# jorgeMFS/HYMET

Hardware: AMD Instinct MI355X
Metric: contigs/s + Mbp/s classified, CAMI-medium, 1/2/4/8 MI355X; % HBM roofline (higher is better)
Workload: dtype u64

## Files before the change

hymet_amd/_lib.py:

```python
from __future__ import annotations

import ctypes
import os

HERE = os.path.dirname(os.path.abspath(__file__))
LIB_PATH = os.path.join(HERE, "libhymet_gpu.so")

_c = ctypes
_i64, _u64, _i32, _u32, _vp = _c.c_int64, _c.c_uint64, _c.c_int, _c.c_uint32, _c.c_void_p

_SIGS = {
    "hymet_version": (_i32, []),
    "hymet_init": (_i32, [_i32, _c.POINTER(_vp)]),
    "hymet_destroy": (_i32, [_vp]),
    "hymet_last_error": (_c.c_char_p, []),
    "hymet_set_stream": (_i32, [_vp, _vp]),
    "hymet_sync": (_i32, [_vp]),
    "hymet_prof_enable": (_i32, [_vp, _i32]),
    "hymet_prof_reset": (_i32, [_vp]),
    "hymet_prof_query": (_i32, [_vp, _c.c_char_p, _c.POINTER(_c.c_double), _c.POINTER(_i64), _c.POINTER(_c.c_double)]),
    "hymet_prof_names": (_i32, [_vp, _c.c_char_p, _i64]),
    "hymet_scratch_trim": (_i32, [_vp, _c.POINTER(_i64)]),
    "hymet_scratch_cached": (_i32, [_vp, _c.POINTER(_i64)]),
    "hymet_scratch_stats": (_i32, [_vp, _vp]),
    "hymet_scratch_reserve": (_i32, [_vp, _i64]),
    "hymet_set_oom_hook": (_i32, [_vp, _vp]),
    "hymet_copy_to_host": (_i32, [_vp, _vp, _vp, _i64, _i32]),
    "hymet_copy_to_device": (_i32, [_vp, _vp, _vp, _i64, _i32]),
    "hymet_pack": (_i32, [_vp, _vp, _i64, _i32, _vp, _vp]),
    "hymet_fasta_index": (_i32, [_vp, _i64, _i32, _i64, _c.POINTER(_i64), _vp, _vp, _vp, _vp, _vp]),
    "hymet_fasta_names": (_i32, [_vp, _vp, _vp, _i64, _vp, _vp]),
    "hymet_fasta_compact": (_i32, [_vp, _vp, _i64, _i64, _vp, _vp, _vp, _i64, _vp, _i64, _vp]),
    "hymet_name_hash": (_i32, [_vp, _vp, _vp, _vp, _i64, _vp]),
    "hymet_sort_pairs_u64": (_i32, [_vp, _vp, _vp, _i64, _i32, _i32]),
    "hymet_scan_u32": (_i32, [_vp, _vp, _vp, _i64, _i32, _vp]),
    "hymet_msh_open": (_i32, [_c.c_char_p, _c.POINTER(_vp)]),
    "hymet_msh_info_get": (_i32, [_vp, _vp]),
    "hymet_msh_copy": (_i32, [_vp, _i32, _vp, _vp, _vp, _vp, _vp, _vp]),
    "hymet_msh_upload": (_i32, [_vp, _vp, _i32, _vp, _vp, _i32]),
    "hymet_msh_upload_range": (_i32, [_vp, _vp, _i32, _vp, _vp, _i32, _i64, _i64]),
    "hymet_msh_text_offsets": (_i32, [_vp, _vp, _vp]),
    "hymet_msh_close": (None, [_vp]),
    "hymet_screen_table_slots": (_i64, [_i64]),
    "hymet_screen_table_build": (_i32, [_vp, _vp, _i64, _vp, _i64, _vp, _vp, _i32]),
    "hymet_screen_count": (_i32, [_vp, _vp, _vp, _i64, _i64, _i64, _i32, _u32, _i32, _c.POINTER(_vp), _c.POINTER(_i64),
                                  _c.POINTER(_vp), _c.POINTER(_i64), _c.POINTER(_vp), _u64, _vp, _i64, _vp, _vp]),
    "hymet_screen_stats": (_i32, [_vp, _vp, _i64, _vp, _vp, _vp, _vp]),
    "hymet_screen_winner": (_i32, [_vp, _vp, _i64, _vp, _vp, _i64, _vp, _i64, _vp, _vp, _vp]),
    "hymet_sketch_max_size": (_i64, []),
    "hymet_sketch_batch": (_i32, [_vp, _vp, _vp, _i64, _i32, _u32, _i32, _i64, _vp, _vp, _vp, _i32, _vp, _vp]),
    "hymet_sketch_counted": (_i32, [_vp, _vp, _vp, _i64, _i32, _u32, _i32, _i32, _i64, _vp, _vp, _vp, _i32, _vp, _vp, _vp,
                                    _vp]),
    "hymet_sketch_counted_max_size": (_i32, []),
    "hymet_sketch_counted_tune": (_i32, [_i32]),
    "hymet_sketch_stream_create": (_i32, [_vp, _i32, _u32, _i32, _i32, _i64, _c.POINTER(_vp)]),
    "hymet_sketch_stream_add": (_i32, [_vp, _vp, _vp, _i64, _i64]),
    "hymet_sketch_stream_end_pass": (_i32, [_vp, _c.POINTER(_i32)]),
    "hymet_sketch_stream_result": (_i32, [_vp, _vp, _vp, _c.POINTER(_i32), _vp]),
    "hymet_sketch_stream_destroy": (_i32, [_vp]),
    "hymet_mash_dist": (_i32, [_vp, _vp, _i64, _vp, _i64, _vp, _i64, _vp, _i64, _i64, _i64, _i32, _vp]),
    "hymet_mash_dist_tile": (_i32, [_i32]),
    "hymet_mash_dist_tune": (_i32, [_i32, _i32]),
    "hymet_mash_dist_select": (_i32, [_vp, _vp, _i64, _i64, _vp, _i32, _vp, _vp, _vp, _i64, _c.POINTER(_i64)]),
    "hymet_mash_dist_tri": (_i32, [_vp, _vp, _i64, _vp, _i64, _i64, _i64, _i32, _vp]),
    "hymet_mash_link": (_i32, [_vp, _vp, _i64, _i64, _i64, _vp, _i32, _vp, _vp]),
    "hymet_mash_labels": (_i32, [_vp, _vp, _i64, _vp]),
    "hymet_mash_dist_sparse": (_i32, [_vp, _vp, _i64, _vp, _i64, _vp, _i64, _vp, _i64, _i64, _i64, _i32, _i32, _vp, _i32,
                                      _i64, _vp, _vp, _vp, _i64, _c.POINTER(_i64), _vp]),
    "hymet_mash_link_edges": (_i32, [_vp, _vp, _i64, _i64, _vp, _vp, _vp]),
    "hymet_mash_greedy": (_i32, [_vp, _vp, _i64, _i64, _i64, _vp, _i32, _vp, _vp, _c.POINTER(_i32)]),
    "hymet_mash_greedy_edges": (_i32, [_vp, _vp, _i64, _i64, _vp, _vp, _i32, _vp, _vp, _c.POINTER(_i32)]),
    "hymet_mash_topk_max": (_i32, []),
    "hymet_mash_topk_tune": (_i32, [_i32]),
    "hymet_mash_dist_topk": (_i32, [_vp, _vp, _i64, _i64, _vp, _i32, _i32, _vp, _vp, _vp]),
    "hymet_mash_topk_edges": (_i32, [_vp, _vp, _i64, _vp, _vp, _i32, _i32, _vp, _vp, _vp]),
    "hymet_mm_sketch": (_i32, [_vp, _vp, _vp, _vp, _vp, _i32, _i32, _i32, _i32, _vp, _vp, _i64, _c.POINTER(_i64)]),
    "hymet_mm_index_build": (_i32, [_vp, _vp, _vp, _vp, _vp, _i32, _i32, _i32, _c.POINTER(_vp)]),
    "hymet_mm_index_destroy": (_i32, [_vp]),
    "hymet_mm_index_info": (_i32, [_vp, _c.POINTER(_i32), _c.POINTER(_i32), _c.POINTER(_i32), _c.POINTER(_i64)]),
    "hymet_mm_index_max_occ": (_i32, [_vp, _vp, _c.c_float, _c.POINTER(_i32)]),
    "hymet_mm_index_save": (_i32, [_vp, _vp, _c.c_char_p, _i32, _c.POINTER(_i64)]),
    "hymet_mm_index_load": (_i32, [_vp, _c.c_char_p, _i64, _c.POINTER(_vp), _c.POINTER(_i64)]),
    "hymet_mm_index_export": (_i32, [_vp, _vp, _vp, _vp]),
    "hymet_mm_map": (_i32, [_vp, _vp, _vp, _vp, _vp, _vp, _vp, _vp, _i32, _c.POINTER(_vp)]),
    "hymet_mm_result_size": (_i32, [_vp, _c.POINTER(_i64)]),
    "hymet_mm_result_copy": (_i32, [_vp, _vp, _vp, _vp]),
    "hymet_mm_result_destroy": (_i32, [_vp]),
    "hymet_paf_acc_create": (_i32, [_vp, _c.POINTER(_vp)]),
    "hymet_paf_acc_reset": (_i32, [_vp]),
    "hymet_paf_acc_destroy": (_i32, [_vp]),
    "hymet_paf_acc_info": (_i32, [_vp, _c.POINTER(_i64), _c.POINTER(_vp), _c.POINTER(_vp), _c.POINTER(_vp),
                                  _c.POINTER(_vp), _c.POINTER(_vp)]),
    "hymet_paf_acc_append": (_i32, [_vp, _vp, _vp, _i64, _i64]),
    "hymet_paf_acc_copy": (_i32, [_vp, _vp, _vp, _vp, _vp]),
    "hymet_paf_acc_field": (_i32, [_vp, _vp, _i32, _vp]),
    "hymet_mm_map_acc": (_i32, [_vp, _vp, _vp, _vp, _vp, _vp, _vp, _vp, _i32, _i32, _i32, _i32, _vp]),
    "hymet_emit_paf": (_i32, [_vp, _vp, _vp, _vp, _vp, _vp, _vp, _vp, _vp, _i64, _c.POINTER(_i64), _vp]),
    "hymet_acc_ref_counts": (_i32, [_vp, _vp, _vp]),
    "hymet_acc_classify": (_i32, [_vp, _vp, _i32, _i32] + [_vp] * 15 + [_c.POINTER(_i32)]),
    "hymet_emit_tsv": (_i32, [_vp, _i32, _i32] + [_vp] * 14 + [_i64, _c.POINTER(_i64)]),
    "hymet_mm_chain_dp": (_i32, [_vp, _vp, _vp, _i64, _i32, _i32, _i32, _i32, _i32, _c.c_float, _c.c_float, _vp, _vp]),
    "hymet_mm_mark_compact": (_i32, [_vp, _vp, _vp, _vp, _i64, _vp, _vp, _i32, _vp, _vp, _vp, _c.POINTER(_i64)]),
    "hymet_mm_stamp_scratch": (_i32, [_vp, _c.POINTER(_i64), _c.POINTER(_i64)]),
    "hymet_mm_anchor_sort": (_i32, [_vp, _vp, _vp, _i64, _vp, _i32, _i32, _i32, _u64, _i64, _vp, _vp, _vp, _vp, _vp]),
    "hymet_lca_ref_counts": (_i32, [_vp, _vp, _i64, _vp]),
    "hymet_lca": (_i32, [_vp, _i32, _i32] + [_vp] * 17),
}

class SparseCounters(_c.Structure):
    _fields_ = [("postings", _i64), ("emitted", _i64), ("candidates", _i64)]


_lib = None
_oom_hook = None


def _release_torch_cache(_user):
    try:
        import torch
        torch.cuda.empty_cache()
    except Exception:
        pass


class HymetError(RuntimeError):
    pass


def load():
    global _lib
    if _lib is not None:
        return _lib
    path = os.environ.get("HYMET_LIB", LIB_PATH)
    if not os.path.exists(path):
        raise HymetError(f"{path} not found: build the HIP extension (python -m hymet_amd.build); "
                         "hymet_amd has no CPU fallback")
    lib = ctypes.CDLL(path)
    for name, (res, args) in _SIGS.items():
        fn = getattr(lib, name)
        fn.restype = res
        fn.argtypes = args
    global _oom_hook
    _oom_hook = _c.CFUNCTYPE(None, _vp)(_release_torch_cache)
    lib.hymet_set_oom_hook(_c.cast(_oom_hook, _vp), None)
    _lib = lib
    return lib


def exported_symbols():
    return list(_SIGS)


def check(rc: int, what: str):
    if rc != 0:
        msg = load().hymet_last_error()
        raise HymetError(f"{what} failed ({rc}): {msg.decode() if msg else ''}")


class Gpu:

    def __init__(self, device: int = 0, stream=None):
        import torch

        if not torch.cuda.is_available():
            raise HymetError("no GPU visible: hymet_amd runs on MI355X (gfx950) only")
        self.torch = torch
        self.device = device
        torch.cuda.set_device(device)
        self.dev = torch.device("cuda", device)
        self.lib = load()
        h = _vp()
        check(self.lib.hymet_init(device, _c.byref(h)), "hymet_init")
        self.ctx = h
        self.stream = stream
        self.children = []
        self.bind_stream(stream)

    def fork(self) -> "Gpu":
        child = Gpu(self.device, stream=self.torch.cuda.Stream(device=self.device))
        self.children.append(child)
        return child

    def bind_stream(self, stream=None):
        s = stream if stream is not None else self.torch.cuda.current_stream(self.device)
        check(self.lib.hymet_set_stream(self.ctx, _vp(s.cuda_stream)), "hymet_set_stream")
        self.bound_stream = s

    def call(self, name, *args):
        check(getattr(self.lib, name)(self.ctx, *args), name)

    def sync(self):
        check(self.lib.hymet_sync(self.ctx), "hymet_sync")
        for ch in self.children:
            ch.sync()

    def prof(self, on: bool = True):
        check(self.lib.hymet_prof_enable(self.ctx, int(on)), "hymet_prof_enable")
        for ch in self.children:
            ch.prof(on)

    def prof_reset(self):
        check(self.lib.hymet_prof_reset(self.ctx), "hymet_prof_reset")
        for ch in self.children:
            ch.prof_reset()

    def prof_table(self):
        buf = _c.create_string_buffer(1 << 16)
        check(self.lib.hymet_prof_names(self.ctx, buf, 1 << 16), "hymet_prof_names")
        out = {}
        for name in buf.value.decode().split():
            ms, n, b = _c.c_double(), _i64(), _c.c_double()
            check(self.lib.hymet_prof_query(self.ctx, name.encode(), _c.byref(ms), _c.byref(n), _c.byref(b)), "hymet_prof_query")
            out[name] = (ms.value, n.value, b.value)
        for ch in self.children:
            for name, (ms, n, b) in ch.prof_table().items():
                m0, n0, b0 = out.get(name, (0.0, 0, 0.0))
                out[name] = (m0 + ms, n0 + n, b0 + b)
        return out

    def trim(self) -> int:
        out = _i64()
        check(self.lib.hymet_scratch_trim(self.ctx, _c.byref(out)), "hymet_scratch_trim")
        return out.value

    def reserve(self, nbytes: int):
        check(self.lib.hymet_scratch_reserve(self.ctx, int(nbytes)), "hymet_scratch_reserve")

    def _alloc(self, fn, n, dtype):
        try:
            return fn(int(n), dtype=dtype, device=self.dev)
        except self.torch.OutOfMemoryError:
            if self.trim() == 0:
                raise
            return fn(int(n), dtype=dtype, device=self.dev)

    def empty(self, n, dtype):
        return self._alloc(self.torch.empty, n, dtype)

    def zeros(self, n, dtype):
        return self._alloc(self.torch.zeros, n, dtype)

    def close(self):
        if self.ctx:
            self.lib.hymet_destroy(self.ctx)
            self.ctx = None

    def __del__(self):
        try:
            self.close()
        except Exception:
            pass


def ptr(t) -> _vp:
    return _vp(t.data_ptr())
```

hymet_amd/csrc/common.hpp:

```cpp
#pragma once
#include <hip/hip_runtime.h>
#include <stdint.h>
#include <algorithm>
#include <cstdlib>
#include <map>
#include <string>
#include <utility>
#include <vector>
#include "../../include/hymet_gpu.h"

struct hymet_ctx {
    int device = 0;
    hipStream_t stream = nullptr;
    bool own_stream = false;
    int n_cu = 256;
    bool prof = false;
    std::map<std::string, std::vector<std::pair<hipEvent_t, hipEvent_t>>> ev;
    std::map<std::string, double> bytes;
    std::map<std::string, std::pair<int, double>> dev_bytes;
    int64_t *prof_dev = nullptr;
    void *stage[2] = {nullptr, nullptr};
    hipEvent_t stage_ev[2] = {nullptr, nullptr};
    int64_t *mbox_h = nullptr;
    int64_t *mbox_d = nullptr;
    int32_t *dctr = nullptr;
    int32_t *stamp = nullptr;
    int64_t stamp_cap = 0;
    size_t stamp_cls = 0;
};

namespace hymet {
struct ProfScope {
    hymet_ctx *c;
    const char *name;
    hipEvent_t a = nullptr, b = nullptr;
    ProfScope(hymet_ctx *ctx, const char *n, double alg_bytes = 0.0) : c(ctx), name(n) {
        if (c && c->prof && hipEventCreate(&a) == hipSuccess && hipEventCreate(&b) == hipSuccess) {
            (void)hipEventRecord(a, c->stream);
            c->bytes[name] += alg_bytes;
        }
    }
    ProfScope(hymet_ctx *ctx, const char *n, int slot, double per_unit) : ProfScope(ctx, n, 0.0) {
        if (c && c->prof) c->dev_bytes[name] = {slot, per_unit};
    }
    ~ProfScope() {
        if (c && c->prof && a && b) {
            (void)hipEventRecord(b, c->stream);
            c->ev[name].push_back({a, b});
        }
    }
};
constexpr int kProfSlots = 8;
inline int64_t *prof_dev_slot(hymet_ctx *c, int k) { return c && c->prof && c->prof_dev ? c->prof_dev + k : nullptr; }
}

namespace hymet {
constexpr int kMbox = 64;
inline int64_t *mb_dev(hymet_ctx *c, int i) { return c->mbox_d + i; }
inline int64_t mb_read(const hymet_ctx *c, int i) { return __atomic_load_n(c->mbox_h + i, __ATOMIC_ACQUIRE); }
}

namespace hymet {
inline const char *env_str(const char *name) {
    const char *e = getenv(name);
    return e && *e ? e : nullptr;
}
inline bool env_flag(const char *name, bool dflt = false) {
    const char *e = env_str(name);
    return e ? e[0] != '0' : dflt;
}
inline int64_t env_int(const char *name, int64_t dflt, int64_t lo, int64_t hi) {
    const char *e = env_str(name);
    return e ? std::max(lo, std::min(hi, (int64_t)atoll(e))) : dflt;
}
}

namespace hymet {
void set_error(const std::string &msg);
int fail(int code, const std::string &msg);
int hip_fail(hipError_t e, const char *what);
inline int64_t cdiv(int64_t a, int64_t b) { return (a + b - 1) / b; }
hipError_t scratch_alloc(size_t bytes, hipStream_t stream, void **p, size_t *cls);
void set_oom_hook(void (*hook)(void *), void *user);
void scratch_free(void *p, hipStream_t stream, size_t cls);
hipError_t stamp_scratch(hymet_ctx *ctx, int64_t n, int32_t **out);
void stamp_release(hymet_ctx *ctx);
}

#define HY_CHECK_LAUNCH(what)                                   \
    do {                                                        \
        hipError_t e_ = hipGetLastError();                      \
        if (e_ != hipSuccess) return hymet::hip_fail(e_, what); \
    } while (0)

#define HY_HIP(call)                                            \
    do {                                                        \
        hipError_t e_ = (call);                                 \
        if (e_ != hipSuccess) return hymet::hip_fail(e_, #call); \
    } while (0)

#define HY_ARG(cond, msg)                                                   \
    do {                                                                    \
        if (!(cond)) return hymet::fail(HYMET_E_ARG, std::string(msg));     \
    } while (0)
```

hymet_amd/csrc/mm_chain.hip:

```cpp
#include "mm_common.hpp"

#include <cstdlib>
#include <string>

namespace hymet {
namespace mm {
namespace {

#ifndef HYMET_CHAIN_RING
#define HYMET_CHAIN_RING 128
#endif
#ifndef HYMET_CHAIN_SUMRING
#define HYMET_CHAIN_SUMRING 16
#endif
#ifndef HYMET_CHAIN_BDQ
#define HYMET_CHAIN_BDQ 32
#endif
#ifndef HYMET_CHAIN_IDQ
#define HYMET_CHAIN_IDQ 64
#endif
#ifndef HYMET_CHAIN_SPEC_GAP0
#define HYMET_CHAIN_SPEC_GAP0 2
#endif
#ifndef HYMET_CHAIN_WPE
// ... 1000 lines not shown
                            const int m = min(ni, 64), base = ni - m;
                            bool gt = false;
                            int2 v = make_int2(0, 0);
                            if (lane < m) {
                                v = L(base + lane);
                                gt = key_less(e0y, i, v.x, v.y);
                            }
                            const uint64_t mg = __ballot(gt);
                            const int ngt = __popcll(mg);
                            if (ngt == m && base > 0) {
                                gy = INT32_MIN;
                            } else {
                                gpos = ni - ngt;
                                const int lg = __ffsll((unsigned long long)mg) - 1;
                                gy = rl(v.x, lg), gj = rl(v.y, lg);
                            }
                        }
                        if (lane >= 1 && !key_less(py, i + lane - 1, gy, gj)) ok = false;
                        gap_own = key_less(ky, i + lane, gy, gj);
                    }
#ifdef HYMET_CHAIN_PROF
                    const bool ok_geom = ok;
#endif
                    ok = ok && cand_ok && wok;
                    const uint64_t bad = __ballot(!ok);
                    const int acc = bad ? __ffsll((unsigned long long)bad) - 1 : 64;
#ifdef HYMET_CHAIN_PROF
                    if (acc < Lb) {
                        const int fl = acc;
                        const bool g_ = rl(ok_geom ? 1 : 0, fl), c_ = rl(cand_ok ? 1 : 0, fl), w_ = rl(wok ? 1 : 0, fl);
                        const bool xs = rl(kx != px ? 1 : 0, fl), yr = rl((py > ky - P.max_dist && py < ky) ? 1 : 0, fl);
                        if (!xs) CCOUNT(12);
                        else if (!yr) CCOUNT(13);
                        else if (!g_) CCOUNT(14);
                        else if (!c_) CCOUNT(15);
                        else if (!w_) CCOUNT(16);
                        else CCOUNT(17);
                    }
                    _pcnt[18] += acc;
#endif
                    if (acc < 4) {
                        spec_next = i + spec_gap;
                        spec_gap = min(spec_gap * 2, 64);
                    } else {
                        spec_gap = kSpecGap0;
                    }
                    AMARK(batch_verified);
                    if (acc > 0) {
                        bool ins_all = false;
                        if (i + acc < n) {
                            const int offn = (i - cb) + 64;
                            const int32_t xn = acc < 64 ? rl(kx, acc) : rl(nx, offn - 64);
                            ins_all = xn != rl(kx, acc - 1) && rl(gap_own ? 1 : 0, acc - 1) != 0;
                        }
                        advance(i + acc);
                        const int32_t k = i + lane;
                        const int32_t pk_local = linked ? (lane == 0 ? b0j : k - 1) : -1;
                        const int32_t pw = (int32_t)((uint32_t)(pk_local + 1) | (uint32_t)span_pw);
                        if (lane < acc) {
                            ring[k & kRingMask] = make_int4(kx, ky, fk, pw);
                            xring[k & (kXRing - 1)] = kx;
                        }
                        __builtin_amdgcn_wave_barrier();
                        CCOUNT(7);
                        GCNT(z, 1);
                        GCNT(w, acc);
                        const int nins = ins_all ? acc : acc - 1;
                        if (nins > 0) {
                            if (P.max_dist_inner > 0) {
                                if (gpos < ni) {
                                    const int kk = gpos + lane;
                                    const int2 v = L(kk);
                                    __builtin_amdgcn_wave_barrier();
                                    if (kk < ni) L(kk + nins) = v;
                                }
                                {
                                    if (lane < nins) L(gpos + lane) = make_int2(ky, k);
                                    __builtin_amdgcn_wave_barrier();
                                }
                                if (gpos == 0) lfy = rl(ky, 0), lfj = i;
                                if (gpos == ni) lby = rl(ky, nins - 1), lbj = i + nins - 1;
                                ni += nins;
                                const int v = fk + ksp;
                                int run = lane < nins ? v : INT32_MIN;
                                int sfx;
                                const int vnx = down1(v);
                                if (__ballot(lane >= nins - 1 || v < vnx) == ~0ull) {
                                    run = rl(v, nins - 1);
                                    sfx = lane < nins - 1 ? run : INT32_MIN;
                                } else
                                {
                                    run = suffix_max(run);
                                    sfx = down1(run);
                                    if (lane == 63) sfx = INT32_MIN;
                                }
                                const int vmax = rl(run, 0);
                                while (it > ih && ib_v <= vmax) {
                                    --it;
                                    if (it > ih) ib_v = idq[(it - 1) & (kIdq - 1)].y;
                                }
                                const bool recd = lane < nins && v > sfx;
                                const uint64_t rm = __ballot(recd);
                                const int nr = __popcll(rm);
                                if (it - ih + nr > kIdq) {
                                    iok = false;
                                } else {
                                    const int rank = __popcll(rm & ((1ull << lane) - 1));
                                    if (recd) idq[(it + rank) & (kIdq - 1)] = make_int2(k, v);
                                    __builtin_amdgcn_wave_barrier();
                                    if (it == ih) if_v = rl(v, __ffsll((unsigned long long)rm) - 1);
                                    ib_v = rl(v, 63 - __clzll((long long)rm));
                                    it += nr;
                                }
                            }
                            const int32_t nb0 = i >> 6, nb1 = (i + nins) >> 6;
                            for (int32_t b = nb0; b < nb1; ++b) complete_block(b);
                            const double pl_last = rld(pk, nins - 1);
                            if (((i + nins) & 63) == 0) {
                                t_pr = 0.0, t_j = -1, t_y = 0;
                            } else if (rld(ipm, nins - 1) == pl_last) {
                                if (nb1 > nb0 || (i & 63) == 0 || t_j < 0 || !(t_pr < pl_last))
                                    t_pr = pl_last, t_j = i + nins - 1, t_y = rl(ky, nins - 1);
                            } else
                            {
                                const int32_t tb = (i + nins) & ~63, j = tb + lane;
                                double tp = 0.0;
                                int32_t tj = -1, ty = 0;
                                if (j < i + nins) {
                                    const Ent e = fetch(j);
                                    tp = prio(e.f, e.x, e.y, c), tj = j, ty = e.y;
                                }
                                wave_argmin(tp, tj, ty);
                                t_pr = Ud(tp), t_j = U(tj), t_y = U(ty);
                            }
                            i0 = i + nins;
                        }
                        const int l = acc - 1;
                        if (lane < acc) {
                            P.f[g0 + k] = fk;
                            P.p[g0 + k] = pk_local < 0 ? -1 : (int32_t)(g0 + pk_local);
                        }
                        prev.x = rl(kx, l), prev.y = rl(ky, l), prev.f = rl(fk, l), prev.pw = rl(pw, l);
                        i += acc;
                        AMARK(batch_end);
                        continue;
                    }
                }
            }
            CPROF(2);
            double bp = 0.0;
            int32_t bj = -1;
            Ent eb;
            bool have_eb = false;
            const int32_t ylo = yi - P.max_dist;
            auto in_range = [&](int32_t y, int32_t j) { return y > ylo && (y < yi || (y == yi && qfirst && j == 0)); };
            if (st < i0) {
                bool cert = st <= (fe << 6);
                int32_t wy = 0, src = -1;
                if (cert) {
                    if (st < (fb << 6)) {
                        const int4 v = hsuf[st & 63];
                        bp = st_pr(v), bj = v.z, wy = v.w, src = 0;
                    }
                    if (fb < fe) {
                        if (!bok) cert = false;
                        else if (better(bf_pr, bf_j, bp, bj)) bp = bf_pr, bj = bf_j, wy = bf_y, src = 1;
                    }
                    if ((fe << 6) < i0 && better(t_pr, t_j, bp, bj)) bp = t_pr, bj = t_j, wy = t_y, src = 2;
                }
                if (cert && bj >= 0 && in_range(wy, bj)) {
                    if (src == 1) eb.x = bf_e.x, eb.y = bf_y, eb.f = bf_e.y, eb.pw = bf_e.z, have_eb = true;
                } else {
                    CCOUNT(3);
                    if (cert && bj >= 0) CCOUNT(6);
                    window_best(yi, ylo, true, bp, bj);
                }
            }
            CPROF(3);
            if (bj >= 0) {
                int32_t exact, width;
                if (!have_eb) eb = bj == i - 1 ? prev : fetch(bj);
                const int32_t sc = eb.f + comput_sc(xi, yi, eb.x, eb.y, eb.sp(), P.pen_gap, P.pen_skip, &exact, &width);
                if (width <= P.bw && sc > max_f) max_f = sc, max_j = bj;
                const int32_t n_inner = i0 > st_in ? i0 - st_in : 0;
                bool walk = !exact && n_inner > 0 && yi > 0 && P.max_dist_inner > 0;
                if (walk && iok && it > ih && if_v <= max_f) walk = false;
                CPROF(5);
                if (walk) {
                    CCOUNT(4);
                    const int32_t ylo_in = yi - P.max_dist_inner;
                    if (!overflow) {
                        int cnt = 0;
                        for (int e = lane; e < ni; e += 64) cnt += L(e).x < yi;
                        cnt = wave_sum(cnt);
                        int nsk = 0;
                        for (int top = cnt - 1; top >= 0; top -= 64) {
                            const int e = top - lane;
                            const int nl = min(64, top + 1);
                            int32_t yj = 0, jl = -1, sc_l = 0, w_l = INT32_MAX, pj = -1;
                            if (e >= 0) {
                                const int2 v = L(e);
                                yj = v.x, jl = v.y;
                                const Ent ej = fetch_p(jl);
                                int32_t ex;
                                sc_l = ej.f + comput_sc(xi, yi, ej.x, ej.y, ej.sp(), P.pen_gap, P.pen_skip, &ex, &w_l);
                                pj = ej.p();
                            }
                            const uint64_t mA = __ballot(e >= 0 && yj < ylo_in);
                            const int LA = mA ? __ffsll((unsigned long long)mA) - 1 : nl;
                            const bool valid = lane < LA && w_l <= P.bw;
                            if (valid && pj >= st_in && pj < i0) P.t_global[g0 + pj] = i + 1;
                            t_used = true;
                            __builtin_amdgcn_s_waitcnt(0);
                            const bool stamped = valid && ld_l2(P.t_global + g0 + jl) == i + 1;
                            const int incl = scan_max(valid ? sc_l : INT32_MIN);
                            const int excl = max(shr1(incl, INT32_MIN), max_f);
                            const bool imp = valid && sc_l > excl;
                            int a = imp ? -1 : (valid && stamped ? 1 : 0);
                            int bb = imp ? 0 : kNegInf;
                            scan_maxplus(a, bb);
                            const int s = max(nsk + a, bb);
                            const uint64_t mB = __ballot(valid && !imp && stamped && s > P.max_chn_skip);
                            const int LB = mB ? __ffsll((unsigned long long)mB) - 1 : 64;
                            const int lim = min(LA, LB + 1);
                            const uint64_t mI = __ballot(imp && lane < lim);
                            if (mI) {
                                const int Lh = 63 - __clzll((long long)mI);
                                max_f = rl(sc_l, Lh);
                                max_j = rl(jl, Lh);
                            }
                            if (mB || LA < nl) break;
                            nsk = rl(s, 63);
                            __builtin_amdgcn_wave_barrier();
                        }
                    } else {
                        int n_skip = 0;
                        int32_t cy_ = yi, cj = INT32_MIN;
                        bool first = true;
                        for (;;) {
                            int32_t by = INT32_MIN, bjl = INT32_MIN;
                            for (int32_t j = st_in + lane; j < i0; j += 64) {
                                const int32_t yj = fetch(j).y;
                                const bool below = first ? (yj <= yi - 1) : key_less(yj, j, cy_, cj);
                                if (below && (bjl == INT32_MIN || key_less(by, bjl, yj, j))) by = yj, bjl = j;
                            }
                            auto take = [&](int32_t oy, int32_t oj) {
                                if (oj != INT32_MIN && (bjl == INT32_MIN || key_less(by, bjl, oy, oj))) by = oy, bjl = oj;
                            };
                            take(xstep<0>(by), xstep<0>(bjl));
                            take(xstep<1>(by), xstep<1>(bjl));
                            take(xstep<2>(by), xstep<2>(bjl));
                            take(xstep<3>(by), xstep<3>(bjl));
                            take(xstep<4>(by), xstep<4>(bjl));
                            take(xstep<5>(by), xstep<5>(bjl));
                            if (bjl == INT32_MIN) break;
                            first = false;
                            cy_ = by, cj = bjl;
                            if (by < ylo_in) break;
                            const Ent ej = fetch_p(bjl);
                            int32_t ex, wl;
                            const int32_t sl = ej.f + comput_sc(xi, yi, ej.x, ej.y, ej.sp(), P.pen_gap, P.pen_skip, &ex, &wl);
                            if (wl <= P.bw) {
                                if (sl > max_f) {
                                    max_f = sl, max_j = bjl;
                                    if (n_skip > 0) --n_skip;
                                } else if (ld_l2(P.t_global + g0 + bjl) == i + 1) {
                                    if (++n_skip > P.max_chn_skip) break;
                                }
                                if (ej.p() >= 0) P.t_global[g0 + ej.p()] = i + 1;
                                t_used = true;
                            }
                        }
                    }
                }
            }
            CPROF(4);
            advance(i + 1);
            P.f[g0 + i] = max_f;
            P.p[g0 + i] = max_j < 0 ? -1 : (int32_t)(g0 + max_j);
            prev.x = xi, prev.y = yi, prev.f = max_f, prev.pw = (int32_t)((uint32_t)(max_j + 1) | (uint32_t)span_pw);
            if (lane == 0) {
                ring[i & kRingMask] = make_int4(prev.x, prev.y, prev.f, prev.pw);
                xring[i & (kXRing - 1)] = prev.x;
            }
            __builtin_amdgcn_wave_barrier();
            ++i;
        }
        if (t_used) {
            __builtin_amdgcn_wave_barrier();
            for (int32_t j = lane; j < n; j += 64) P.t_global[g0 + j] = 0;
        }
        CPROF_FLUSH;
        GTIME_STOP;
    }
}

struct BacktrackParams {
    const int64_t *g_start;
    const int32_t *f;
    const int32_t *p;
    uint8_t *t;
    const int32_t *z_cnt;
    const int32_t *z_idx;
    int32_t n_groups;
    int min_cnt, min_sc, max_drop;
    int64_t long_min;
    unsigned long long *prof;
    int32_t *chain_ids;
    uint64_t *chain_u;
    int64_t *chain_first;
    int32_t *n_chains;
};

constexpr int kBtWin = 8;

constexpr int64_t kBtLong = 64;
#ifndef HYMET_BT_GRAB
#define HYMET_BT_GRAB 1
#endif
#ifndef HYMET_BT_STRIPES
#define HYMET_BT_STRIPES 8
#endif
constexpr int kBtGrab = HYMET_BT_GRAB, kBtStripes = HYMET_BT_STRIPES, kBtCtrPad = 64;
#ifndef HYMET_BT_CHUNKS
#define HYMET_BT_CHUNKS 1
#endif
constexpr int kBtChunks = HYMET_BT_CHUNKS;
#ifndef HYMET_BT_PROBE
#define HYMET_BT_PROBE 4
#endif
constexpr int kBtProbe = HYMET_BT_PROBE;

__device__ __forceinline__ int32_t uni(int32_t v) { return __builtin_amdgcn_readfirstlane(v); }
__device__ __forceinline__ int64_t uni64(int64_t v) {
    return (int64_t)((uint64_t)(uint32_t)uni((int32_t)(v >> 32)) << 32 | (uint32_t)uni((int32_t)v));
}

__global__ void bt_long_count_kernel(const int64_t *g_start, const int32_t *order, int32_t n_work, int64_t long_min,
                                     int32_t *cnt) {
    int lo = 0, hi = n_work;
    while (lo < hi) {
        const int mid = (lo + hi) >> 1;
        const int g = order[mid];
        if (g_start[g + 1] - g_start[g] > long_min) lo = mid + 1;
        else hi = mid;
    }
    cnt[0] = lo;
    for (int k = 1; k <= kBtStripes; k++) cnt[k * kBtCtrPad] = 0;
}

__global__ __launch_bounds__(64) void backtrack_long_kernel(BacktrackParams P, const int32_t *list, const int32_t *cnt,
                                                            int32_t *counter) {
    __shared__ int32_t s_w;
    const int lane = threadIdx.x;
    const int32_t n_long = uni(ld_l2(cnt));
    int stripe = (int)(blockIdx.x % kBtStripes), exhausted = 0;
    int32_t w = 0, w_end = 0;
    for (;;) {
        if (w >= w_end) {
            for (;;) {
                if (lane == 0) s_w = atomicAdd(counter + stripe * kBtCtrPad, kBtGrab);
                __syncthreads();
                w = uni(s_w);
                __syncthreads();
                w_end = w + kBtGrab;
                if (stripe + kBtStripes * w < n_long || ++exhausted == kBtStripes) break;
                stripe = stripe + 1 == kBtStripes ? 0 : stripe + 1;
            }
            if (exhausted == kBtStripes) break;
        }
        const int32_t wcur = stripe + kBtStripes * w++;
        if (wcur >= n_long) {
            w = w_end;
            continue;
        }
        const int32_t g = uni(list[wcur]);
        const int64_t g0 = uni64(P.g_start[g]);
        const int64_t z0 = g0, z1 = g0 + uni(P.z_cnt[g]);
        int64_t wpos = g0;
        int nc = 0;
        int64_t k = z1 - 1;
        uint64_t c_probe = 0, c_walk = 0, c_step = 0, c_reload = 0, t_walk = 0, t_post = 0;
        const uint64_t t_g0 = P.prof ? clock64() : 0;
        int64_t ptop = -1;
        int64_t zrem = z1 - z0;
        int32_t zc[kBtProbe], tv[kBtProbe], zfv[kBtProbe];
        int32_t zpv[kBtProbe];
        int32_t tqv[kBtProbe], fqv[kBtProbe];
        bool stale = false;
        while (k >= z0 && zrem > 0) {
            if (ptop < 0 || k <= ptop - 64 * kBtProbe) {
                c_probe++;
                ptop = k;
                stale = false;
#pragma unroll
                for (int c = 0; c < kBtProbe; c++) {
                    const int64_t kk = k - 64 * c - lane;
                    zc[c] = kk >= z0 ? P.z_idx[kk] : 0;
                }
#pragma unroll
                for (int c = 0; c < kBtProbe; c++) {
                    const int64_t kk = k - 64 * c - lane;
                    tv[c] = kk >= z0 ? ld_l2(P.t + zc[c]) : 1;
                }
#pragma unroll
                for (int c = 0; c < kBtProbe; c++) {
                    zfv[c] = tv[c] == 0 ? P.f[zc[c]] : 0;
                    zpv[c] = tv[c] == 0 ? P.p[zc[c]] : -1;
                }
#pragma unroll
                for (int c = 0; c < kBtProbe; c++) {
                    const bool q = tv[c] == 0 && zpv[c] >= 0;
                    tqv[c] = q ? ld_l2(P.t + zpv[c]) : 0;
                    fqv[c] = q ? P.f[zpv[c]] : 0;
                }
            } else if (stale) {
                stale = false;
#pragma unroll
                for (int c = 0; c < kBtProbe; c++) {
                    const int64_t kk = ptop - 64 * c - lane;
                    if (kk >= z0 && kk <= k && tv[c] == 0) tv[c] = ld_l2(P.t + zc[c]);
                }
            }
            const int d = (int)(ptop - k);
            int hit = -1;
            int32_t zsel = 0, zfsel = 0;
            int32_t zpsel = -1;
            int32_t tqsel = 0, fqsel = 0;
#pragma unroll
            for (int c = kBtProbe - 1; c >= 0; c--) {
                const uint64_t m = __ballot(tv[c] == 0 && 64 * c + lane >= d);
                if (m) {
                    const int h = __ffsll((unsigned long long)m) - 1;
                    hit = 64 * c + h;
                    zsel = __builtin_amdgcn_readlane(zc[c], h);
                    zfsel = __builtin_amdgcn_readlane(zfv[c], h);
                    zpsel = __builtin_amdgcn_readlane(zpv[c], h);
                    tqsel = __builtin_amdgcn_readlane(tqv[c], h);
                    fqsel = __builtin_amdgcn_readlane(fqv[c], h);
                }
            }
            hit = uni(hit);
            if (hit < 0) {
                k = ptop - 64 * kBtProbe;
                continue;
            }
            const int64_t zi = (int64_t)uni(zsel);
            k = ptop - hit - 1;
            const int32_t zf = uni(zfsel);
            if (P.min_cnt >= 2 && (zpsel < 0 || uni(tqsel) != 0)) {
                const int32_t sv = zpsel < 0 ? zf : zf - uni(fqsel);
                if (sv > 0) P.t[zi] = 1, zrem--;
                c_walk++;
                continue;
            }
            stale = true;
            int32_t *buf = P.chain_ids + wpos;
            buf[0] = (int32_t)zi;
            P.t[zi] = 2;
            int64_t len = 1, nv = 0;
            int64_t zc_len = 1, zc_nv = 0;
            int32_t max_s = 0;
            int64_t nxt = (int64_t)uni(zpsel);
            int64_t whi = -1;
            int32_t wpc[kBtChunks], wfc[kBtChunks], wtc[kBtChunks];
#pragma unroll
            for (int c = 0; c < kBtChunks; c++) wpc[c] = -1, wfc[c] = 0, wtc[c] = 1;
            c_walk++;
            const uint64_t t_w0 = P.prof ? clock64() : 0;
            for (;;) {
                c_step++;
                if (nxt < 0) {
                    if (zf > max_s) max_s = zf, nv = len, zc_nv = zc_len;
                    break;
                }
                if (nxt > whi || nxt <= whi - 64 * kBtChunks) {
                    c_reload++;
                    whi = nxt;
#pragma unroll
                    for (int c = 0; c < kBtChunks; c++) {
                        const int64_t jj = nxt - 64 * c - lane;
                        const bool ok = jj >= g0;
                        wpc[c] = ok ? P.p[jj] : -1;
                        wfc[c] = ok ? P.f[jj] : 0;
                        wtc[c] = ok ? ld_l2(P.t + jj) : 1;
                    }
                }
                const int d = (int)(whi - nxt);
                const int cc = d >> 6, o = d & 63;
                int32_t wp = wpc[0], wf = wfc[0], wt = wtc[0];
#pragma unroll
                for (int c = 1; c < kBtChunks; c++)
                    if (cc == c) wp = wpc[c], wf = wfc[c], wt = wtc[c];
                const int64_t j = whi - 64 * cc - lane;
                const bool in = lane >= o;
                const uint64_t ms = __ballot(in && (lane == 63 || wp != j - 1 || j - 1 < g0));
                const int R = uni(__ffsll((unsigned long long)ms) - 1);
                const bool cand = in && lane <= R;
                const int32_t sv = cand ? zf - wf : INT32_MIN;
                const int32_t incl = scan_max(sv);
                const int32_t ex = max(max_s, shr1(incl, INT32_MIN));
                const bool upd = cand && sv > ex;
                const bool drop = cand && !upd && (int64_t)ex - sv > P.max_drop;
                const uint64_t mdrop = __ballot(drop);
                const uint64_t mb = mdrop | __ballot(cand && wt != 0);
                const uint64_t mupd = __ballot(upd);
                int last = R, ulim = R;
                const bool done = mb != 0;
                if (done) {
                    const int E = uni(__ffsll((unsigned long long)mb) - 1);
                    last = E - 1;
                    ulim = (mdrop >> E) & 1 ? E - 1 : E;
                }
                const uint64_t lim = ulim < 0 ? 0ull : ulim >= 63 ? ~0ull : (2ull << ulim) - 1;
                const uint64_t mu = mupd & lim;
                const uint64_t mz = __ballot(lane >= o && lane <= last && wf >= P.min_sc);
                if (mu) {
                    const int u = 63 - __clzll((long long)mu);
                    nv = len + (u - o);
                    zc_nv = zc_len + __popcll(mz & ((1ull << u) - 1));
                    max_s = __builtin_amdgcn_readlane(incl, u);
                }
                if (lane >= o && lane <= last) {
                    buf[len + (lane - o)] = (int32_t)j;
                    P.t[j] = 2;
                }
                len += last - o + 1;
                zc_len += __popcll(mz);
                if (done) break;
                nxt = (int64_t)__builtin_amdgcn_readlane(wp, R);
            }
            const uint64_t t_w1 = P.prof ? clock64() : 0;
            t_walk += t_w1 - t_w0;
            __builtin_amdgcn_fence(__ATOMIC_SEQ_CST, "workgroup");
            for (int64_t a = nv + lane; a < len; a += 64) P.t[ld_l2(buf + a)] = 0;
            zrem -= zc_nv;
            const int32_t sc = nv == 0 ? 0 : max_s;
            if (sc >= P.min_sc && nv > 0 && nv >= P.min_cnt) {
                P.chain_u[g0 + nc] = (uint64_t)(uint32_t)sc << 32 | (uint32_t)nv;
                P.chain_first[g0 + nc] = wpos;
                nc++;
                wpos += nv;
            } else {
                for (int64_t a = lane; a < nv; a += 64) P.t[ld_l2(buf + a)] = 1;
            }
            __builtin_amdgcn_fence(__ATOMIC_SEQ_CST, "workgroup");
            if (P.prof) t_post += clock64() - t_w1;
        }
        P.n_chains[g] = nc;
        if (P.prof) {
            const uint64_t v[8] = {1, c_probe, c_walk, c_step, c_reload, t_walk, t_post, clock64() - t_g0};
            for (int q = 0; q < 8; q++) atomicAdd(P.prof + q, lane == 0 ? (unsigned long long)v[q] : 0ull);
        }
    }
}


__global__ __launch_bounds__(64) void backtrack_groups_kernel(BacktrackParams P) {
    const int g = blockIdx.x * blockDim.x + threadIdx.x;
    if (g >= P.n_groups) return;
    const int64_t g0 = P.g_start[g];
    if (P.g_start[g + 1] - g0 > P.long_min) return;
    int64_t wpos = g0;
    int nc = 0;
    const int64_t z0 = g0, z1 = g0 + P.z_cnt[g];
    int64_t k = z1 - 1;
    while (k >= z0) {
        int32_t zc[kBtWin], tc[kBtWin];
#pragma unroll
        for (int u = 0; u < kBtWin; u++) zc[u] = k - u >= z0 ? P.z_idx[k - u] : 0;
#pragma unroll
        for (int u = 0; u < kBtWin; u++) tc[u] = k - u >= z0 ? P.t[zc[u]] : 1;
        int hit = -1;
#pragma unroll
        for (int u = kBtWin - 1; u >= 0; u--)
            if (tc[u] == 0) hit = u;
        if (hit < 0) {
            k -= kBtWin;
            continue;
        }
        int64_t zi = 0;
#pragma unroll
        for (int u = 0; u < kBtWin; u++)
            if (u == hit) zi = zc[u];
        k -= hit + 1;
        const int32_t zf = P.f[zi];
        int32_t *buf = P.chain_ids + wpos;
        int64_t len = 0, nv = 0;
        int32_t max_s = 0;
        int64_t i = zi, nxt = P.p[zi];
        int64_t whi = -1;
        int32_t wp[kBtWin], wf[kBtWin], wt[kBtWin];
        for (;;) {
            buf[len++] = (int32_t)i;
            P.t[i] = 2;
            int32_t fn = 0, tn = 1;
            int64_t pn = -1;
            if (nxt >= 0) {
                if (nxt > whi || nxt <= whi - kBtWin) {
                    whi = nxt;
#pragma unroll
                    for (int u = 0; u < kBtWin; u++) {
                        const bool ok = nxt - u >= g0;
                        wp[u] = ok ? P.p[nxt - u] : -1;
                        wf[u] = ok ? P.f[nxt - u] : 0;
                        wt[u] = ok ? P.t[nxt - u] : 1;
                    }
                }
                const int64_t o = whi - nxt;
#pragma unroll
                for (int u = 0; u < kBtWin; u++)
                    if (o == u) fn = wf[u], tn = wt[u], pn = wp[u];
            }
            const int32_t s = nxt < 0 ? zf : zf - fn;
            if (s > max_s) {
                max_s = s;
                nv = len;
            } else if (max_s - s > P.max_drop) {
                break;
            }
            if (nxt < 0 || tn != 0) break;
            i = nxt;
            nxt = pn;
        }
        const int32_t sc = nv == 0 ? 0 : max_s;
        for (int64_t a = nv; a < len; a++) P.t[buf[a]] = 0;
        if (sc >= P.min_sc && nv > 0 && nv >= P.min_cnt) {
            P.chain_u[g0 + nc] = (uint64_t)(uint32_t)sc << 32 | (uint32_t)nv;
            P.chain_first[g0 + nc] = wpos;
            nc++;
            wpos += nv;
        } else {
            for (int64_t a = 0; a < nv; a++) P.t[buf[a]] = 1;
        }
    }
    P.n_chains[g] = nc;
}

}


#ifndef HYMET_CHAIN_SMALL
#define HYMET_CHAIN_SMALL 24
#endif
constexpr int kSmall = HYMET_CHAIN_SMALL;
#ifndef HYMET_CHAIN_SMALL_LONG
#define HYMET_CHAIN_SMALL_LONG 16
#endif
constexpr int kSmallLong = HYMET_CHAIN_SMALL_LONG < kSmall ? HYMET_CHAIN_SMALL_LONG : kSmall;

__global__ void chain_small_split_kernel(const int64_t *g_start, const int32_t *order, int32_t n_work, int32_t *split,
                                         int32_t *counter, int small_max) {
    if (threadIdx.x != 0) return;
    for (int k = 0; k < kChainStripes; k++) counter[k * kChainCtrPad] = 0;
    int32_t lo = 0, hi = n_work;
    while (lo < hi) {
        const int32_t mid = (lo + hi) >> 1;
        const int g = order[mid];
        if (g_start[g + 1] - g_start[g] <= small_max) hi = mid;
        else lo = mid + 1;
    }
    *split = lo;
}

__global__ __launch_bounds__(256) void chain_work_anchors_kernel(const int64_t *g_start, const int32_t *order,
                                                                  int32_t n_work, const int32_t *split, int64_t *cnt) {
    __shared__ unsigned long long sw, ss;
    if (threadIdx.x == 0) sw = 0, ss = 0;
    __syncthreads();
    const int32_t sp = *split;
    unsigned long long w = 0, s = 0;
    for (int32_t k = blockIdx.x * 256 + threadIdx.x; k < n_work; k += gridDim.x * 256) {
        const int g = order[k];
        const unsigned long long a = (unsigned long long)(g_start[g + 1] - g_start[g]);
        if (k < sp) w += a;
        else s += a;
    }
    for (int o = 32; o > 0; o >>= 1) w += __shfl_xor(w, o), s += __shfl_xor(s, o);
    if ((threadIdx.x & 63) == 0) atomicAdd(&sw, w), atomicAdd(&ss, s);
    __syncthreads();
    if (threadIdx.x == 0) {
        atomicAdd(reinterpret_cast<unsigned long long *>(cnt), sw);
        atomicAdd(reinterpret_cast<unsigned long long *>(cnt + 1), ss);
    }
}

__global__ __launch_bounds__(64) void chain_small_kernel(ChainParams P, const int32_t *split) {
    const int32_t w = *split + (int32_t)(blockIdx.x * 64 + threadIdx.x);
    if (w >= P.n_work) return;
    const int g = P.order[w];
    const int64_t g0 = P.g_start[g];
    const int n = (int)(P.g_start[g + 1] - g0);
    const bool qfirst = P.g_qfirst[g] != 0;
    const double c = 0.5 * (double)P.pen_gap;
    int32_t X[kSmall], Y[kSmall], F[kSmall], PJ[kSmall], T[kSmall];
    int8_t ord[kSmall];
    for (int j = 0; j < n; ++j) {
        X[j] = P.ax[g0 + j], Y[j] = (int32_t)P.ay[g0 + j];
        F[j] = 0, PJ[j] = -1, T[j] = -1;
        int k = j;
        while (k > 0 && Y[ord[k - 1]] > Y[j]) {
            ord[k] = ord[k - 1];
            --k;
        }
        ord[k] = (int8_t)j;
    }
    uint32_t in_out = 0, in_in = 0;
    int size_out = 0, size_in = 0, i0 = 0, st = 0, st_in = 0;
    for (int i = 0; i < n; ++i) {
        const int32_t xi = X[i], yi = Y[i];
        int32_t max_f = P.span, max_j = -1;
        if (i0 < i && X[i0] != xi) {
            for (int j = i0; j < i; ++j) {
                in_out |= 1u << j, size_out++;
                if (P.max_dist_inner > 0) in_in |= 1u << j, size_in++;
            }
            i0 = i;
        }
        while (st < i && ((int64_t)(uint32_t)xi > (int64_t)(uint32_t)X[st] + P.max_dist || size_out > P.cap_rmq_size)) {
            if (st < i0) in_out &= ~(1u << st), size_out--;
            ++st;
        }
        if (P.max_dist_inner > 0)
            while (st_in < i &&
                   ((int64_t)(uint32_t)xi > (int64_t)(uint32_t)X[st_in] + P.max_dist_inner || size_in > P.cap_rmq_size)) {
                if (st_in < i0) in_in &= ~(1u << st_in), size_in--;
                ++st_in;
            }
        double bp = 0.0;
        int32_t bj = -1;
        const int32_t ylo = yi - P.max_dist;
        for (uint32_t m = in_out; m; m &= m - 1) {
            const int j = __ffs(m) - 1;
            const int32_t yj = Y[j];
            if (yj > ylo && (yj < yi || (yj == yi && qfirst && j == 0))) {
                const double pr = prio(F[j], X[j], yj, c);
                if (better(pr, j, bp, bj)) bp = pr, bj = j;
            }
        }
        if (bj >= 0) {
            int32_t exact, width;
            const int32_t sc = F[bj] + comput_sc(xi, yi, X[bj], Y[bj], P.span, P.pen_gap, P.pen_skip, &exact, &width);
            if (width <= P.bw && sc > max_f) max_f = sc, max_j = bj;
            if (!exact && size_in > 0 && yi > 0) {
                const int32_t ylo_in = yi - P.max_dist_inner;
                int r = n - 1;
                while (r >= 0 && Y[ord[r]] >= yi) --r;
                int n_skip = 0;
                for (; r >= 0; --r) {
                    const int jj = ord[r];
                    if (Y[jj] < ylo_in) break;
                    if (!(in_in >> jj & 1)) continue;
                    int32_t ex2, w2;
                    const int32_t sc2 = F[jj] + comput_sc(xi, yi, X[jj], Y[jj], P.span, P.pen_gap, P.pen_skip, &ex2, &w2);
                    if (w2 <= P.bw) {
                        if (sc2 > max_f) {
                            max_f = sc2, max_j = jj;
                            if (n_skip > 0) --n_skip;
                        } else if (T[jj] == i) {
                            if (++n_skip > P.max_chn_skip) break;
                        }
                        if (PJ[jj] >= 0) T[PJ[jj]] = i;
                    }
                }
            }
        }
        F[i] = max_f, PJ[i] = max_j;
        P.f[g0 + i] = max_f;
        P.p[g0 + i] = max_j < 0 ? -1 : (int32_t)(g0 + max_j);
    }
}

int launch_chain_raw(hipStream_t st, const ChainParams &P0, int64_t blocks, int32_t *split) {
    ChainParams P = P0;
    hipLaunchKernelGGL(chain_small_split_kernel, dim3(1), dim3(64), 0, st, P.g_start, P.order, P.n_work, split,
                       P.work_counter, P.max_dist > 10000 ? kSmallLong : kSmall);
    HY_CHECK_LAUNCH("chain_small_split_kernel");
    P.work_end = split;
    const bool long_pass = P.max_dist > 10000;
    if (long_pass) hipLaunchKernelGGL(chain_groups_kernel<1>, dim3((unsigned)blocks), dim3(64), kChainLds, st, P);
    else hipLaunchKernelGGL(chain_groups_kernel<0>, dim3((unsigned)blocks), dim3(64), kChainLds, st, P);
    HY_CHECK_LAUNCH("chain_groups_kernel");
    hipLaunchKernelGGL(chain_small_kernel, dim3((unsigned)cdiv(P.n_work, 64)), dim3(64), 0, st, P, (const int32_t *)split);
    HY_CHECK_LAUNCH("chain_small_kernel");
    return HYMET_OK;
}

int launch_chain(hymet_ctx *ctx, const int32_t *ax, const uint32_t *ay, int span, const int64_t *g_start, const uint8_t *g_qfirst,
                 const int32_t *order, int32_t n_work, int32_t *f, int32_t *p, int32_t *t_global, int max_dist,
                 int max_dist_inner, int bw, int max_chn_skip, int cap_rmq_size, float pen_gap, float pen_skip,
                 int64_t n_anchors, int64_t n_groups) {
    if (n_work <= 0) return HYMET_OK;
    DevBuf cnt, sum, split;
    const size_t n_sum = (size_t)(n_anchors >> 6) + (size_t)n_groups + 2;
    HY_HIP(sum.alloc(16 * kGSumInts * n_sum, ctx->stream));
    HY_HIP(cnt.alloc(4 * (size_t)kChainCtrPad * kChainStripes, ctx->stream));
    HY_HIP(split.alloc(4, ctx->stream));
    if (max_dist < bw) max_dist = bw;
    if (max_dist_inner <= 0 || max_dist_inner >= max_dist) max_dist_inner = 0;
    ChainParams P{ax, ay, span, g_start, g_qfirst, order, n_work, cnt.as<int32_t>(), f, p, t_global, sum.as<int4>(), max_dist, max_dist_inner, bw, max_chn_skip, cap_rmq_size, pen_gap, pen_skip, nullptr};
    int64_t blocks = n_work;
    int per_cu = 0;
    const bool long_pass = max_dist > 10000;
    auto kern = long_pass ? chain_groups_kernel<1> : chain_groups_kernel<0>;
    if (hipOccupancyMaxActiveBlocksPerMultiprocessor(&per_cu, kern, 64, kChainLds) != hipSuccess ||
        per_cu <= 0)
        per_cu = 8;
    per_cu = (int)env_int("HYMET_CHAIN_WAVES", per_cu, 1, per_cu);
    const int64_t cap = (int64_t)ctx->n_cu * per_cu;
    if (blocks > cap) blocks = cap;
    const int slot = long_pass ? 2 : 0;
    hipStream_t st = ctx->stream;
    {
        ProfScope _ps(ctx, long_pass ? "mm_chain_long" : "mm_chain", slot, 24.0);
        hipLaunchKernelGGL(chain_small_split_kernel, dim3(1), dim3(64), 0, st, P.g_start, P.order, P.n_work,
                           split.as<int32_t>(), P.work_counter, long_pass ? kSmallLong : kSmall);
        HY_CHECK_LAUNCH("chain_small_split_kernel");
        if (int64_t *pc = prof_dev_slot(ctx, slot)) {
            const unsigned wb = (unsigned)std::min<int64_t>(cdiv(P.n_work, 256), 1024);
            hipLaunchKernelGGL(chain_work_anchors_kernel, dim3(wb), dim3(256), 0, st, P.g_start, P.order, P.n_work,
                               (const int32_t *)split.as<int32_t>(), pc);
            HY_CHECK_LAUNCH("chain_work_anchors_kernel");
        }
        P.work_end = split.as<int32_t>();
        if (long_pass) hipLaunchKernelGGL(chain_groups_kernel<1>, dim3((unsigned)blocks), dim3(64), kChainLds, st, P);
        else hipLaunchKernelGGL(chain_groups_kernel<0>, dim3((unsigned)blocks), dim3(64), kChainLds, st, P);
        HY_CHECK_LAUNCH("chain_groups_kernel");
    }
    ProfScope _pl(ctx, long_pass ? "mm_chain_long_small" : "mm_chain_small", slot + 1, 24.0);
    hipLaunchKernelGGL(chain_small_kernel, dim3((unsigned)cdiv(P.n_work, 64)), dim3(64), 0, st, P, (const int32_t *)split.as<int32_t>());
    HY_CHECK_LAUNCH("chain_small_kernel");
    return HYMET_OK;
}

int launch_backtrack(hymet_ctx *ctx, const int64_t *g_start, const int32_t *f, const int32_t *p, uint8_t *t,
                     const int32_t *z_cnt, const int32_t *z_idx, int32_t n_groups, const int32_t *order, int32_t n_work,
                     int min_cnt, int min_sc, int max_drop, int32_t *chain_ids, uint64_t *chain_u, int64_t *chain_first,
                     int32_t *n_chains, int64_t n_anchors) {
    if (n_groups <= 0) return HYMET_OK;
    const int64_t long_min = env_int("HYMET_BT_LONG", kBtLong, 0, INT64_MAX);
    const bool prof = env_flag("HYMET_BT_PROF");
    DevBuf pbuf;
    if (prof) {
        HY_HIP(pbuf.alloc(64, ctx->stream));
        HY_HIP(hipMemsetAsync(pbuf.p, 0, 64, ctx->stream));
    }
    BacktrackParams P{g_start,  f,         p,       t,           z_cnt,    z_idx, n_groups, min_cnt, min_sc, max_drop,
                      long_min, (unsigned long long *)pbuf.p, chain_ids, chain_u, chain_first, n_chains};
    DevBuf cnt;
    HY_HIP(cnt.alloc(4 * (size_t)kBtCtrPad * (kBtStripes + 1), ctx->stream));
    ProfScope _ps(ctx, "mm_backtrack", 18.0 * (double)n_anchors);
    if (n_work > 0) {
        hipLaunchKernelGGL(bt_long_count_kernel, dim3(1), dim3(1), 0, ctx->stream, g_start, order, n_work, long_min,
                           cnt.as<int32_t>());
        HY_CHECK_LAUNCH("bt_long_count_kernel");
    }
    hipLaunchKernelGGL(backtrack_groups_kernel, dim3((unsigned)cdiv(n_groups, 64)), dim3(64), 0, ctx->stream, P);
    HY_CHECK_LAUNCH("backtrack_groups_kernel");
    if (n_work > 0) {
        ProfScope _pl(ctx, "mm_backtrack.long");
        const int per_cu = (int)env_int("HYMET_BT_WAVES", 24, 1, 1024);
        const int64_t nb = std::min<int64_t>(n_work, (int64_t)ctx->n_cu * per_cu);
        hipLaunchKernelGGL(backtrack_long_kernel, dim3((unsigned)nb), dim3(64), 0, ctx->stream, P, order,
                           cnt.as<int32_t>(), cnt.as<int32_t>() + kBtCtrPad);
        HY_CHECK_LAUNCH("backtrack_long_kernel");
    }
    if (prof) {
        unsigned long long h[8];
        HY_HIP(hipMemcpyAsync(h, pbuf.p, 64, hipMemcpyDeviceToHost, ctx->stream));
        HY_HIP(hipStreamSynchronize(ctx->stream));
        fprintf(stderr, "[bt_long] groups=%llu probes=%llu walks=%llu steps=%llu reloads=%llu cyc_walk=%.3g cyc_post=%.3g cyc_all=%.3g\n",
                h[0], h[1], h[2], h[3], h[4], (double)h[5], (double)h[6], (double)h[7]);
    }
    return HYMET_OK;
}

}
}
```

hymet_amd/csrc/mm_chainset.hip:

```cpp
#include "mm_stages.hpp"

#include <algorithm>
#include <cstdio>

namespace hymet {
namespace mm {

int launch_chain(hymet_ctx *ctx, const int32_t *ax, const uint32_t *ay, int span, const int64_t *g_start, const uint8_t *g_qfirst,
                 const int32_t *order, int32_t n_work, int32_t *f, int32_t *p, int32_t *t_global, int max_dist,
                 int max_dist_inner, int bw, int max_chn_skip, int cap_rmq_size, float pen_gap, float pen_skip,
                 int64_t n_anchors, int64_t n_groups);
int launch_backtrack(hymet_ctx *ctx, const int64_t *g_start, const int32_t *f, const int32_t *p, uint8_t *t,
                     const int32_t *z_cnt, const int32_t *z_idx, int32_t n_groups, const int32_t *order, int32_t n_work,
                     int min_cnt, int min_sc, int max_drop, int32_t *chain_ids, uint64_t *chain_u, int64_t *chain_first,
                     int32_t *n_chains, int64_t n_anchors);

namespace {

constexpr int kGTile = 16384;

__device__ __forceinline__ uint64_t group_tile_bits(const uint32_t *hb, int64_t n, const int64_t *qoff, int n_q, int64_t t0,
                                                    uint64_t *qs) {
    __shared__ int s_q0;
    const int tid = threadIdx.x;
    const int64_t t1 = min(t0 + kGTile, n);
    const int64_t a0 = t0 + 64 * (int64_t)tid;
    const uint64_t hw = a0 < n ? reinterpret_cast<const uint64_t *>(hb)[a0 >> 6] : 0;
    qs[tid] = 0;
    if (tid == 0) {
        int lo = 0, hi = n_q;
        while (lo < hi) {
            const int mid = (lo + hi) >> 1;
            if (qoff[mid + 1] <= t0) lo = mid + 1;
            else hi = mid;
        }
        s_q0 = lo;
    }
    __syncthreads();
    for (int q = s_q0 + tid; q < n_q; q += 256) {
        const int64_t a = qoff[q];
        if (a >= t1) break;
        if (a >= t0 && a < qoff[q + 1]) atomicOr((unsigned long long *)&qs[(a - t0) >> 6], 1ull << ((a - t0) & 63));
    }
    __syncthreads();
    const int64_t m = n - a0;
    const uint64_t live = m >= 64 ? ~0ull : m > 0 ? (1ull << m) - 1 : 0ull;
    return (hw | qs[tid]) & live;
}

__global__ __launch_bounds__(256) void group_heads_count_kernel(const uint32_t *hb, int64_t n, const int64_t *qoff, int n_q,
                                                          uint32_t *tile_cnt) {
    __shared__ uint64_t qs[kGTile / 64];
    __shared__ uint32_t ws[4];
    const uint64_t h = group_tile_bits(hb, n, qoff, n_q, (int64_t)blockIdx.x * kGTile, qs);
    uint32_t c = (uint32_t)__popcll(h);
    for (int o = 32; o > 0; o >>= 1) c += (uint32_t)__shfl_xor((int)c, o, 64);
    if ((threadIdx.x & 63) == 0) ws[threadIdx.x >> 6] = c;
    __syncthreads();
    if (threadIdx.x == 0) tile_cnt[blockIdx.x] = ws[0] + ws[1] + ws[2] + ws[3];
}

__global__ __launch_bounds__(256) void group_heads_write_kernel(const uint32_t *hb, int64_t n, const int64_t *qoff, int n_q,
                                                          const int64_t *tile_off, int64_t *g_start, uint8_t *qfirst,
                                                          int64_t G) {
    __shared__ uint64_t qs[kGTile / 64];
    __shared__ uint32_t ws[4];
    const int64_t t0 = (int64_t)blockIdx.x * kGTile;
    uint64_t h = group_tile_bits(hb, n, qoff, n_q, t0, qs);
    const int lane = threadIdx.x & 63, w = threadIdx.x >> 6;
    const uint32_t c = (uint32_t)__popcll(h);
    uint32_t inc = c;
    for (int d = 1; d < 64; d <<= 1) {
        const uint32_t o = (uint32_t)__shfl_up((int)inc, d, 64);
        if (lane >= d) inc += o;
    }
    if (lane == 63) ws[w] = inc;
    __syncthreads();
    int64_t g = tile_off[blockIdx.x] + inc - c;
    for (int k = 0; k < w; k++) g += ws[k];
    const uint64_t qw = qs[threadIdx.x];
    const int64_t a0 = t0 + 64 * (int64_t)threadIdx.x;
    while (h) {
        const int b = __ffsll((unsigned long long)h) - 1;
        h &= h - 1;
        g_start[g] = a0 + b;
        qfirst[g] = (uint8_t)(qw >> b & 1);
        ++g;
    }
    if (blockIdx.x == gridDim.x - 1 && threadIdx.x == 0) g_start[G] = n;
}

__global__ void x_low_kernel(const uint64_t *x, int64_t n, uint32_t *x32) {
    const int64_t i = (int64_t)blockIdx.x * blockDim.x + threadIdx.x;
    if (i < n) x32[i] = (uint32_t)x[i];
}

__global__ __launch_bounds__(256) void head_bits_x_kernel(const uint64_t *x, int64_t n, uint64_t *hb) {
    const int64_t i = (int64_t)blockIdx.x * 256 + threadIdx.x;
    const bool hd = i < n && (i == 0 || (x[i] >> 32) != (x[i - 1] >> 32));
    const uint64_t b = __ballot(hd);
    if ((threadIdx.x & 63) == 0 && i < n) hb[i >> 6] = b;
}

__global__ void max_group_kernel(const int64_t *g_start, const int32_t *order, int32_t G, int64_t *out) {
    if (blockIdx.x != 0 || threadIdx.x != 0) return;
    int64_t best = 0;
    for (int32_t w = 0; w < G; w++) {
        const int g = order[w];
        const int64_t sz = g_start[g + 1] - g_start[g];
        best = max(best, sz);
        if (sz < 0xffff) break;
    }
    *out = best;
}

__global__ void nonwork_fp_kernel(const int64_t *g_start, int32_t G, int min_cnt, int32_t *f, int32_t *p) {
    const int g = blockIdx.x * blockDim.x + threadIdx.x;
    if (g >= G) return;
    const int64_t a0 = g_start[g], a1 = g_start[g + 1];
    if (a1 - a0 >= min_cnt) return;
    for (int64_t a = a0; a < a1; a++) f[a] = 0, p[a] = -1;
}

__global__ void group_size_kernel(const int64_t *g_start, int32_t G, int min_cnt, uint32_t *key, uint32_t *gidx,
                                  uint32_t *is_work, uint8_t *qfirst, int32_t *zlists) {
    const int g = blockIdx.x * blockDim.x + threadIdx.x;
    if (g < 8) zlists[g] = 0;
    if (g >= G) return;
    if (qfirst) qfirst[g] = 0;
    const int64_t sz = g_start[g + 1] - g_start[g];
    key[g] = 0xffffu - (uint32_t)min(sz, (int64_t)0xffff);
    gidx[g] = (uint32_t)g;
    is_work[g] = sz >= min_cnt ? 1u : 0u;
}

constexpr int kZs = 2048;
constexpr int kZRuns = 16;
constexpr int kZmLds = 6144;
constexpr int kZmUnit = 2048;
constexpr int kZLane = 16;
#ifndef HYMET_Z_DEPTH
#define HYMET_Z_DEPTH 8
#endif
constexpr int kZDepth = HYMET_Z_DEPTH;

struct ZParams {
    const int32_t *f;
    const int64_t *g_start;
    const int32_t *order;
    int32_t G;
    int min_sc, max_runs;
    int zm_lds, zm_unit;
    uint64_t *zkey;
    int32_t *z_idx;
    int32_t *z_cnt;
    int32_t *z_runs;
    int32_t *run_start;
    int32_t *lists;
    int32_t *merge_list;
    int64_t *mergeu_list;
    int32_t *mid_list;
    int32_t *big_list;
    int64_t *big_off;
    int64_t *mail;
};

__global__ void zsplit_kernel(ZParams P) {
    if (threadIdx.x != 0 || blockIdx.x != 0) return;
    int32_t lo = 0, hi = P.G;
    while (lo < hi) {
        const int32_t mid = (lo + hi) >> 1;
        const int g = P.order[mid];
        if (P.g_start[g + 1] - P.g_start[g] <= kZLane) hi = mid;
        else lo = mid + 1;
    }
    P.lists[0] = lo;
}

__device__ __forceinline__ uint64_t shfl64(uint64_t v, int src) {
    const uint32_t lo = (uint32_t)__shfl((int)(uint32_t)v, src, 64);
    const uint32_t hi = (uint32_t)__shfl((int)(uint32_t)(v >> 32), src, 64);
    return (uint64_t)hi << 32 | lo;
}

__global__ __launch_bounds__(256) void zorder_wave_kernel(ZParams P) {
    const int lane = threadIdx.x & 63;
    const int32_t split = P.lists[0];
    const int nw = (int)(gridDim.x * (blockDim.x >> 6));
    int32_t pend[3] = {0, 0, 0};
    int np[3] = {0, 0, 0};
    unsigned long long big_m = 0;
    int32_t *const lst[3] = {P.merge_list, P.mid_list, P.big_list};
    auto flush = [&](int l) {
        if (np[l] == 0) return;
        int base = 0;
        if (lane == 0) base = atomicAdd(P.lists + (l == 0 ? 3 : l == 1 ? 1 : 2), np[l]);
        base = __shfl(base, 0, 64);
        if (lane < np[l]) lst[l][base + lane] = pend[l];
        np[l] = 0;
    };
    auto push = [&](int l, int g) {
        if (lane == np[l]) pend[l] = g;
        if (++np[l] == 64) flush(l);
    };
    for (int wb = (int)(blockIdx.x * (blockDim.x >> 6) + (threadIdx.x >> 6)); wb < split; wb += 64 * nw) {
        const int64_t wl = (int64_t)wb + (int64_t)lane * nw;
        int gl = 0;
        int64_t sl = 0, el = 0;
        if (wl < split) {
            gl = P.order[wl];
            sl = P.g_start[gl];
            el = P.g_start[gl + 1];
        }
        const int nr = (int)min((int64_t)64, ((int64_t)split - wb + nw - 1) / nw);
        for (int r = 0; r < nr; r++) {
            const int g = __builtin_amdgcn_readlane(gl, r);
            const int64_t g0 = (int64_t)((uint64_t)(uint32_t)__builtin_amdgcn_readlane((int32_t)(sl >> 32), r) << 32 |
                                         (uint32_t)__builtin_amdgcn_readlane((int32_t)sl, r));
            const int64_t n = (int64_t)((uint64_t)(uint32_t)__builtin_amdgcn_readlane((int32_t)(el >> 32), r) << 32 |
                                        (uint32_t)__builtin_amdgcn_readlane((int32_t)el, r)) - g0;
            int32_t *rs = P.run_start + (int64_t)g * kZRuns;
            int m = 0, K = 0;
            uint64_t last = 0;
            const uint64_t below = (1ull << lane) - 1;
            for (int64_t base0 = 0; base0 < n; base0 += 64 * kZDepth) {
                int32_t fc[kZDepth];
#pragma unroll
                for (int d = 0; d < kZDepth; d++) {
                    const int64_t i = base0 + 64 * d + lane;
                    fc[d] = i < n ? P.f[g0 + i] : 0;
                }
#pragma unroll
                for (int d = 0; d < kZDepth; d++) {
                    const int64_t i = base0 + 64 * d + lane;
                    const bool ok = i < n;
                    const int32_t fv = fc[d];
                    const bool z = ok && fv >= P.min_sc;
                    const uint64_t bal = __ballot(z);
                    if (bal == 0) continue;
                    const uint64_t key = (uint64_t)(uint32_t)fv << 32 | (uint32_t)(g0 + i);
                    const uint64_t lower = bal & below;
                    const int pos = m + __popcll(lower);
                    const int prev = lower ? 63 - __clzll((long long)lower) : lane;
                    uint64_t pk = shfl64(key, prev);
                    if (!lower) pk = last;
                    const bool desc = z && pos > 0 && key < pk;
                    const uint64_t dbal = __ballot(desc);
                    if (z) P.z_idx[g0 + pos] = (int32_t)(g0 + i);
                    if (desc) {
                        const int r = K + 1 + __popcll(dbal & below);
                        if (r < kZRuns) rs[r] = pos;
                    }
                    K += __popcll(dbal);
                    m += __popcll(bal);
                    last = shfl64(key, 63 - __clzll((long long)bal));
                }
            }
            const int runs = m > 0 ? K + 1 : 0;
            if (lane == 0) {
                rs[0] = 0;
                P.z_cnt[g] = m;
                P.z_runs[g] = runs;
            }
            if (runs > 1) {
                int m2 = 0;
                for (int64_t base0 = 0; base0 < n; base0 += 64 * kZDepth) {
                    int32_t fc[kZDepth];
#pragma unroll
                    for (int d = 0; d < kZDepth; d++) {
                        const int64_t i = base0 + 64 * d + lane;
                        fc[d] = i < n ? P.f[g0 + i] : 0;
                    }
#pragma unroll
                    for (int d = 0; d < kZDepth; d++) {
                        const int64_t i = base0 + 64 * d + lane;
                        const bool z = i < n && fc[d] >= P.min_sc;
                        const uint64_t bal = __ballot(z);
                        if (bal == 0) continue;
                        if (z) P.zkey[g0 + m2 + __popcll(bal & below)] = (uint64_t)(uint32_t)fc[d] << 32 | (uint32_t)(g0 + i);
                        m2 += __popcll(bal);
                    }
                }
            }
            if (runs > 1 && runs <= P.max_runs) {
                if (m <= P.zm_lds) {
                    push(0, g);
                } else {
                    const int nu = (m + P.zm_unit - 1) / P.zm_unit;
                    int base = 0;
                    if (lane == 0) base = atomicAdd(P.lists + 6, nu);
                    base = __shfl(base, 0, 64);
                    for (int u = lane; u < nu; u += 64) P.mergeu_list[base + u] = (int64_t)g << 32 | (uint32_t)u;
                }
            }
            if (runs > P.max_runs) {
                if (m <= kZs) {
                    push(1, g);
                } else {
                    push(2, g);
                    big_m += (unsigned long long)m;
                }
            }
        }
    }
    flush(0), flush(1), flush(2);
    if (lane == 0 && big_m) atomicAdd((unsigned long long *)(P.lists + 4), big_m);
}

__global__ __launch_bounds__(256) void zorder_lane_kernel(ZParams P) {
    const int32_t w = P.lists[0] + (int32_t)(blockIdx.x * blockDim.x + threadIdx.x);
    if (w >= P.G) return;
    const int g = P.order[w];
    const int64_t g0 = P.g_start[g];
    const int n = (int)(P.g_start[g + 1] - g0);
    uint64_t key[kZLane];
#pragma unroll
    for (int j = 0; j < kZLane; j++) {
        const int32_t fv = j < n ? P.f[g0 + j] : 0;
        key[j] = j < n && fv >= P.min_sc ? (uint64_t)(uint32_t)fv << 32 | (uint32_t)(g0 + j) : ~0ull;
    }
    int m = 0;
#pragma unroll
    for (int j = 0; j < kZLane; j++) {
        if (key[j] == ~0ull) continue;
        int r = 0;
#pragma unroll
        for (int k = 0; k < kZLane; k++) r += key[k] < key[j];
        P.z_idx[g0 + r] = (int32_t)(uint32_t)key[j];
        m++;
    }
    P.z_cnt[g] = m;
    P.z_runs[g] = m > 0 ? 1 : 0;
}

__device__ __forceinline__ void zmerge_group(const uint64_t *zk, const int32_t *rs, int K, int m, int qa, int qb,
                                             int32_t *out) {
    const int S = (qb - qa + (int)blockDim.x - 1) / (int)blockDim.x;
    const int q0 = qa + (int)threadIdx.x * S, q1 = min(q0 + S, qb);
    if (q0 >= qb) return;
    int rsr[kZRuns + 1], lo[kZRuns];
#pragma unroll
    for (int k = 0; k <= kZRuns; k++) rsr[k] = k <= K ? rs[k] : m;
    int own = 0, own_s = 0;
#pragma unroll
    for (int k = 1; k < kZRuns; k++)
        if (k < K && rsr[k] <= q0) own = k, own_s = rsr[k];
    uint64_t prev = ~0ull;
    for (int q = q0; q < q1; q++) {
        const uint64_t key = zk[q];
        const bool restart = key < prev;
        prev = key;
        if (restart && q > q0) own++, own_s = q;
        int pos = q - own_s;
#pragma unroll
        for (int k = 0; k < kZRuns; k++) {
            if (k < K && k != own) {
                const int s1 = rsr[k + 1];
                int l = restart ? rsr[k] : lo[k];
                if (l < s1 && zk[l] < key) {
                    int b = 1;
                    while (l + b < s1 && zk[l + b] < key) {
                        l += b;
                        b <<= 1;
                    }
                    int a = l + 1, e = min(l + b, s1);
                    while (a < e) {
                        const int mid = (a + e) >> 1;
                        if (zk[mid] < key) a = mid + 1;
                        else e = mid;
                    }
                    l = a;
                }
                lo[k] = l;
                pos += l - rsr[k];
            }
        }
        out[pos] = (int32_t)(uint32_t)key;
    }
}

__global__ __launch_bounds__(256) void zmerge_kernel(ZParams P) {
    __shared__ uint64_t sk[kZmLds];
    __shared__ int32_t srs[kZRuns + 1];
    const int n_list = P.lists[3], n_units = P.lists[6];
    if (blockIdx.x == 0 && threadIdx.x == 0) {
        P.mail[0] = P.lists[2];
        P.mail[1] = *reinterpret_cast<const int64_t *>(P.lists + 4);
    }
    for (int w = blockIdx.x; w < n_units + n_list; w += gridDim.x) {
        const bool unit = w < n_units;
        const int64_t uw = unit ? P.mergeu_list[w] : 0;
        const int g = unit ? (int)(uw >> 32) : P.merge_list[w - n_units];
        const int K = P.z_runs[g];
        const int64_t z0 = P.g_start[g];
        const int m = P.z_cnt[g];
        const int32_t *rs = P.run_start + (int64_t)g * kZRuns;
        const uint64_t *zk = P.zkey + z0;
        __syncthreads();
        if (threadIdx.x <= K) srs[threadIdx.x] = threadIdx.x < K ? rs[threadIdx.x] : m;
        if (!unit)
            for (int q = threadIdx.x; q < m; q += blockDim.x) sk[q] = zk[q];
        __syncthreads();
        if (unit) {
            const int qa = (int)(uint32_t)uw * P.zm_unit;
            zmerge_group(zk, srs, K, m, qa, min(qa + P.zm_unit, m), P.z_idx + z0);
        } else {
            zmerge_group(sk, srs, K, m, 0, m, P.z_idx + z0);
        }
    }
}

__global__ __launch_bounds__(256) void zsort_block_kernel(ZParams P) {
    __shared__ uint64_t s[kZs];
    const int n_list = P.lists[1];
    for (int w = blockIdx.x; w < n_list; w += gridDim.x) {
        const int g = P.mid_list[w];
        const int64_t z0 = P.g_start[g];
        const int n = P.z_cnt[g];
        int np = 128;
        while (np < n) np <<= 1;
        for (int i = threadIdx.x; i < np; i += 256) s[i] = i < n ? P.zkey[z0 + i] : ~0ull;
        __syncthreads();
        for (int k = 2; k <= np; k <<= 1)
            for (int j = k >> 1; j > 0; j >>= 1) {
                for (int i = threadIdx.x; i < np; i += 256) {
                    const int ij = i ^ j;
                    if (ij > i) {
                        const uint64_t a = s[i], b = s[ij];
                        if (((i & k) == 0) == (a > b)) {
                            s[i] = b;
                            s[ij] = a;
                        }
                    }
                }
                __syncthreads();
            }
        for (int i = threadIdx.x; i < n; i += 256) P.z_idx[z0 + i] = (int32_t)(uint32_t)s[i];
        __syncthreads();
    }
}

__global__ void zbig_count_kernel(ZParams P, int32_t n_big, uint32_t *cnt) {
    const int r = blockIdx.x * blockDim.x + threadIdx.x;
    if (r < n_big) cnt[r] = (uint32_t)P.z_cnt[P.big_list[r]];
}

__global__ void zbig_gather_kernel(ZParams P, uint64_t *skey, uint32_t *sval) {
    const int r = blockIdx.x, g = P.big_list[r];
    const int64_t z0 = P.g_start[g], n = P.z_cnt[g], o = P.big_off[r];
    for (int64_t t = threadIdx.x; t < n; t += blockDim.x) {
        const uint64_t k = P.zkey[z0 + t];
        skey[o + t] = (uint64_t)r << 32 | (k >> 32);
        sval[o + t] = (uint32_t)k;
    }
}

__global__ void zbig_scatter_kernel(ZParams P, const uint32_t *sval) {
    const int r = blockIdx.x, g = P.big_list[r];
    const int64_t z0 = P.g_start[g], n = P.z_cnt[g], o = P.big_off[r];
    for (int64_t t = threadIdx.x; t < n; t += blockDim.x) P.z_idx[z0 + t] = (int32_t)sval[o + t];
}

__global__ void chain_list_kernel(const int64_t *g_start, const int32_t *n_chains, const int64_t *c_pos, int32_t G,
                                  const uint64_t *chain_u, const int64_t *chain_first, const int32_t *chain_ids,
                                  uint64_t *ckey, uint64_t *cu, int64_t *cfirst) {
    const int g = blockIdx.x * blockDim.x + threadIdx.x;
    if (g >= G) return;
    const int64_t g0 = g_start[g];
    int64_t o = c_pos[g];
    for (int c = 0; c < n_chains[g]; c++, o++) {
        const int64_t fo = chain_first[g0 + c];
        ckey[o] = (uint64_t)chain_ids[fo + (uint32_t)chain_u[g0 + c] - 1];
        cu[o] = chain_u[g0 + c];
        cfirst[o] = fo;
    }
}

__global__ void chain_cnt_kernel(const uint64_t *cu, const uint32_t *cq, const uint32_t *qflag, int64_t n, uint32_t *cnt,
                                 uint32_t *cnt2) {
    const int64_t i = (int64_t)blockIdx.x * blockDim.x + threadIdx.x;
    if (i >= n) return;
    const uint32_t m = (uint32_t)cu[i];
    const bool fl = qflag && qflag[cq[i]];
    cnt[i] = fl ? 0u : m;
    if (cnt2) cnt2[i] = fl ? m : 0u;
}

__global__ void rechain_flag_kernel(const uint32_t *ay, const int32_t *chain_ids, const uint64_t *cu, const int64_t *cfirst,
                                    const int64_t *qc, const int64_t *qlen, int n_q, int rescue_size, float rescue_ratio,
                                    uint32_t *flag) {
    const int q = blockIdx.x * blockDim.x + threadIdx.x;
    if (q >= n_q) return;
    const int64_t c0 = qc[q], nc = qc[q + 1] - c0;
    uint32_t f = 0;
    if (nc > 1) {
        const int32_t m = (int32_t)cu[c0];
        const int64_t fo = cfirst[c0];
        const int32_t st = (int32_t)ay[chain_ids[fo + m - 1]], en = (int32_t)ay[chain_ids[fo]];
        const int32_t ql = (int32_t)qlen[q];
        if (ql - (en - st) > rescue_size || (float)(en - st) > __fmul_rn((float)ql, rescue_ratio)) f = 1;
    }
    flag[q] = f;
}

__global__ void chain_qb_kernel(const int64_t *qc, const int64_t *bpos, int64_t n_chain, int64_t nb, int n_q, int64_t *qb) {
    const int q = blockIdx.x * blockDim.x + threadIdx.x;
    if (q > n_q) return;
    const int64_t c = qc[q];
    qb[q] = c < n_chain ? bpos[c] : nb;
}

__device__ __forceinline__ uint32_t keep_bits16(const uint8_t *t, int64_t n, const uint32_t *qflag, const int64_t *qoff,
                                                int n_q, int64_t e0) {
    if (e0 >= n) return 0u;
    int lo = 0, hi = n_q - 1;
    while (lo < hi) {
        const int mid = (lo + hi + 1) >> 1;
        if (qoff[mid] <= e0) lo = mid;
        else hi = mid - 1;
    }
    int q = lo;
    int64_t qend = qoff[q + 1];
    uint32_t v[4] = {0, 0, 0, 0};
    if (e0 + 16 <= n) {
        const uint4 w = *reinterpret_cast<const uint4 *>(t + e0);
        v[0] = w.x, v[1] = w.y, v[2] = w.z, v[3] = w.w;
    } else {
#pragma unroll
        for (int u = 0; u < 16; u++) v[u >> 2] |= (e0 + u < n ? (uint32_t)t[e0 + u] : 0u) << (8 * (u & 3));
    }
    uint32_t bits = 0, fl = qflag[q];
#pragma unroll
    for (int u = 0; u < 16; u++) {
        while (e0 + u >= qend && q + 1 < n_q) {
            q++;
            qend = qoff[q + 1];
            fl = qflag[q];
        }
        bits |= (uint32_t)((v[u >> 2] >> (8 * (u & 3)) & 0xffu) == 2u && fl != 0) << u;
    }
    return bits;
}

__global__ __launch_bounds__(256) void mark_count_kernel(const uint8_t *t, int64_t n, const uint32_t *qflag,
                                                         const int64_t *qoff, int n_q, uint32_t *cnt, int64_t *last_kept) {
    __shared__ uint32_t ws[4];
    __shared__ int64_t wl[4];
    const int64_t e0 = (int64_t)blockIdx.x * 4096 + threadIdx.x * 16;
    const uint32_t kb = keep_bits16(t, n, qflag, qoff, n_q, e0);
    uint32_t c = __popc(kb);
    long long l = kb ? e0 + 31 - __clz((int)kb) : -1;
    for (int o = 32; o > 0; o >>= 1) {
        c += __shfl_xor((int)c, o, 64);
        l = max(l, __shfl_xor(l, o, 64));
    }
    if ((threadIdx.x & 63) == 0) ws[threadIdx.x >> 6] = c, wl[threadIdx.x >> 6] = l;
    __syncthreads();
    if (threadIdx.x == 0) {
        cnt[blockIdx.x] = ws[0] + ws[1] + ws[2] + ws[3];
        last_kept[blockIdx.x] = max(max(wl[0], wl[1]), max(wl[2], wl[3]));
    }
}

__global__ __launch_bounds__(256) void mark_compact_kernel(const uint8_t *t, int64_t n, const uint32_t *qflag,
                                                           const int64_t *qoff, int n_q, const int64_t *tile_off,
                                                           const int64_t *last_kept, const uint64_t *ax, const uint32_t *ay,
                                                           uint64_t *ox, uint32_t *oy, uint32_t *ohb, uint32_t *ox32) {
    __shared__ uint32_t rc[64];
    __shared__ uint32_t nk[64];
    __shared__ uint32_t lx[64];
    __shared__ uint16_t kb[256];
    const int64_t t0 = (int64_t)blockIdx.x * 4096;
    const int lane = threadIdx.x & 63, w = threadIdx.x >> 6;
    kb[threadIdx.x] = (uint16_t)keep_bits16(t, n, qflag, qoff, n_q, t0 + threadIdx.x * 16);
    __syncthreads();
    bool m[16];
#pragma unroll
    for (int j = 0; j < 16; j++) {
        const int r = j * 256 + threadIdx.x;
        m[j] = (kb[r >> 4] >> (r & 15)) & 1;
        const uint64_t b = __ballot(m[j]);
        if (lane == 0) rc[j * 4 + w] = (uint32_t)__popcll(b);
    }
    __syncthreads();
    uint32_t v = 0, inc = 0;
    if (w == 0) nk[lane] = rc[lane];
    if (w == 0) {
        v = rc[lane];
        inc = v;
        for (int d = 1; d < 64; d <<= 1) {
            const uint32_t o = (uint32_t)__shfl_up((int)inc, d, 64);
            if (lane >= d) inc += o;
        }
    }
    __syncthreads();
    if (w == 0) rc[lane] = inc - v;
    __syncthreads();
    const int64_t base = tile_off[blockIdx.x];
    uint32_t xh[16];
#pragma unroll
    for (int j = 0; j < 16; j++) {
        const uint64_t b = __ballot(m[j]);
        xh[j] = 0;
        if (m[j]) {
            const int64_t e = t0 + j * 256 + threadIdx.x;
            const int64_t o = base + rc[j * 4 + w] + __popcll(b & ((1ull << lane) - 1));
            const uint64_t xv = ax[e];
            xh[j] = (uint32_t)(xv >> 32);
            ox[o] = xv;
            ox32[o] = (uint32_t)xv;
            oy[o] = ay[e];
        }
        if (b && lane == 63 - __clzll((long long)b)) lx[j * 4 + w] = xh[j];
    }
    __syncthreads();
#pragma unroll
    for (int j = 0; j < 16; j++) {
        const uint64_t b = __ballot(m[j]);
        const uint64_t below = b & ((1ull << lane) - 1);
        const int src = below ? 63 - __clzll((long long)below) : lane;
        const uint32_t xp = (uint32_t)__shfl((int)xh[j], src, 64);
        if (m[j]) {
            bool hd;
            if (below) {
                hd = xp != xh[j];
            } else {
                int c = j * 4 + w - 1;
                while (c >= 0 && nk[c] == 0) --c;
                if (c >= 0) {
                    hd = lx[c] != xh[j];
                } else {
                    int64_t tt = (int64_t)blockIdx.x - 1;
                    while (tt >= 0 && last_kept[tt] < 0) --tt;
                    hd = tt < 0 || (uint32_t)(ax[last_kept[tt]] >> 32) != xh[j];
                }
            }
            if (hd) {
                const int64_t o = base + rc[j * 4 + w] + __popcll(below);
                atomicOr(ohb + (o >> 5), 1u << (o & 31));
            }
        }
    }
}

__global__ void chain_query_kernel(const uint64_t *ckey, int64_t n, const int64_t *a_off, int n_q, uint32_t *cq) {
    const int64_t c = (int64_t)blockIdx.x * blockDim.x + threadIdx.x;
    if (c < n) cq[c] = (uint32_t)upper_idx(a_off, n_q, (int64_t)ckey[c]);
}

__global__ void count_per_query_kernel(const uint32_t *cq, int64_t n, int n_q, int64_t *q_first) {
    const int64_t p = (int64_t)blockIdx.x * blockDim.x + threadIdx.x;
    if (p > n) return;
    const int64_t qp = p == 0 ? -1 : (int64_t)cq[p - 1];
    const int64_t qc = p == n ? (int64_t)n_q : (int64_t)cq[p];
    for (int64_t q = qp + 1; q <= qc; q++) q_first[q] = p;
}

struct Groups {
    DevBuf g_start;
    DevBuf qfirst;
    int64_t G = 0;
};

struct WorkList {
    DevBuf order;
    DevBuf zlists;
    int64_t n_work = 0, largest = 0;
};

struct DpArgs {
    int max_dist, max_dist_inner, bw, max_chn_skip, cap_rmq_size;
    float pen_gap, pen_skip;
    int min_cnt;
};

struct ZOrder {
    DevBuf idx, cnt;
};

struct Backtrack {
    DevBuf ids, u, first, n_chains;
};

static int derive_heads(hymet_ctx *ctx, AnchorSet &A) {
    const int64_t n = A.n;
    if (!A.has_hb) {
        HY_HIP(A.hb.alloc(head_bits_bytes(n), ctx->stream));
        LAUNCH1(head_bits_x_kernel, n, A.ax.as<uint64_t>(), n, A.hb.as<uint64_t>());
        A.has_hb = true;
    }
    if (!A.has_x32) {
        HY_HIP(A.ax32.alloc(4 * (size_t)n, ctx->stream));
        LAUNCH1(x_low_kernel, n, A.ax.as<uint64_t>(), n, A.ax32.as<uint32_t>());
        A.has_x32 = true;
    }
    return HYMET_OK;
}

static int build_groups(hymet_ctx *ctx, const AnchorSet &A, int n_q, Groups &Gr) {
    const int64_t n = A.n, ntile = cdiv(n, kGTile);
    DevBuf tcnt, toff;
    HY_HIP(tcnt.alloc(4 * (size_t)(ntile + 1), ctx->stream));
    HY_HIP(toff.alloc(8 * (size_t)(ntile + 1), ctx->stream));
    hipLaunchKernelGGL(group_heads_count_kernel, dim3((unsigned)ntile), dim3(256), 0, ctx->stream, A.hb.as<uint32_t>(), n,
                       A.d_off.as<int64_t>(), n_q, tcnt.as<uint32_t>());
    HY_CHECK_LAUNCH("group_heads_count_kernel");
    int rc = exclusive_scan_u32_i64(ctx, tcnt.as<uint32_t>(), toff.as<int64_t>(), ntile, &Gr.G);
    if (rc) return rc;
    HY_HIP(Gr.g_start.alloc(8 * (size_t)(Gr.G + 1), ctx->stream));
    HY_HIP(Gr.qfirst.alloc((size_t)Gr.G, ctx->stream));
    hipLaunchKernelGGL(group_heads_write_kernel, dim3((unsigned)ntile), dim3(256), 0, ctx->stream, A.hb.as<uint32_t>(), n,
                       A.d_off.as<int64_t>(), n_q, toff.as<int64_t>(), Gr.g_start.as<int64_t>(), Gr.qfirst.as<uint8_t>(), Gr.G);
    HY_CHECK_LAUNCH("group_heads_write_kernel");
    return HYMET_OK;
}

static int build_work_list(hymet_ctx *ctx, const Groups &Gr, int min_cnt, WorkList &W) {
    const int64_t G = Gr.G;
    DevBuf skey, sidx, swork, skey2, sidx2, wpos;
    for (DevBuf *b : {&skey, &sidx, &swork, &skey2, &sidx2}) HY_HIP(b->alloc(4 * (size_t)G, ctx->stream));
    HY_HIP(W.zlists.alloc(32, ctx->stream));
    LAUNCH1(group_size_kernel, std::max<int64_t>(G, 8), Gr.g_start.as<int64_t>(), (int32_t)G, min_cnt, skey.as<uint32_t>(),
            sidx.as<uint32_t>(), swork.as<uint32_t>(), (uint8_t *)nullptr, W.zlists.as<int32_t>());
    int rc = scan_flags(ctx, swork.as<uint32_t>(), G, wpos, &W.n_work);
    if (rc) return rc;
    uint32_t *kp = skey.as<uint32_t>(), *ka = skey2.as<uint32_t>(), *vp = sidx.as<uint32_t>(), *va = sidx2.as<uint32_t>();
    rc = sort_pairs(ctx, kp, ka, vp, va, G, 0, 16, "radix_sort_groups");
    if (rc) return rc;
    LAUNCH1(max_group_kernel, 1, Gr.g_start.as<int64_t>(), (const int32_t *)vp, (int32_t)G, mb_dev(ctx, kMbGmax));
    HY_HIP(hipStreamSynchronize(ctx->stream));
    W.largest = mb_read(ctx, kMbGmax);
    HY_ARG(W.largest < (1ll << 24) - 1, "chaining: an anchor group exceeds 2^24 anchors");
    W.order.swap(vp == sidx.as<uint32_t>() ? sidx : sidx2);
    return HYMET_OK;
}

static int chain_dp(hymet_ctx *ctx, const DpArgs &a, const AnchorSet &A, const Groups &Gr, const WorkList &W, DevBuf &f,
                    DevBuf &p) {
    HY_HIP(f.alloc(4 * (size_t)A.n, ctx->stream));
    HY_HIP(p.alloc(4 * (size_t)A.n, ctx->stream));
    int32_t *stamp = nullptr;
    HY_HIP(stamp_scratch(ctx, A.n, &stamp));
    LAUNCH1(nonwork_fp_kernel, Gr.G, Gr.g_start.as<int64_t>(), (int32_t)Gr.G, a.min_cnt, f.as<int32_t>(), p.as<int32_t>());
    return launch_chain(ctx, A.ax32.as<int32_t>(), A.ay.as<uint32_t>(), A.span, Gr.g_start.as<int64_t>(), Gr.qfirst.as<uint8_t>(),
                        W.order.as<int32_t>(), (int32_t)W.n_work, f.as<int32_t>(), p.as<int32_t>(), stamp, a.max_dist,
                        a.max_dist_inner, a.bw, a.max_chn_skip, a.cap_rmq_size, a.pen_gap, a.pen_skip, A.n, Gr.G);
}

static int z_order(hymet_ctx *ctx, int min_sc, const DevBuf &f, int64_t n, const Groups &Gr, const WorkList &W, ZOrder &Z) {
    const int64_t G = Gr.G;
    DevBuf zkey, z_runs, run_start, merge_list, mergeu_list, mid_list, big_list, big_off;
    HY_HIP(zkey.alloc(8 * (size_t)n, ctx->stream));
    HY_HIP(Z.idx.alloc(4 * (size_t)n, ctx->stream));
    HY_HIP(Z.cnt.alloc(4 * (size_t)G, ctx->stream));
    HY_HIP(z_runs.alloc(4 * (size_t)G, ctx->stream));
    HY_HIP(run_start.alloc(4 * (size_t)G * kZRuns, ctx->stream));
    HY_HIP(merge_list.alloc(4 * (size_t)G, ctx->stream));
    const int zm_lds = (int)env_int("HYMET_ZM_LDS", kZmLds, 0, kZmLds);
    const int zm_unit = (int)env_int("HYMET_ZM_UNIT", kZmUnit, 1, INT32_MAX);
    const int max_runs = (int)env_int("HYMET_Z_RUNS", kZRuns, 1, kZRuns);
    HY_HIP(mergeu_list.alloc(8 * (size_t)(n / zm_unit + G + 16), ctx->stream));
    HY_HIP(mid_list.alloc(4 * (size_t)G, ctx->stream));
    HY_HIP(big_list.alloc(4 * (size_t)G, ctx->stream));
    HY_HIP(big_off.alloc(8 * (size_t)G, ctx->stream));
    ProfScope _ps(ctx, "mm_z_order", 16.0 * (double)n);
    ZParams P{f.as<int32_t>(), Gr.g_start.as<int64_t>(), W.order.as<int32_t>(), (int32_t)G, min_sc,
              max_runs, zm_lds, zm_unit, zkey.as<uint64_t>(), Z.idx.as<int32_t>(), Z.cnt.as<int32_t>(), z_runs.as<int32_t>(),
              run_start.as<int32_t>(), W.zlists.as<int32_t>(), merge_list.as<int32_t>(), mergeu_list.as<int64_t>(),
              mid_list.as<int32_t>(), big_list.as<int32_t>(),
              big_off.as<int64_t>(), mb_dev(ctx, kMbZBig)};
    hipLaunchKernelGGL(zsplit_kernel, dim3(1), dim3(64), 0, ctx->stream, P);
    HY_CHECK_LAUNCH("zsplit_kernel");
    const int64_t nwb = std::min<int64_t>(cdiv(G, 4), (int64_t)ctx->n_cu * 8);
    hipLaunchKernelGGL(zorder_wave_kernel, dim3((unsigned)std::max<int64_t>(nwb, 1)), dim3(256), 0, ctx->stream, P);
    HY_CHECK_LAUNCH("zorder_wave_kernel");
    LAUNCH1(zorder_lane_kernel, G, P);
    const int64_t nb = std::min<int64_t>(G, (int64_t)ctx->n_cu * 8);
    hipLaunchKernelGGL(zmerge_kernel, dim3((unsigned)nb), dim3(256), 0, ctx->stream, P);
    HY_CHECK_LAUNCH("zmerge_kernel");
    hipLaunchKernelGGL(zsort_block_kernel, dim3((unsigned)nb), dim3(256), 0, ctx->stream, P);
    HY_CHECK_LAUNCH("zsort_block_kernel");
    HY_HIP(hipStreamSynchronize(ctx->stream));
    const int64_t n_big = mb_read(ctx, kMbZBig), nz_big = mb_read(ctx, kMbZBigTotal);
    if (n_big == 0) return HYMET_OK;
    DevBuf bcnt;
    HY_HIP(bcnt.alloc(4 * (size_t)(n_big + 1), ctx->stream));
    LAUNCH1(zbig_count_kernel, n_big, P, (int32_t)n_big, bcnt.as<uint32_t>());
    int64_t nz_scan = 0;
    int rc = exclusive_scan_u32_i64(ctx, bcnt.as<uint32_t>(), big_off.as<int64_t>(), n_big, &nz_scan);
    if (rc) return rc;
    if (nz_scan != nz_big) return hymet::fail(HYMET_E_INTERNAL, "hymet_mm_map: z list count mismatch");
    DevBuf sk, sk2, sv, sv2;
    HY_HIP(sk.alloc(8 * (size_t)nz_big, ctx->stream));
    HY_HIP(sk2.alloc(8 * (size_t)nz_big, ctx->stream));
    HY_HIP(sv.alloc(4 * (size_t)nz_big, ctx->stream));
    HY_HIP(sv2.alloc(4 * (size_t)nz_big, ctx->stream));
    hipLaunchKernelGGL(zbig_gather_kernel, dim3((unsigned)n_big), dim3(256), 0, ctx->stream, P, sk.as<uint64_t>(),
                       sv.as<uint32_t>());
    HY_CHECK_LAUNCH("zbig_gather_kernel");
    uint64_t *kp = sk.as<uint64_t>(), *ka = sk2.as<uint64_t>();
    uint32_t *vp = sv.as<uint32_t>(), *va = sv2.as<uint32_t>();
    rc = sort_pairs(ctx, kp, ka, vp, va, nz_big, 0, 32 + bits_for(n_big), "radix_sort_z_big");
    if (rc) return rc;
    hipLaunchKernelGGL(zbig_scatter_kernel, dim3((unsigned)n_big), dim3(256), 0, ctx->stream, P, (const uint32_t *)vp);
    HY_CHECK_LAUNCH("zbig_scatter_kernel");
    return HYMET_OK;
}

static int backtrack(hymet_ctx *ctx, const hymet_mm_opt *opt, int bw, int64_t n, const Groups &Gr, const WorkList &W,
                     const DevBuf &f, const DevBuf &p, DevBuf &t, const ZOrder &Z, Backtrack &B) {
    HY_HIP(B.ids.alloc(4 * (size_t)n, ctx->stream));
    HY_HIP(B.u.alloc(8 * (size_t)n, ctx->stream));
    HY_HIP(B.first.alloc(8 * (size_t)n, ctx->stream));
    HY_HIP(B.n_chains.alloc(4 * (size_t)Gr.G, ctx->stream));
    return launch_backtrack(ctx, Gr.g_start.as<int64_t>(), f.as<int32_t>(), p.as<int32_t>(), t.as<uint8_t>(), Z.cnt.as<int32_t>(),
                            Z.idx.as<int32_t>(), (int32_t)Gr.G, W.order.as<int32_t>(), (int32_t)W.n_work, opt->min_cnt,
                            opt->min_chain_score, bw, B.ids.as<int32_t>(), B.u.as<uint64_t>(), B.first.as<int64_t>(),
                            B.n_chains.as<int32_t>(), n);
}

static int chain_list(hymet_ctx *ctx, const AnchorSet &A, int n_q, const Groups &Gr, const Backtrack &B, ChainSet &C,
                      DevBuf &cfirst) {
    const int64_t G = Gr.G;
    DevBuf cpos;
    int64_t NC = 0;
    int rc = scan_flags(ctx, (const uint32_t *)B.n_chains.p, G, cpos, &NC);
    if (rc) return rc;
    C.n_chain = NC;
    DevBuf ckey, cu, cf;
    HY_HIP(ckey.alloc(8 * (size_t)(NC + 1), ctx->stream));
    HY_HIP(cu.alloc(8 * (size_t)(NC + 1), ctx->stream));
    HY_HIP(cf.alloc(8 * (size_t)(NC + 1), ctx->stream));
    LAUNCH1(chain_list_kernel, G, Gr.g_start.as<int64_t>(), B.n_chains.as<int32_t>(), cpos.as<int64_t>(), (int32_t)G,
            B.u.as<uint64_t>(), B.first.as<int64_t>(), B.ids.as<int32_t>(), ckey.as<uint64_t>(), cu.as<uint64_t>(),
            cf.as<int64_t>());
    DevBuf perm, perm2, ckeyb;
    HY_HIP(perm.alloc(4 * (size_t)(NC + 1), ctx->stream));
    HY_HIP(perm2.alloc(4 * (size_t)(NC + 1), ctx->stream));
    HY_HIP(ckeyb.alloc(8 * (size_t)(NC + 1), ctx->stream));
    LAUNCH1(iota_u32_kernel, NC, perm.as<uint32_t>(), NC);
    uint64_t *ck = ckey.as<uint64_t>(), *cka = ckeyb.as<uint64_t>();
    uint32_t *pp = perm.as<uint32_t>(), *ppa = perm2.as<uint32_t>();
    rc = sort_pairs(ctx, ck, cka, pp, ppa, NC, 0, bits_for(A.n), "radix_sort_chains");
    if (rc) return rc;
    HY_HIP(C.cu.alloc(8 * (size_t)(NC + 1), ctx->stream));
    HY_HIP(cfirst.alloc(8 * (size_t)(NC + 1), ctx->stream));
    LAUNCH1(gather_kernel<uint64_t>, NC, cu.as<uint64_t>(), pp, C.cu.as<uint64_t>(), NC);
    LAUNCH1(gather_kernel<int64_t>, NC, cf.as<int64_t>(), pp, cfirst.as<int64_t>(), NC);
    HY_HIP(C.cq.alloc(4 * (size_t)(NC + 1), ctx->stream));
    LAUNCH1(chain_query_kernel, NC, ck, NC, A.d_off.as<int64_t>(), n_q, C.cq.as<uint32_t>());
    HY_HIP(C.d_qc.alloc(8 * (size_t)(n_q + 1), ctx->stream));
    hipLaunchKernelGGL(count_per_query_kernel, dim3((unsigned)cdiv(NC + 1, 256)), dim3(256), 0, ctx->stream,
                       C.cq.as<uint32_t>(), NC, n_q, C.d_qc.as<int64_t>());
    HY_CHECK_LAUNCH("count_per_query_kernel");
    return HYMET_OK;
}

static int chain_layout(hymet_ctx *ctx, const AnchorSet &A, int n_q, const DevBuf &chain_ids, const DevBuf &cfirst,
                        ChainSet &C, LeanJoin *lj, DevBuf &t) {
    const int64_t NC = C.n_chain;
    DevBuf ccnt, ccnt2;
    HY_HIP(ccnt.alloc(4 * (size_t)(NC + 1), ctx->stream));
    if (lj) {
        HY_HIP(lj->flag.alloc(4 * (size_t)n_q, ctx->stream));
        LAUNCH1(rechain_flag_kernel, n_q, A.ay.as<uint32_t>(), chain_ids.as<int32_t>(), C.cu.as<uint64_t>(),
                cfirst.as<int64_t>(), C.d_qc.as<int64_t>(), lj->qlen, n_q, lj->rescue_size, lj->rescue_ratio,
                lj->flag.as<uint32_t>());
        HY_HIP(ccnt2.alloc(4 * (size_t)(NC + 1), ctx->stream));
    }
    LAUNCH1(chain_cnt_kernel, NC, C.cu.as<uint64_t>(), C.cq.as<uint32_t>(), lj ? lj->flag.as<uint32_t>() : nullptr, NC,
            ccnt.as<uint32_t>(), lj ? ccnt2.as<uint32_t>() : nullptr);
    int64_t NB = 0;
    int rc = scan_flags(ctx, ccnt.as<uint32_t>(), NC, C.cboff, &NB);
    if (rc) return rc;
    C.n_anchor = NB;
    HY_HIP(C.d_qb.alloc(8 * (size_t)(n_q + 1), ctx->stream));
    LAUNCH1(chain_qb_kernel, n_q + 1, C.d_qc.as<int64_t>(), C.cboff.as<int64_t>(), NC, NB, n_q, C.d_qb.as<int64_t>());
    if (lj) {
        DevBuf boff2;
        rc = scan_flags(ctx, ccnt2.as<uint32_t>(), NC, boff2, &lj->n2);
        if (rc) return rc;
        lj->mark.swap(t);
        HY_HIP(lj->qb2.alloc(8 * (size_t)(n_q + 1), ctx->stream));
        LAUNCH1(chain_qb_kernel, n_q + 1, C.d_qc.as<int64_t>(), boff2.as<int64_t>(), NC, lj->n2, n_q, lj->qb2.as<int64_t>());
    }
    return HYMET_OK;
}

}

int chain_set(hymet_ctx *ctx, const hymet_mm_opt *opt, float pen_gap, float pen_skip, int bw, AnchorSet &A, int n_q,
              ChainSet &C, LeanJoin *lj) {
    const int64_t n = A.n;
    HY_ARG(n >= 0 && n < INT32_MAX, "chain_set: an anchor set of 2^31 anchors or more (32-bit chain links)");
    C.ax = A.ax.as<uint64_t>(), C.ay = A.ay.as<uint32_t>(), C.span = A.span;
    if (n == 0) {
        HY_HIP(C.d_qc.alloc(8 * (size_t)(n_q + 1), ctx->stream));
        HY_HIP(C.d_qb.alloc(8 * (size_t)(n_q + 1), ctx->stream));
        HY_HIP(hipMemsetAsync(C.d_qc.p, 0, 8 * (size_t)(n_q + 1), ctx->stream));
        HY_HIP(hipMemsetAsync(C.d_qb.p, 0, 8 * (size_t)(n_q + 1), ctx->stream));
        return HYMET_OK;
    }
    int rc = derive_heads(ctx, A);
    if (rc) return rc;
    Groups Gr;
    rc = build_groups(ctx, A, n_q, Gr);
    if (rc) return rc;
    DevBuf t;
    HY_HIP(t.alloc((size_t)n + 16, ctx->stream));
    HY_HIP(hipMemsetAsync(t.p, 0, (size_t)n + 16, ctx->stream));
    WorkList W;
    rc = build_work_list(ctx, Gr, opt->min_cnt, W);
    if (rc) return rc;
    if (env_flag("HYMET_CHAIN_STATS"))
        fprintf(stderr, "[chain] bw %d anchors %lld groups %lld work %lld largest %lld\n", bw, (long long)n, (long long)Gr.G,
                (long long)W.n_work, (long long)W.largest);
    DevBuf f, p;
    rc = chain_dp(ctx, DpArgs{opt->max_gap, opt->rmq_inner_dist, bw, opt->max_chain_skip, opt->rmq_size_cap, pen_gap, pen_skip,
                              opt->min_cnt}, A, Gr, W, f, p);
    if (rc) return rc;
    ZOrder Z;
    rc = z_order(ctx, opt->min_chain_score, f, n, Gr, W, Z);
    if (rc) return rc;
    Backtrack B;
    rc = backtrack(ctx, opt, bw, n, Gr, W, f, p, t, Z, B);
    if (rc) return rc;
    DevBuf cfirst;
    rc = chain_list(ctx, A, n_q, Gr, B, C, cfirst);
    if (rc) return rc;
    rc = chain_layout(ctx, A, n_q, B.ids, cfirst, C, lj, t);
    if (rc) return rc;
    C.ids.swap(B.ids);
    C.cfirst.swap(cfirst);
    return HYMET_OK;
}

static int compact_marked(hymet_ctx *ctx, const AnchorSet &S1, const uint8_t *mark, const uint32_t *flag, int n_q,
                          int64_t expect, AnchorSet &S2) {
    hipStream_t st = ctx->stream;
    const int64_t n1 = S1.n, nt = cdiv(n1, 4096);
    DevBuf tcnt, toff, tlast;
    HY_HIP(tcnt.alloc(4 * (size_t)(nt + 1), st));
    HY_HIP(toff.alloc(8 * (size_t)(nt + 1), st));
    HY_HIP(tlast.alloc(8 * (size_t)(nt + 1), st));
    hipLaunchKernelGGL(mark_count_kernel, dim3((unsigned)nt), dim3(256), 0, st, mark, n1, flag,
                       S1.d_off.as<int64_t>(), n_q, tcnt.as<uint32_t>(), tlast.as<int64_t>());
    HY_CHECK_LAUNCH("mark_count_kernel");
    int64_t A2 = 0;
    int rc = exclusive_scan_u32_i64(ctx, tcnt.as<uint32_t>(), toff.as<int64_t>(), nt, &A2);
    if (rc) return rc;
    if (expect >= 0 && A2 != expect) return hymet::fail(HYMET_E_INTERNAL, "hymet_mm_map: long-join anchor count mismatch");
    HY_HIP(S2.ax.alloc(8 * (size_t)(A2 + 1), st));
    HY_HIP(S2.ay.alloc(4 * (size_t)(A2 + 1), st));
    HY_HIP(S2.hb.alloc(head_bits_bytes(A2), st));
    HY_HIP(S2.ax32.alloc(4 * (size_t)(A2 + 1), st));
    HY_HIP(hipMemsetAsync(S2.hb.p, 0, head_bits_bytes(A2), st));
    hipLaunchKernelGGL(mark_compact_kernel, dim3((unsigned)nt), dim3(256), 0, st, mark, n1, flag,
                       S1.d_off.as<int64_t>(), n_q, toff.as<int64_t>(), tlast.as<int64_t>(), S1.ax.as<uint64_t>(),
                       S1.ay.as<uint32_t>(), S2.ax.as<uint64_t>(), S2.ay.as<uint32_t>(), S2.hb.as<uint32_t>(),
                       S2.ax32.as<uint32_t>());
    HY_CHECK_LAUNCH("mark_compact_kernel");
    S2.n = A2;
    S2.span = S1.span;
    S2.has_hb = S2.has_x32 = true;
    return HYMET_OK;
}

int marked_anchor_set(hymet_ctx *ctx, const AnchorSet &S1, const LeanJoin &lj, const uint32_t *flag, int n_q, int64_t A2,
                      AnchorSet &S2) {
    if (A2 != lj.n2) return hymet::fail(HYMET_E_INTERNAL, "hymet_mm_map: long-join anchor count mismatch");
    return compact_marked(ctx, S1, lj.mark.as<uint8_t>(), flag, n_q, A2, S2);
}

static int narrow_y(const uint64_t *h_y, int64_t n, std::vector<uint32_t> &y32, int *span, const char *what) {
    y32.resize((size_t)n);
    for (int64_t i = 0; i < n; i++) {
        if ((h_y[i] >> 32) != (h_y[0] >> 32)) return hymet::fail(HYMET_E_ARG, what);
        y32[(size_t)i] = (uint32_t)h_y[i];
    }
    *span = n > 0 ? (int)(h_y[0] >> 32 & 0xff) : 0;
    return HYMET_OK;
}

}
}

using namespace hymet;
using namespace hymet::mm;

extern "C" int hymet_mm_chain_dp(hymet_ctx *ctx, const uint64_t *h_x, const uint64_t *h_y, int64_t n, int max_dist,
                                 int max_dist_inner, int bw, int max_chn_skip, int cap_rmq_size, float pen_gap,
                                 float pen_skip, int32_t *h_f, int64_t *h_p) {
    HY_ARG(ctx && (n == 0 || (h_x && h_y && h_f && h_p)), "hymet_mm_chain_dp: null argument");
    HY_ARG(n >= 0 && n < INT32_MAX, "hymet_mm_chain_dp: n out of range");
    if (n == 0) return HYMET_OK;
    HY_HIP(hipSetDevice(ctx->device));
    hipStream_t st = ctx->stream;
    AnchorSet A;
    const int64_t h_off[2] = {0, n};
    A.n = n;
    std::vector<uint32_t> y32;
    int rc = narrow_y(h_y, n, y32, &A.span, "hymet_mm_chain_dp: the anchors' y values carry different spans");
    if (rc) return rc;
    HY_HIP(A.ax.alloc(8 * (size_t)n, st));
    HY_HIP(A.ay.alloc(4 * (size_t)n, st));
    HY_HIP(A.d_off.alloc(sizeof h_off, st));
    HY_HIP(hipMemcpyAsync(A.ax.p, h_x, 8 * (size_t)n, hipMemcpyHostToDevice, st));
    HY_HIP(hipMemcpyAsync(A.ay.p, y32.data(), 4 * (size_t)n, hipMemcpyHostToDevice, st));
    HY_HIP(hipMemcpyAsync(A.d_off.p, h_off, sizeof h_off, hipMemcpyHostToDevice, st));
    rc = derive_heads(ctx, A);
    if (rc) return rc;
    Groups Gr;
    rc = build_groups(ctx, A, 1, Gr);
    if (rc) return rc;
    WorkList W;
    rc = build_work_list(ctx, Gr, 1, W);
    if (rc) return rc;
    DevBuf f, p;
    rc = chain_dp(ctx, DpArgs{max_dist, max_dist_inner, bw, max_chn_skip, cap_rmq_size, pen_gap, pen_skip, 1}, A, Gr, W, f, p);
    if (rc) return rc;
    HY_HIP(hipMemcpyAsync(h_f, f.p, 4 * (size_t)n, hipMemcpyDeviceToHost, st));
    std::vector<int32_t> p32((size_t)n);
    HY_HIP(hipMemcpyAsync(p32.data(), p.p, 4 * (size_t)n, hipMemcpyDeviceToHost, st));
    HY_HIP(hipStreamSynchronize(st));
    for (int64_t i = 0; i < n; i++) h_p[i] = p32[(size_t)i];
    return HYMET_OK;
}

namespace {
__global__ __launch_bounds__(256) void stamp_nonzero_kernel(const int32_t *t, int64_t n, unsigned long long *out) {
    unsigned long long c = 0;
    for (int64_t i = (int64_t)blockIdx.x * 256 + threadIdx.x; i < n; i += (int64_t)gridDim.x * 256) c += t[i] != 0;
    for (int o = 32; o > 0; o >>= 1) c += __shfl_xor(c, o, 64);
    if ((threadIdx.x & 63) == 0 && c) atomicAdd(out, c);
}
}

extern "C" int hymet_mm_stamp_scratch(hymet_ctx *ctx, int64_t *capacity, int64_t *nonzero) {
    HY_ARG(ctx && capacity && nonzero, "hymet_mm_stamp_scratch: null argument");
    HY_HIP(hipSetDevice(ctx->device));
    hipStream_t st = ctx->stream;
    HY_HIP(hipStreamSynchronize(st));
    *capacity = ctx->stamp_cap;
    *nonzero = 0;
    if (ctx->stamp_cap == 0) return HYMET_OK;
    DevBuf cnt;
    HY_HIP(cnt.alloc(8, st));
    HY_HIP(hipMemsetAsync(cnt.p, 0, 8, st));
    const int64_t nb = std::min<int64_t>(cdiv(ctx->stamp_cap, 256), (int64_t)ctx->n_cu * 8);
    hipLaunchKernelGGL(stamp_nonzero_kernel, dim3((unsigned)nb), dim3(256), 0, st, (const int32_t *)ctx->stamp, ctx->stamp_cap,
                       cnt.as<unsigned long long>());
    HY_CHECK_LAUNCH("stamp_nonzero_kernel");
    unsigned long long h = 0;
    HY_HIP(hipMemcpyAsync(&h, cnt.p, 8, hipMemcpyDeviceToHost, st));
    HY_HIP(hipStreamSynchronize(st));
    *nonzero = (int64_t)h;
    return HYMET_OK;
}

extern "C" int hymet_mm_mark_compact(hymet_ctx *ctx, const uint64_t *h_x, const uint64_t *h_y, const int32_t *h_mark, int64_t n,
                                     const int64_t *h_qoff, const uint32_t *h_qflag, int32_t n_q, uint64_t *h_ox,
                                     uint64_t *h_oy, uint32_t *h_ohb, int64_t *n_kept) {
    HY_ARG(ctx && h_x && h_y && h_mark && h_qoff && h_qflag && h_ox && h_oy && h_ohb && n_kept,
           "hymet_mm_mark_compact: null argument");
    HY_ARG(n > 0 && n < INT32_MAX && n_q > 0, "hymet_mm_mark_compact: n or n_q out of range");
    HY_ARG(h_qoff[0] == 0 && h_qoff[n_q] == n, "hymet_mm_mark_compact: query offsets do not span the anchors");
    for (int32_t q = 0; q < n_q; q++) HY_ARG(h_qoff[q] <= h_qoff[q + 1], "hymet_mm_mark_compact: query offsets not rising");
    HY_HIP(hipSetDevice(ctx->device));
    hipStream_t st = ctx->stream;
    AnchorSet S1, S2;
    S1.n = n;
    std::vector<uint32_t> y32;
    int rc = narrow_y(h_y, n, y32, &S1.span, "hymet_mm_mark_compact: the anchors' y values carry different spans");
    if (rc) return rc;
    DevBuf mark, flag;
    HY_HIP(S1.ax.alloc(8 * (size_t)n, st));
    HY_HIP(S1.ay.alloc(4 * (size_t)n, st));
    HY_HIP(S1.d_off.alloc(8 * (size_t)(n_q + 1), st));
    std::vector<uint8_t> m8((size_t)n);
    for (int64_t i = 0; i < n; i++) m8[(size_t)i] = h_mark[i] == 2 ? 2 : (h_mark[i] != 0);
    HY_HIP(mark.alloc((size_t)n + 16, st));
    HY_HIP(flag.alloc(4 * (size_t)n_q, st));
    HY_HIP(hipMemcpyAsync(S1.ax.p, h_x, 8 * (size_t)n, hipMemcpyHostToDevice, st));
    HY_HIP(hipMemcpyAsync(S1.ay.p, y32.data(), 4 * (size_t)n, hipMemcpyHostToDevice, st));
    HY_HIP(hipMemcpyAsync(S1.d_off.p, h_qoff, 8 * (size_t)(n_q + 1), hipMemcpyHostToDevice, st));
    HY_HIP(hipMemcpyAsync(mark.p, m8.data(), (size_t)n, hipMemcpyHostToDevice, st));
    HY_HIP(hipMemcpyAsync(flag.p, h_qflag, 4 * (size_t)n_q, hipMemcpyHostToDevice, st));
    rc = compact_marked(ctx, S1, mark.as<uint8_t>(), flag.as<uint32_t>(), n_q, -1, S2);
    if (rc) {
        HY_HIP(hipStreamSynchronize(st));
        return rc;
    }
    const int64_t m = S2.n;
    std::vector<uint32_t> oy32((size_t)m);
    if (m > 0) {
        HY_HIP(hipMemcpyAsync(h_ox, S2.ax.p, 8 * (size_t)m, hipMemcpyDeviceToHost, st));
        HY_HIP(hipMemcpyAsync(oy32.data(), S2.ay.p, 4 * (size_t)m, hipMemcpyDeviceToHost, st));
        HY_HIP(hipMemcpyAsync(h_ohb, S2.hb.p, 4 * (size_t)((m + 31) / 32), hipMemcpyDeviceToHost, st));
    }
    HY_HIP(hipStreamSynchronize(st));
    for (int64_t i = 0; i < m; i++) h_oy[i] = (h_y[0] >> 32) << 32 | oy32[(size_t)i];
    *n_kept = m;
    return HYMET_OK;
}
```

hymet_amd/csrc/mm_common.hpp:

```cpp
#pragma once
#include "common.hpp"

#include <cstring>
#include <vector>

namespace hymet {
namespace mm {

constexpr uint64_t kMax64 = ~0ull;
constexpr int kChunk = 512;

__host__ __device__ __forceinline__ uint64_t hash64m(uint64_t key, uint64_t mask) {
    key = (~key + (key << 21)) & mask;
    key = key ^ key >> 24;
    key = ((key + (key << 3)) + (key << 8)) & mask;
    key = key ^ key >> 14;
    key = ((key + (key << 2)) + (key << 4)) & mask;
    key = key ^ key >> 28;
    key = (key + (key << 31)) & mask;
    return key;
}
__host__ __device__ __forceinline__ uint64_t hash64(uint64_t key) {
    key = (~key + (key << 21));
    key = key ^ key >> 24;
    key = ((key + (key << 3)) + (key << 8));
    key = key ^ key >> 14;
    key = ((key + (key << 2)) + (key << 4));
    key = key ^ key >> 28;
    key = (key + (key << 31));
    return key;
}

struct MiniWord {
    uint64_t bits;
    uint32_t base;
    uint32_t pad;
};
__device__ __forceinline__ int32_t mini_word_idx(const MiniWord &e, int32_t x) {
    const uint64_t below = (1ull << (x & 63)) - 1;
    return (e.bits >> (x & 63) & 1) ? (int32_t)(e.base + (uint32_t)__popcll(e.bits & below)) : -1;
}

struct DevBuf {
    void *p = nullptr;
    size_t n = 0, cls = 0;
    hipStream_t st = nullptr;
    DevBuf() = default;
    DevBuf(const DevBuf &) = delete;
    DevBuf &operator=(const DevBuf &) = delete;
    ~DevBuf() { release(); }
    hipError_t alloc(size_t bytes, hipStream_t stream) {
        release();
        n = bytes;
        st = stream;
        return scratch_alloc(bytes == 0 ? 16 : bytes, stream, &p, &cls);
    }
    void release() {
        if (p) scratch_free(p, st, cls);
        p = nullptr;
        n = 0;
    }
    template <typename T>
    T *as() const { return reinterpret_cast<T *>(p); }
    void swap(DevBuf &o) {
        std::swap(p, o.p);
        std::swap(n, o.n);
        std::swap(cls, o.cls);
        std::swap(st, o.st);
    }
};

struct SketchParams {
    const uint32_t *w2b;
    const uint32_t *wm;
    const int64_t *seq_start;
    const int64_t *seq_len;
    const int64_t *chunk_off;
    int64_t n_chunks;
    int n_seq;
    int k;
    int warm;
    int rid_mode;
    uint32_t *counts;
    const int64_t *out_off;
    uint64_t *out_x;
    uint64_t *out_y;
    int slot_cap;
    uint32_t *overflow;
};

int launch_sketch(hymet_ctx *ctx, int w, bool write, const SketchParams &P);

int exclusive_scan_u32_i64(hymet_ctx *ctx, const uint32_t *in, int64_t *out, int64_t n, int64_t *total);
int scan_u32_i64(hymet_ctx *ctx, const uint32_t *in, int64_t *out, int64_t n, DevBuf &part, int64_t *mail = nullptr);
enum : int { kMbScan = 0, kMbGmax = 1, kMbZBig = 2, kMbZBigTotal = 3, kMbFlag = 4, kMbRegBig = 5, kMbRegBig2 = 6, kMbQClass = 8,
             kMbGroups = 20, kMbGClass = 24 };
enum : int { kCtrQClass = 0, kCtrGroups = 16, kCtrGClass = 24, kCtrScan = 40, kCtrMaxScan = 41, kCtrRegBig = 42, kCtrRegBig2 = 44 };
enum : int { kCtrUfErr = 48 };
enum : int { kCtrGreedyErr = 49 };

__device__ __forceinline__ void publish_counters(int32_t *cnt, int n, int64_t *mail) {
    __shared__ bool last;
    __syncthreads();
    if (threadIdx.x == 0) {
        __threadfence();
        last = atomicAdd(reinterpret_cast<uint32_t *>(cnt + n), 1u) == gridDim.x - 1;
    }
    __syncthreads();
    if (!last) return;
    __threadfence();
    if ((int)threadIdx.x < n) mail[threadIdx.x] = atomicExch(cnt + threadIdx.x, 0);
    if (threadIdx.x == 0) atomicExch(cnt + n, 0);
}

inline int bits_for(int64_t v) {
    int b = 0;
    while (b < 63 && (1ll << b) <= v) b++;
    return b < 1 ? 1 : b;
}
int scan_u32(hymet_ctx *ctx, const uint32_t *in, uint32_t *out, int64_t n, DevBuf &part, int64_t *mail = nullptr);
int scan_u64(hymet_ctx *ctx, const uint64_t *in, uint64_t *out, int64_t n, DevBuf &part, int64_t *mail = nullptr);
int inclusive_max_scan_i32(hymet_ctx *ctx, const int32_t *in, int32_t *out, int64_t n, DevBuf &part);

inline int anchor_word_ybits(int rb, int pb, int64_t max_qlen) {
    int yb = 1;
    while (yb <= 32 && (1ll << yb) <= max_qlen) yb++;
    return yb <= 32 && 1 + rb + pb + yb <= 63 ? yb : 0;
}
int grouped_anchor_sort(hymet_ctx *ctx, const uint64_t *word, int64_t n, const int64_t *d_qoff, int n_q, int rb, int pb,
                        int64_t max_qlen, uint64_t *oword, uint64_t *ax, uint32_t *ay, uint32_t *hb,
                        uint32_t *ax32, unsigned long long *d_stats = nullptr);
inline size_t head_bits_bytes(int64_t n) { return 8 * (size_t)((n + 63) / 64 + 1); }

int sketch_sequences(hymet_ctx *ctx, const uint32_t *d_2b, const uint32_t *d_mask, const int64_t *h_starts,
                     const int64_t *h_lens, int n_seq, int w, int k, int rid_mode, DevBuf &d_x, DevBuf &d_y,
                     int64_t *n_out, DevBuf *d_seq_off);

}
}

struct hymet_mm_index {
    int w = 10, k = 15, n_seq = 0;
    int64_t n_pos = 0;
    int64_t n_buckets = 0;
    uint32_t *d_koff = nullptr;
    uint64_t *d_pos = nullptr;
    uint32_t *d_hash = nullptr;
    int64_t *d_len = nullptr;
    std::vector<int64_t> h_len;
    int device = 0;
};

struct hymet_paf_acc {
    int device = 0;
    int64_t n = 0, cap = 0;
    hymet::mm::DevBuf regs;
    hymet::mm::DevBuf q;
    hymet::mm::DevBuf part;
    hymet::mm::DevBuf rl;
    hymet::mm::DevBuf t;
};
```

hymet_amd/csrc/mm_regs.hip:

```cpp
#include "mm_common.hpp"

#include <cstdio>
#include <cstdlib>

namespace hymet {
namespace mm {
namespace {

__device__ __forceinline__ uint32_t wang32(uint32_t key) {
    key += ~(key << 15);
    key ^= (key >> 10);
    key += (key << 3);
    key ^= (key >> 6);
    key += ~(key << 11);
    key ^= (key >> 16);
    return key;
}

struct U128 {
    uint64_t x, y;
};
__device__ __forceinline__ bool lt128(const U128 &a, const U128 &b) { return a.x < b.x || (a.x == b.x && a.y < b.y); }

template <typename T, typename Less>
__device__ void heap_sort(T *a, int64_t n, Less less) {
    auto sift = [&](int64_t i, int64_t m) {
        for (;;) {
            int64_t l = 2 * i + 1, r = l + 1, b = i;
            if (l < m && less(a[b], a[l])) b = l;
            if (r < m && less(a[b], a[r])) b = r;
            if (b == i) return;
            T t = a[b];
            a[b] = a[i];
            a[i] = t;
            i = b;
        }
    };
    for (int64_t i = n / 2 - 1; i >= 0; --i) sift(i, n);
    for (int64_t e = n - 1; e > 0; --e) {
        T t = a[0];
        a[0] = a[e];
        a[e] = t;
        sift(0, e);
    }
}

struct RegParams {
    const uint64_t *ax;
    const uint32_t *ay;
    int span;
    const int32_t *ids;
    const int64_t *cfirst;
    const uint64_t *cu;
    const int64_t *cboff;
    const int64_t *qc;
    const int64_t *qb;
    const uint64_t *mini_pos;
    const int64_t *mp_off;
    const int64_t *qlen;
    const uint32_t *name_hash;
    const int32_t *rep_len;
    const int64_t *ref_len;
    int n_q;
    int seed, k;
    float mask_level, pri_ratio;
    int mask_len, best_n, max_gap, min_chain_score;
    U128 *z;
    hymet_mm_reg *regs;
    int32_t *w;
    uint64_t *cov;
    int32_t *tmp;
    int32_t *n_regs;
    const int32_t *c_mlen, *c_blen, *c_st, *c_last, *c_fv;
    const uint64_t *q_sumk;
    const uint32_t *skip_q;
    int wave_min;
    int lds_max;
    unsigned long long *prof;
    int prim_regs;
};

__device__ void set_coor(hymet_mm_reg *r, int32_t qlen, uint64_t x0, uint32_t y0, uint64_t x1, uint32_t y1, int32_t q_span,
                         int32_t mlen, int32_t blen) {
    r->rev = (int32_t)(x0 >> 63);
    r->rid = (int32_t)(x0 << 1 >> 33);
    r->rs = (int32_t)x0 + 1 > q_span ? (int32_t)x0 + 1 - q_span : 0;
    r->re = (int32_t)x1 + 1;
    if (!r->rev) {
        r->qs = (int32_t)y0 + 1 - q_span;
        r->qe = (int32_t)y1 + 1;
    } else {
        r->qs = qlen - ((int32_t)y1 + 1);
        r->qe = qlen - ((int32_t)y0 + 1 - q_span);
    }
    r->mlen = mlen;
    r->blen = blen;
}

struct AnchorStatParams {
    const uint64_t *ax, *cu;
    const uint32_t *ay;
    int span;
    const int32_t *ids;
    const int64_t *cfirst;
    const int64_t *cboff, *qb, *qlen, *mp_off;
    const uint64_t *mini_pos;
    int64_t NB, NC;
    int n_q;
    const uint32_t *cq;
    int32_t *c_mlen, *c_blen, *c_st, *c_last;
    const MiniWord *mtab;
    const int64_t *qbase;
    const uint32_t *skip_q;
};

__device__ __forceinline__ int32_t mini_idx_at(const AnchorStatParams &P, int64_t q, int qlen, uint64_t ax, uint32_t ay) {
    int32_t x = (int32_t)ay;
    if (ax >> 63) x = qlen - 1 - (int32_t)ay + P.span - 1;
    return (x >= 0 && x < qlen) ? mini_word_idx(P.mtab[(P.qbase[q] + x) >> 6], x) : -1;
}

#ifndef HYMET_STAT_ITEMS
#define HYMET_STAT_ITEMS 2
#endif
constexpr int kStatItems = HYMET_STAT_ITEMS;
constexpr int kStatSpan = 256 * kStatItems;

__global__ void block_chain_kernel(const int64_t *cboff, int64_t NC, int64_t NB, int32_t *blk_c0) {
    const int64_t c = (int64_t)blockIdx.x * blockDim.x + threadIdx.x;
    if (c >= NC) return;
    const int64_t s = cboff[c], e = c + 1 < NC ? cboff[c + 1] : NB;
    for (int64_t b = (s + kStatSpan - 1) / kStatSpan; b * kStatSpan < e; ++b) blk_c0[b] = (int32_t)c;
}

__global__ __launch_bounds__(256) void chain_stats_flat_kernel(AnchorStatParams P, const int32_t *blk_c0, int32_t *c_fv) {
    constexpr int K = kStatItems;
    __shared__ int32_t s_st[kStatSpan + 1];
    const int64_t b0 = (int64_t)blockIdx.x * kStatSpan;
    const int64_t cb0 = blk_c0[blockIdx.x];
    for (int i = threadIdx.x; i <= kStatSpan; i += blockDim.x) {
        const int64_t cc = cb0 + i;
        s_st[i] = cc < P.NC ? (int32_t)min(P.cboff[cc] - b0, (int64_t)kStatSpan) : kStatSpan;
    }
    __syncthreads();
    const int lane = threadIdx.x & 63;
    int64_t c[K], q[K], f0[K];
    bool act[K];
    int32_t cnt[K], j[K], qlen[K], cur[K];
    uint64_t x[K];
    uint32_t y[K];
    const bool one_chain = s_st[1] >= kStatSpan;
    int32_t t_dm = 0, t_db = 0, t_fv = INT32_MAX;
    int64_t qb[K];
    if (one_chain) {
        const int64_t qq = (int64_t)P.cq[cb0];
        const int32_t cn = (int32_t)P.cu[cb0];
        const int64_t cbs = P.cboff[cb0], f00 = P.cfirst[cb0] + cn - 1;
        const int ql = (int)P.qlen[qq];
        const int64_t qbb = P.qbase[qq];
        const bool sk = P.skip_q && P.skip_q[qq];
#pragma unroll
        for (int k = 0; k < K; k++) {
            const int64_t b = b0 + 256 * k + threadIdx.x;
            c[k] = b < P.NB ? cb0 : -1;
            q[k] = qq, cnt[k] = cn, f0[k] = f00, qlen[k] = ql, qb[k] = qbb;
            act[k] = b < P.NB && !sk;
            j[k] = act[k] ? (int32_t)(b - cbs) : 0;
        }
    } else {
#pragma unroll
        for (int k = 0; k < K; k++) {
            const int r = 256 * k + (int)threadIdx.x;
            const int64_t b = b0 + r;
            c[k] = -1;
            if (b < P.NB) {
                int lo = 0, hi = kStatSpan;
                while (lo < hi) {
                    const int mid = (lo + hi + 1) >> 1;
                    if (s_st[mid] <= r) lo = mid;
                    else hi = mid - 1;
                }
                c[k] = cb0 + lo;
                if (lo == kStatSpan) {
                    int64_t l2 = c[k], h2 = P.NC - 1;
                    while (l2 < h2) {
                        const int64_t mid = (l2 + h2 + 1) >> 1;
                        if (P.cboff[mid] <= b) l2 = mid;
                        else h2 = mid - 1;
                    }
                    c[k] = l2;
                }
            }
        }
#pragma unroll
        for (int k = 0; k < K; k++) q[k] = (int64_t)P.cq[c[k] >= 0 ? c[k] : 0];
#pragma unroll
        for (int k = 0; k < K; k++) {
            const int64_t cc = c[k] >= 0 ? c[k] : 0;
            cnt[k] = (int32_t)P.cu[cc];
            const int64_t cb = P.cboff[cc];
            f0[k] = P.cfirst[cc] + cnt[k] - 1;
            j[k] = (int32_t)(b0 + 256 * k + threadIdx.x - cb);
            qlen[k] = (int)P.qlen[q[k]];
            qb[k] = P.qbase[q[k]];
        }
#pragma unroll
        for (int k = 0; k < K; k++) {
            act[k] = c[k] >= 0;
            if (P.skip_q) act[k] = act[k] && !P.skip_q[q[k]];
            if (!act[k]) j[k] = 0;
        }
    }
#pragma unroll
    for (int k = 0; k < K; k++) {
        const int64_t a = P.ids[f0[k] - j[k]];
        x[k] = P.ax[a], y[k] = P.ay[a];
    }
#pragma unroll
    for (int k = 0; k < K; k++) {
        int32_t xq = (int32_t)y[k];
        if (x[k] >> 63) xq = qlen[k] - 1 - (int32_t)y[k] + P.span - 1;
        const bool inq = xq >= 0 && xq < qlen[k];
        const int32_t xc = inq ? xq : 0;
        const int32_t v = mini_word_idx(P.mtab[(qb[k] + xc) >> 6], xc);
        cur[k] = act[k] && inq ? v : -1;
    }
#pragma unroll
    for (int k = 0; k < K; k++) {
        const int32_t ci = (int32_t)c[k];
        const int32_t cprev = __shfl_up(ci, 1, 64), cnext = __shfl_down(ci, 1, 64);
        uint64_t xp = __shfl_up(x[k], 1, 64), xn = __shfl_down(x[k], 1, 64);
        uint32_t yp = __shfl_up(y[k], 1, 64), yn = __shfl_down(y[k], 1, 64);
        const int32_t cur_p = __shfl_up(cur[k], 1, 64), cur_n = __shfl_down(cur[k], 1, 64);
        int dm = 0, db = 0, fv = INT32_MAX;
        if (act[k]) {
            const bool rev = x[k] >> 63;
            const bool own_p = lane > 0 && cprev == ci, own_n = lane < 63 && cnext == ci;
            if (j[k] > 0 && !own_p) {
                const int64_t a = P.ids[f0[k] - j[k] + 1];
                xp = P.ax[a], yp = P.ay[a];
            }
            if (rev && j[k] + 1 < cnt[k] && !own_n) {
                const int64_t a = P.ids[f0[k] - j[k] - 1];
                xn = P.ax[a], yn = P.ay[a];
            }
            const int32_t span = P.span;
            if (j[k] == 0) {
                dm = db = span;
            } else {
                const int32_t tl = (int32_t)x[k] - (int32_t)xp;
                const int32_t ql = (int32_t)y[k] - (int32_t)yp;
                db = tl > ql ? tl : ql;
                dm = tl > span && ql > span ? span : tl < ql ? tl : ql;
            }
            const int32_t kk = rev ? cnt[k] - 1 - j[k] : j[k];
            fv = cnt[k];
            if (kk >= 1) {
                const int32_t prev = rev ? (own_n ? cur_n : mini_idx_at(P, q[k], qlen[k], xn, yn))
                                         : (own_p ? cur_p : mini_idx_at(P, q[k], qlen[k], xp, yp));
                if (cur[k] < 0 || cur[k] <= prev) fv = kk;
            }
            if (kk == 0) P.c_st[c[k]] = cur[k];
            if (kk == cnt[k] - 1) P.c_last[c[k]] = cur[k];
        }
        if (one_chain) {
            t_dm += dm, t_db += db, t_fv = min(t_fv, fv);
            continue;
        }
        const int32_t cr = act[k] ? ci : -1;
#pragma unroll
        for (int d = 1; d < 64; d <<= 1) {
            const int32_t co = __shfl_up(cr, d, 64);
            const int dmo = __shfl_up(dm, d, 64), dbo = __shfl_up(db, d, 64), fvo = __shfl_up(fv, d, 64);
            if (lane >= d && co == cr) dm += dmo, db += dbo, fv = min(fv, fvo);
        }
        const int32_t cn = __shfl_down(cr, 1, 64);
        if (act[k] && (lane == 63 || cn != cr)) {
            atomicAdd(P.c_mlen + c[k], dm);
            atomicAdd(P.c_blen + c[k], db);
            atomicMin(c_fv + c[k], fv);
        }
    }
    if (one_chain) {
        __shared__ int32_t r_dm[4], r_db[4], r_fv[4];
#pragma unroll
        for (int o = 32; o > 0; o >>= 1) {
            t_dm += __shfl_xor(t_dm, o, 64);
            t_db += __shfl_xor(t_db, o, 64);
            t_fv = min(t_fv, __shfl_xor(t_fv, o, 64));
        }
        const int w = threadIdx.x >> 6;
        if (lane == 0) r_dm[w] = t_dm, r_db[w] = t_db, r_fv[w] = t_fv;
        __syncthreads();
        if (threadIdx.x == 0 && act[0]) {
            atomicAdd(P.c_mlen + cb0, r_dm[0] + r_dm[1] + r_dm[2] + r_dm[3]);
            atomicAdd(P.c_blen + cb0, r_db[0] + r_db[1] + r_db[2] + r_db[3]);
            atomicMin(c_fv + cb0, min(min(r_fv[0], r_fv[1]), min(r_fv[2], r_fv[3])));
        }
    }
}

__global__ __launch_bounds__(64) void query_sumk_kernel(const uint64_t *mini_pos, const int64_t *mp_off, int n_q,
                                                        unsigned long long *sumk) {
    for (int q = blockIdx.x; q < n_q; q += gridDim.x) {
        unsigned long long sk = 0;
        const int64_t m1 = mp_off[q + 1];
        for (int64_t m = mp_off[q] + threadIdx.x; m < m1; m += 256) {
            uint64_t v[4];
#pragma unroll
            for (int j = 0; j < 4; j++) v[j] = m + 64 * j < m1 ? mini_pos[m + 64 * j] : 0;
#pragma unroll
            for (int j = 0; j < 4; j++) sk += v[j] >> 32 & 0xff;
        }
        for (int o = 32; o > 0; o >>= 1) sk += __shfl_xor(sk, o, 64);
        if (threadIdx.x == 0) sumk[q] = sk;
    }
}

constexpr int kRegWave = 16;
constexpr int kRegSmall = 256;
constexpr int kRegEntryBytes = 16 + 16 + 4 * 3 + 8;
constexpr int kRegScrStride = 2 * ((kRegEntryBytes + 15) & ~15) - 16;
static_assert(kRegScrStride % 16 == 0 && kRegScrStride >= 2 * kRegEntryBytes, "regions scratch stride");

__device__ __forceinline__ bool wave_query(const RegParams &P, int q, int n, int32_t qlen) {
    return n > P.wave_min && qlen != 0 && !(P.skip_q && P.skip_q[q]);
}

__device__ void regions_seq(const RegParams &P, int q) {
    const int64_t c0 = P.qc[q], c1 = P.qc[q + 1];
    int n = (int)(c1 - c0);
    const int32_t qlen = (int32_t)P.qlen[q];
    if (n == 0 || qlen == 0 || (P.skip_q && P.skip_q[q])) {
        P.n_regs[q] = 0;
        return;
    }
    const int64_t b0 = P.qb[q];
    U128 *z = P.z + c0;
    hymet_mm_reg *r = P.regs + c0;
    uint32_t hash = P.name_hash[q];
    hash ^= wang32((uint32_t)qlen) + wang32((uint32_t)P.seed);
    hash = wang32(hash);
    for (int i = 0; i < n; ++i) {
        const int64_t k = P.cboff[c0 + i] - b0;
        const uint64_t u = P.cu[c0 + i];
        const int64_t a = P.ids[P.cfirst[c0 + i] + (int32_t)u - 1];
        const uint32_t h = (uint32_t)hash64((hash64(P.ax[a]) + hash64((uint64_t)P.span << 32 | P.ay[a])) ^ hash);
        z[i].x = u ^ h;
        z[i].y = (uint64_t)k << 32 | (uint32_t)i;
    }
    heap_sort(z, n, [](const U128 &a, const U128 &b) { return lt128(a, b); });
    for (int i = 0; i < n >> 1; ++i) {
        U128 t = z[i];
        z[i] = z[n - 1 - i];
        z[n - 1 - i] = t;
    }
    for (int i = 0; i < n; ++i) {
        hymet_mm_reg *ri = &r[i];
        ri->id = i;
        ri->parent = -1;
        ri->score = (int32_t)(z[i].x >> 32);
        ri->hash = (uint32_t)z[i].x;
        const int64_t c = c0 + (uint32_t)z[i].y;
        ri->cnt = (int32_t)P.cu[c];
        ri->as = (int32_t)(z[i].y >> 32);
        ri->div = -1.0f;
        ri->subsc = 0;
        ri->n_sub = 0;
        ri->strand_retained = 0;
        ri->mapq = 0;
        ri->pad = (int32_t)(c - c0);
        const int64_t a0 = P.ids[P.cfirst[c] + ri->cnt - 1], a1 = P.ids[P.cfirst[c]];
        set_coor(ri, qlen, P.ax[a0], P.ay[a0], P.ax[a1], P.ay[a1], P.span, P.c_mlen[c], P.c_blen[c]);
    }
    {
        int32_t *w = P.w + c0;
        uint64_t *cov = P.cov + c0;
        for (int i = 0; i < n; ++i) r[i].id = i;
        int i, j, k;
        w[0] = 0, r[0].parent = 0;
        for (i = 1, k = 1; i < n; ++i) {
            hymet_mm_reg *ri = &r[i];
            const int si = ri->qs, ei = ri->qe;
            int n_cov = 0, uncov_len = 0;
            for (j = 0; j < k; ++j) {
                const hymet_mm_reg *rp = &r[w[j]];
                int sj = rp->qs, ej = rp->qe;
                if (ej <= si || sj >= ei) continue;
                if (sj < si) sj = si;
                if (ej > ei) ej = ei;
                cov[n_cov++] = (uint64_t)(uint32_t)sj << 32 | (uint32_t)ej;
            }
            if (n_cov == 0) goto set_parent_test;
            {
                int x = si;
                heap_sort(cov, n_cov, [](uint64_t a, uint64_t b) { return a < b; });
                for (int jj = 0; jj < n_cov; ++jj) {
                    if ((int)(cov[jj] >> 32) > x) uncov_len += (int)(cov[jj] >> 32) - x;
                    x = (int32_t)cov[jj] > x ? (int32_t)cov[jj] : x;
                }
                if (ei > x) uncov_len += ei - x;
            }
            for (j = 0; j < k; ++j) {
                hymet_mm_reg *rp = &r[w[j]];
                const int sj = rp->qs, ej = rp->qe;
                if (ej <= si || sj >= ei) continue;
                const int mn = ej - sj < ei - si ? ej - sj : ei - si;
                const int mx = ej - sj > ei - si ? ej - sj : ei - si;
                const int ol = si < sj ? (ei < sj ? 0 : ei < ej ? ei - sj : ej - sj) : (ej < si ? 0 : ej < ei ? ej - si : ei - si);
                if (__fsub_rn(__fdiv_rn((float)ol, (float)mn), __fdiv_rn((float)uncov_len, (float)mx)) > P.mask_level &&
                    uncov_len <= P.mask_len) {
                    const int sci = ri->score;
                    ri->parent = rp->parent;
                    rp->subsc = rp->subsc > sci ? rp->subsc : sci;
                    if (ri->cnt >= rp->cnt) ++rp->n_sub;
                    break;
                }
            }
        set_parent_test:
            if (j == k) w[k++] = i, ri->parent = i, ri->n_sub = 0;
        }
    }
    {
        const int min_diff = P.k * 2;
        const int min_strand_sc = (int)(P.max_gap * 0.8);
        int i, k, n_2nd = 0;
        for (i = k = 0; i < n; ++i) {
            const int p = r[i].parent;
            if (p == i) {
                r[k++] = r[i];
            } else if (((float)r[i].score >= __fmul_rn((float)r[p].score, P.pri_ratio) || r[i].score + min_diff >= r[p].score) &&
                       n_2nd < P.best_n) {
                if (!(r[i].qs == r[p].qs && r[i].qe == r[p].qe && r[i].rid == r[p].rid && r[i].rs == r[p].rs && r[i].re == r[p].re))
                    r[k++] = r[i], ++n_2nd;
            } else if (n_2nd < P.best_n && r[i].score > min_strand_sc && r[i].rev != r[p].rev) {
                r[i].strand_retained = 1;
                r[k++] = r[i], ++n_2nd;
            }
        }
        if (k != n) {
            int32_t *tmp = P.tmp + c0;
            int max_id = -1;
// ... 314 lines not shown
                    }
                    const uint64_t mh = __ballot(hit);
                    if (mh) jfound = __ffsll((unsigned long long)mh) - 1;
                }
            } else {
                int ncov = 0;
                for (int jb = 0; jb < k; jb += 64) {
                    const int j = jb + lane;
                    int sj = ps, ej = pe;
                    if (j >= R) {
                        sj = 0, ej = 0;
                        if (j < k) {
                            const int4 o = slot[wl[j]];
                            sj = o.x, ej = o.y;
                        }
                    }
                    const bool ov = j < k && !(ej <= si || sj >= ei);
                    const uint64_t mov = __ballot(ov);
                    if (ov) covb[ncov + __popcll(mov & ((1ull << lane) - 1))] = (uint64_t)(uint32_t)max(sj, si) << 32 | (uint32_t)min(ej, ei);
                    ncov += __popcll(mov);
                }
                wsync();
                if (ncov > 0) {
                    int uncov = 0, carry = si;
                    if (ncov == 1) {
                        const uint64_t kv = covb[0];
                        const int s_ = (int)(kv >> 32), e_ = (int)(uint32_t)kv;
                        uncov = s_ > si ? s_ - si : 0;
                        carry = max(si, e_);
                    } else if (ncov <= 64) {
                        const uint64_t kv = wave_sort_u64(lane < ncov ? covb[lane] : ~0ull);
                        const int s_ = (int)(kv >> 32), e_ = lane < ncov ? (int)(uint32_t)kv : INT32_MIN;
                        const int x = wave_excl_max(e_, si);
                        uncov = wave_sum_i(lane < ncov && s_ > x ? s_ - x : 0);
                        carry = max(si, wave_max_i(e_));
                    } else {
                        int mm = 64;
                        while (mm < ncov) mm <<= 1;
                        for (int t = ncov + lane; t < mm; t += 64) covb[t] = ~0ull;
                        wsync();
                        lds_sort_asc_u64(covb, mm);
                        for (int tb = 0; tb < ncov; tb += 64) {
                            const int t = tb + lane;
                            const uint64_t kv = t < ncov ? covb[t] : ~0ull;
                            const int s_ = (int)(kv >> 32), e_ = t < ncov ? (int)(uint32_t)kv : INT32_MIN;
                            const int x = wave_excl_max(e_, carry);
                            uncov += wave_sum_i(t < ncov && s_ > x ? s_ - x : 0);
                            carry = max(carry, wave_max_i(e_));
                        }
                    }
                    if (ei > carry) uncov += ei - carry;
                    for (int jb = 0; jb < k && jfound < 0; jb += 64) {
                        const int j = jb + lane;
                        bool hit = false;
                        int sj = ps, ej = pe;
                        bool in = true;
                        if (j >= R) {
                            in = j < k;
                            if (in) {
                                const int4 o = slot[wl[j]];
                                sj = o.x, ej = o.y;
                            }
                        }
                        if (in && !(ej <= si || sj >= ei)) {
                            const int mn = ej - sj < ei - si ? ej - sj : ei - si;
                            const int mx = ej - sj > ei - si ? ej - sj : ei - si;
                            const int ol = si < sj ? (ei < sj ? 0 : ei < ej ? ei - sj : ej - sj)
                                                   : (ej < si ? 0 : ej < ei ? ej - si : ei - si);
                            hit = __fsub_rn(__fdiv_rn((float)ol, (float)mn), __fdiv_rn((float)uncov, (float)mx)) > P.mask_level &&
                                  uncov <= P.mask_len;
                        }
                        const uint64_t mh = __ballot(hit);
                        if (mh) jfound = jb + __ffsll((unsigned long long)mh) - 1;
                    }
                }
            }
            if (jfound >= 0) {
                if (jfound < R) {
                    const int p = __builtin_amdgcn_readlane(pw, jfound);
                    if (lane == 0) r[i].parent = p;
                    if (lane == jfound) {
                        psb = psb > sci ? psb : sci;
                        if (cnti >= pc) ++pnb;
                    }
                } else {
                    const int p = wl[jfound];
                    if (lane == 0) {
                        r[i].parent = p;
                        psub[jfound] = psub[jfound] > sci ? psub[jfound] : sci;
                        if (cnti >= slot[p].w) ++pns[jfound];
                    }
                    wsync();
                }
            } else {
                if (k < R) {
                    if (lane == k) ps = si, pe = ei, pc = cnti, pw = i, psb = 0, pnb = 0;
                } else {
                    if (lane == 0) wl[k] = i, psub[k] = 0, pns[k] = 0;
                }
                if (lane == 0) r[i].parent = i;
                ++k;
                if (k > R) wsync();
            }
        }
        if (lane < k && lane < R) {
            r[pw].subsc = psb;
            r[pw].n_sub = pnb;
        }
        for (int j = R + lane; j < k; j += 64) {
            r[wl[j]].subsc = psub[j];
            r[wl[j]].n_sub = pns[j];
        }
    }
    __threadfence_block();
    wsync();
    RPROF(3);
    int nk = 0;
    {
        const int min_diff = P.k * 2;
        const int min_strand_sc = (int)(P.max_gap * 0.8);
        int n_2nd = 0;
        int32_t *kept = wl;
        uint64_t *sflag = covb;
        for (int t = lane; t < (n + 63) / 64; t += 64) sflag[t] = 0;
        wsync();
        for (int base = 0; base < n; base += 64) {
            const int i = base + lane;
            const int pl = i < n ? r[i].parent : 0;
            uint64_t keepm = 0, strm = 0;
            const int cnt_chunk = min(64, n - base);
            for (int l = 0; l < cnt_chunk; ++l) {
                const int ii = base + l, p = __builtin_amdgcn_readlane(pl, l);
                bool keep = false, str = false;
                if (p == ii) {
                    keep = true;
                } else {
                    const int src = nk > p ? kept[p] : p;
                    const int4 mi = slot[ii], xi = aux[ii], mp = slot[src], xp = aux[src];
                    if (((float)mi.z >= __fmul_rn((float)mp.z, P.pri_ratio) || mi.z + min_diff >= mp.z) && n_2nd < P.best_n) {
                        if (!(mi.x == mp.x && mi.y == mp.y && (xi.x & 0x7fffffff) == (xp.x & 0x7fffffff) && xi.y == xp.y &&
                              xi.z == xp.z))
                            keep = true, ++n_2nd;
                    } else if (n_2nd < P.best_n && mi.z > min_strand_sc && ((uint32_t)xi.x >> 31) != ((uint32_t)xp.x >> 31)) {
                        keep = str = true, ++n_2nd;
                    }
                }
                if (keep) {
                    if (lane == 0) kept[nk] = ii;
                    keepm |= 1ull << l;
                    ++nk;
                }
                if (str) strm |= 1ull << l;
                wsync();
            }
            if (lane == 0) sflag[base >> 6] = strm;
            wsync();
        }
        if (nk != n) {
            for (int ob = 0; ob < nk; ob += 64) {
                const int o = ob + lane;
                hymet_mm_reg v;
                if (o < nk) {
                    const int src = kept[o];
                    v = r[src];
                    if (sflag[src >> 6] >> (src & 63) & 1) v.strand_retained = 1;
                }
                __threadfence_block();
                wsync();
                if (o < nk) r[o] = v;
                __threadfence_block();
                wsync();
            }
            int32_t *pos_of = psub;
            for (int j = lane; j < n; j += 64) pos_of[j] = -1;
            wsync();
            for (int o = lane; o < nk; o += 64) pos_of[kept[o]] = o;
            wsync();
            for (int o = lane; o < nk; o += 64) {
                const int par = r[o].parent;
                r[o].id = o;
                r[o].parent = par >= 0 && pos_of[par] >= 0 ? pos_of[par] : -1;
            }
        } else {
            for (int o = lane; o < n; o += 64)
                if (sflag[o >> 6] >> (o & 63) & 1) r[o].strand_retained = 1;
        }
        n = nk;
    }
    __threadfence_block();
    wsync();
    RPROF(4);
    {
        const int64_t m0 = P.mp_off[q];
        const int32_t nm = (int32_t)(P.mp_off[q + 1] - m0);
        if (nm > 0) {
            const uint64_t sum_k = P.q_sumk[q];
            const float avg_k = __fdiv_rn((float)sum_k, (float)nm);
            for (int i = lane; i < n; i += 64) {
                hymet_mm_reg *ri = &r[i];
                float div = -1.0f;
                if (ri->cnt != 0) {
                    const int64_t c = c0 + ri->pad;
                    const int32_t st = P.c_st[c];
                    if (st >= 0) {
                        const int32_t fv = P.c_fv[c] < ri->cnt ? P.c_fv[c] : ri->cnt;
                        const int32_t n_match = fv;
                        const int32_t en = fv == ri->cnt ? P.c_last[c] : nm - 1;
                        const int32_t l_ref = (int32_t)P.ref_len[ri->rid];
                        int32_t n_tot = en - st + 1;
                        if ((float)ri->qs > avg_k && (float)ri->rs > avg_k) ++n_tot;
                        if ((float)(qlen - ri->qe) > avg_k && (float)(l_ref - ri->re) > avg_k) ++n_tot;
                        div = n_match >= n_tot ? 0.0f : (float)(1.0 - pow((double)n_match / n_tot, 1.0 / (double)avg_k));
                    }
                }
                ri->div = div;
            }
        }
    }
    __threadfence_block();
    wsync();
    RPROF(5);
    {
        int first_drop = n;
        for (int base = 0; base < n && first_drop == n; base += 64) {
            const int i = base + lane;
            bool drop = false;
            if (i < n && r[i].strand_retained) {
                const int p = r[i].parent;
                drop = !(r[i].div < __fmul_rn(r[p].div, 5.0f) || r[i].div < 0.01f);
            }
            const uint64_t md = __ballot(drop);
            if (md) first_drop = base + __ffsll((unsigned long long)md) - 1;
        }
        if (first_drop < n) {
            if (lane == 0) {
                int i, k = first_drop;
                for (i = first_drop + 1; i < n; ++i) {
                    const int p = r[i].parent;
                    if (!r[i].strand_retained || r[i].div < __fmul_rn(r[p].div, 5.0f) || r[i].div < 0.01f) r[k++] = r[i];
                }
                psub[0] = k;
            }
            __threadfence_block();
            wsync();
            n = psub[0];
        }
    }
    __threadfence_block();
    wsync();
    {
        const float q_coef = 40.0f;
        int64_t sum_sc = 0;
        for (int i = lane; i < n; i += 64)
            if (r[i].parent == r[i].id) sum_sc += r[i].score;
        sum_sc = wave_sum_l(sum_sc);
        const float uniq_ratio = __fdiv_rn((float)sum_sc, (float)(sum_sc + P.rep_len[q]));
        for (int i = lane; i < n; i += 64) {
            hymet_mm_reg *ri = &r[i];
            ri->pad = 0;
            if (ri->parent == ri->id) {
                const float pen_s1 = __fmul_rn(ri->score > 100 ? 1.0f : __fmul_rn(0.01f, (float)ri->score), uniq_ratio);
                float pen_cm = ri->cnt > 10 ? 1.0f : __fmul_rn(0.1f, (float)ri->cnt);
                pen_cm = pen_s1 < pen_cm ? pen_s1 : pen_cm;
                const int subsc = ri->subsc > P.min_chain_score ? ri->subsc : P.min_chain_score;
                const float x = __fdiv_rn((float)subsc, (float)ri->score);
                int mapq = (int)__fmul_rn(__fmul_rn(__fmul_rn(pen_cm, q_coef), __fsub_rn(1.0f, x)), logf((float)ri->score));
                mapq -= (int)__fadd_rn(__fmul_rn(4.343f, logf((float)(ri->n_sub + 1))), .499f);
                mapq = mapq > 0 ? mapq : 0;
                ri->mapq = mapq < 60 ? mapq : 60;
            } else
                ri->mapq = 0;
        }
    }
    RPROF(6);
    if (P.prof) {
        atomicAdd(P.prof + 6, lane == 0 ? 1ull : 0ull);
        atomicAdd(P.prof + 7, lane == 0 ? (unsigned long long)(c1 - c0) : 0ull);
    }
#undef RPROF
    if (lane == 0) P.n_regs[q] = n;
}

__global__ void chain_stats_init_kernel(int32_t *c_mlen, int32_t *c_blen, int32_t *c_fv, int64_t n) {
    const int64_t i = (int64_t)blockIdx.x * blockDim.x + threadIdx.x;
    if (i < n) c_mlen[i] = 0, c_blen[i] = 0, c_fv[i] = 0x7f7f7f7f;
}

}

int launch_regions(hymet_ctx *ctx, const uint64_t *ax, const uint32_t *ay, int span, const int32_t *ids, const int64_t *cfirst,
                   const uint64_t *cu, const int64_t *cboff,
                   const int64_t *qc, const int64_t *qb, const uint64_t *mini_pos, const int64_t *mp_off, const int64_t *qlen,
                   const uint32_t *name_hash, const int32_t *rep_len, const int64_t *ref_len, int n_q, const hymet_mm_opt *o,
                   int k, void *z, hymet_mm_reg *regs, int32_t *w, uint64_t *cov, int32_t *tmp, int32_t *n_regs,
                   int64_t NB, int64_t NC, int64_t NM, const uint32_t *cq,
                   const MiniWord *mtab, const int64_t *qbase, const uint32_t *skip_q, uint64_t *sumk, bool sumk_done) {
    if (n_q <= 0) return HYMET_OK;
    hipStream_t st = ctx->stream;
    DevBuf cst, blk;
    HY_HIP(cst.alloc(4 * 5 * (size_t)(NC + 1), st));
    int32_t *c_mlen = cst.as<int32_t>(), *c_blen = c_mlen + (NC + 1), *c_st = c_blen + (NC + 1), *c_last = c_st + (NC + 1),
            *c_fv = c_last + (NC + 1);
    {
        ProfScope _ps(ctx, "mm_chain_stats", (double)NB * (4.0 + 12.0 + 4.0) + (double)NM * 8.0);
        AnchorStatParams A{ax, cu, ay, span, ids, cfirst, cboff, qb, qlen, mp_off, mini_pos, NB, NC, n_q, cq,
                           c_mlen, c_blen, c_st, c_last, mtab, qbase, skip_q};
        if (NB > 0) {
            hipLaunchKernelGGL(chain_stats_init_kernel, dim3((unsigned)cdiv(NC + 1, 256)), dim3(256), 0, st, c_mlen, c_blen,
                               c_fv, NC + 1);
            HY_CHECK_LAUNCH("chain_stats_init_kernel");
            HY_HIP(blk.alloc(4 * (size_t)(cdiv(NB, kStatSpan) + 1), st));
            hipLaunchKernelGGL(block_chain_kernel, dim3((unsigned)cdiv(NC, 256)), dim3(256), 0, st, cboff, NC, NB,
                               blk.as<int32_t>());
            HY_CHECK_LAUNCH("block_chain_kernel");
            hipLaunchKernelGGL(chain_stats_flat_kernel, dim3((unsigned)cdiv(NB, kStatSpan)), dim3(256), 0, st, A,
                               (const int32_t *)blk.as<int32_t>(), c_fv);
            HY_CHECK_LAUNCH("chain_stats_flat_kernel");
        }
        if (!sumk_done) {
            const int nqb = n_q < ctx->n_cu * 64 ? n_q : ctx->n_cu * 64;
            hipLaunchKernelGGL(query_sumk_kernel, dim3((unsigned)nqb), dim3(64), 0, st, mini_pos, mp_off, n_q,
                               (unsigned long long *)sumk);
            HY_CHECK_LAUNCH("query_sumk_kernel");
        }
    }
    RegParams P{ax, ay, span, ids, cfirst, cu, cboff, qc, qb, mini_pos, mp_off, qlen, name_hash, rep_len, ref_len, n_q, o->seed, k,
                o->mask_level, o->pri_ratio, o->mask_len, o->best_n, o->max_gap, o->min_chain_score, (U128 *)z, regs, w, cov,
                tmp, n_regs, c_mlen, c_blen, c_st, c_last, c_fv, sumk, skip_q, kRegWave, kRegSmall, nullptr, 64};
    P.wave_min = (int)env_int("HYMET_REG_WAVE", P.wave_min, 0, INT32_MAX);
    P.lds_max = (int)env_int("HYMET_REG_LDS", P.lds_max, 32, kRegSmall);
    P.prim_regs = (int)env_int("HYMET_REG_PRIM", P.prim_regs, 0, 64);
    ProfScope _ps(ctx, "mm_regions", (double)NC * (8.0 + 8.0 + 4.0 * 5) + (double)n_q * 64.0);
    if (env_flag("HYMET_REG_STATS")) {
        std::vector<int64_t> hq(n_q + 1);
        HY_HIP(hipMemcpyAsync(hq.data(), qc, 8 * (size_t)(n_q + 1), hipMemcpyDeviceToHost, st));
        HY_HIP(hipStreamSynchronize(st));
        int64_t h[8] = {0}, mx = 0, tot = 0, big_tot = 0;
        for (int q = 0; q < n_q; q++) {
            const int64_t c = hq[q + 1] - hq[q];
            const int b = c <= 48 ? 0 : c <= 256 ? 1 : c <= 1024 ? 2 : c <= 2048 ? 3 : c <= 8192 ? 4 : 5;
            h[b]++, mx = c > mx ? c : mx, tot += c;
            if (c > 2048) big_tot += c;
        }
        fprintf(stderr, "[regions] n_q %d anchors %lld chains %lld max %lld | <=48 %lld <=256 %lld <=1k %lld <=2k %lld <=8k %lld >8k %lld (chains in >2k: %lld)\n",
                n_q, (long long)NB, (long long)tot, (long long)mx, (long long)h[0], (long long)h[1], (long long)h[2], (long long)h[3],
                (long long)h[4], (long long)h[5], (long long)big_tot);
    }
    if (env_flag("HYMET_REG_PROF")) {
        HY_HIP(hipMalloc((void **)&P.prof, 8 * 8));
        HY_HIP(hipMemsetAsync(P.prof, 0, 8 * 8, st));
    }
    DevBuf big, gscr;
    HY_HIP(big.alloc(4 * (size_t)n_q, st));
    HY_HIP(gscr.alloc((size_t)kRegScrStride * (size_t)(NC + 1), st));
    int32_t *n_big = ctx->dctr + kCtrRegBig;
    hipLaunchKernelGGL(regions_kernel, dim3((unsigned)cdiv(n_q, 64)), dim3(64), 0, st, P, big.as<int32_t>(), n_big);
    HY_CHECK_LAUNCH("regions_kernel");
    hipLaunchKernelGGL(regions_wave_kernel, dim3((unsigned)std::min<int64_t>(n_q, 12 * (int64_t)ctx->n_cu)), dim3(64),
                       (size_t)kRegSmall * kRegEntryBytes, st, P, (const int32_t *)big.as<int32_t>(), n_big,
                       mb_dev(ctx, kMbRegBig), gscr.as<unsigned char>());
    HY_CHECK_LAUNCH("regions_wave_kernel");
    if (P.prof) {
        unsigned long long h[8];
        HY_HIP(hipMemcpyAsync(h, P.prof, sizeof h, hipMemcpyDeviceToHost, st));
        HY_HIP(hipStreamSynchronize(st));
        fprintf(stderr, "[regprof] queries %llu chains %llu | Mcycles keys %.1f sort+fill %.1f parent %.1f select %.1f est %.1f filter+mapq %.1f\n",
                h[6], h[7], h[0] / 1e6, h[1] / 1e6, h[2] / 1e6, h[3] / 1e6, h[4] / 1e6, h[5] / 1e6);
        (void)hipFree(P.prof);
    }
    return HYMET_OK;
}

}
}
```

include/hymet_gpu.h:

```cpp
#ifndef HYMET_GPU_H
#define HYMET_GPU_H

#include <stdint.h>

#ifdef __cplusplus
extern "C" {
#endif

#define HYMET_OK 0
#define HYMET_E_HIP (-1)
#define HYMET_E_ARG (-2)
#define HYMET_E_CAPACITY (-3)
#define HYMET_E_INTERNAL (-4)

typedef struct hymet_ctx hymet_ctx;

int hymet_init(int device, hymet_ctx **out);
int hymet_destroy(hymet_ctx *ctx);
const char *hymet_last_error(void);
int hymet_set_stream(hymet_ctx *ctx, void *hip_stream);
int hymet_sync(hymet_ctx *ctx);
int hymet_version(void);
int hymet_prof_enable(hymet_ctx *ctx, int on);
int hymet_prof_reset(hymet_ctx *ctx);
int hymet_prof_query(hymet_ctx *ctx, const char *name, double *total_ms, int64_t *count, double *alg_bytes);
int hymet_prof_names(hymet_ctx *ctx, char *buf, int64_t cap);
int hymet_scratch_trim(hymet_ctx *ctx, int64_t *freed_bytes);
int hymet_scratch_cached(hymet_ctx *ctx, int64_t *bytes);
int hymet_scratch_reserve(hymet_ctx *ctx, int64_t bytes);
int hymet_set_oom_hook(void (*hook)(void *user), void *user);
int hymet_scratch_stats(hymet_ctx *ctx, int64_t *counts);
int hymet_copy_to_host(hymet_ctx *ctx, void *dst, const void *src, int64_t n, int threads);
int hymet_copy_to_device(hymet_ctx *ctx, void *dst, const void *src, int64_t n, int threads);

int hymet_pack(hymet_ctx *ctx, const uint8_t *d_ascii, int64_t n, int alphabet,
               uint32_t *d_2b, uint32_t *d_mask);

int hymet_fasta_index(const char *h_buf, int64_t n, int threads, int64_t cap, int64_t *n_rec, int64_t *h_name_off,
                      int32_t *h_name_len, int64_t *h_seq_off, int64_t *h_seq_end, int64_t *h_nbases);
int hymet_fasta_names(const char *h_buf, const int64_t *h_name_off, const int32_t *h_name_len, int64_t n, char *h_pool,
                      int64_t *h_pool_off);
int hymet_fasta_compact(hymet_ctx *ctx, const uint8_t *d_raw, int64_t raw_len, int64_t raw_base, const int64_t *h_seq_off,
                        const int64_t *h_seq_end, const int64_t *h_nbases, int64_t n_rec, uint8_t *d_pool,
                        int64_t pool_len, int64_t *d_pool_start);
int hymet_name_hash(hymet_ctx *ctx, const uint8_t *d_raw, const int64_t *d_name_off, const int32_t *d_name_len, int64_t n,
                    uint32_t *d_hash);

int64_t hymet_screen_table_slots(int64_t n_hashes);
int hymet_screen_table_build(hymet_ctx *ctx, const uint64_t *d_hashes, int64_t n_hashes,
                             uint64_t *d_table, int64_t n_slots, int64_t *d_scratch, int32_t *d_canon_of,
                             int key_bits);
int hymet_sort_pairs_u64(hymet_ctx *ctx, uint64_t *d_keys, uint32_t *d_vals, int64_t n, int begin_bit, int end_bit);

int hymet_scan_u32(hymet_ctx *ctx, const uint32_t *d_in, int64_t *d_out, int64_t n, int mode, int64_t *total);

typedef struct hymet_msh hymet_msh;
typedef struct {
    int32_t k, window_size, sketch_size;
    uint32_t seed;
    int32_t noncanonical, preserve_case, use64;
    int64_t n_refs, n_hashes, names_bytes, comments_bytes, alphabet_len;
} hymet_msh_info;
int hymet_msh_open(const char *path, hymet_msh **out);
int hymet_msh_info_get(const hymet_msh *m, hymet_msh_info *info);
int hymet_msh_copy(const hymet_msh *m, int threads, uint64_t *hashes, int64_t *offsets, int64_t *lengths,
                   char *names, char *comments, char *alphabet);
int hymet_msh_text_offsets(const hymet_msh *m, int64_t *name_start, int64_t *comment_start);
int hymet_msh_upload(hymet_ctx *ctx, const hymet_msh *m, int threads, uint64_t *pinned, uint64_t *d_hashes,
                     int n_chunks);
int hymet_msh_upload_range(hymet_ctx *ctx, const hymet_msh *m, int threads, uint64_t *pinned, uint64_t *d_hashes,
                           int n_chunks, int64_t lo_h, int64_t hi_h);
void hymet_msh_close(hymet_msh *m);
int hymet_screen_count(hymet_ctx *ctx, const uint32_t *d_2b, const uint32_t *d_mask,
                       int64_t n_bases, int64_t pos_begin, int64_t pos_end, int k, uint32_t seed,
                       int ndb, const uint64_t *const *h_d_tables, const int64_t *h_n_slots,
                       const uint64_t *const *h_d_hashes, const int64_t *h_n_hashes,
                       uint32_t *const *h_d_counts, uint64_t cand_thr, uint64_t *d_cand,
                       int64_t cand_cap, unsigned long long *d_cand_n,
                       unsigned long long *d_nkmers);
int hymet_screen_stats(hymet_ctx *ctx, const int64_t *d_ref_off, int64_t n_refs,
                       const int32_t *d_canon_of, const uint32_t *d_counts, uint32_t *d_shared,
                       uint32_t *d_median);
int hymet_screen_winner(hymet_ctx *ctx, const int64_t *d_ref_off, int64_t n_refs,
                        const int32_t *d_canon_of, const uint32_t *d_counts, int64_t n_hashes,
                        const int32_t *d_comp, int64_t n_comp, uint32_t *d_win, uint32_t *d_shared,
                        uint32_t *d_median);

int64_t hymet_sketch_max_size(void);
int hymet_sketch_batch(hymet_ctx *ctx, const uint32_t *d_2b, const uint32_t *d_mask, int64_t n_bases,
                       int k, uint32_t seed, int32_t s, int64_t n_chunks, const int32_t *h_chunk_sketch,
                       const int64_t *h_chunk_begin, const int64_t *h_chunk_end, int32_t n_sketches,
                       uint64_t *d_out, int32_t *d_out_n);
int hymet_sketch_counted(hymet_ctx *ctx, const uint32_t *d_2b, const uint32_t *d_mask, int64_t n_bases,
                         int k, uint32_t seed, int32_t s, int32_t min_copies, int64_t n_chunks,
                         const int32_t *h_chunk_sketch, const int64_t *h_chunk_begin,
                         const int64_t *h_chunk_end, int32_t n_sketches, uint64_t *d_out,
                         uint32_t *d_out_count, int32_t *d_out_n, int64_t *h_stats);
int hymet_sketch_counted_max_size(void);
int hymet_sketch_counted_tune(int keep);
typedef struct hymet_sketch_stream hymet_sketch_stream;
int hymet_sketch_stream_create(hymet_ctx *ctx, int k, uint32_t seed, int32_t s, int32_t min_copies,
                               int64_t max_live, hymet_sketch_stream **out);
int hymet_sketch_stream_add(hymet_sketch_stream *st, const uint32_t *d_2b, const uint32_t *d_mask,
                            int64_t n_bases, int64_t slice_bases);
int hymet_sketch_stream_end_pass(hymet_sketch_stream *st, int32_t *need_more);
int hymet_sketch_stream_result(hymet_sketch_stream *st, uint64_t *d_out, uint32_t *d_out_count, int32_t *n,
                               int64_t *h_stats);
int hymet_sketch_stream_destroy(hymet_sketch_stream *st);

int hymet_mash_dist(hymet_ctx *ctx, const uint64_t *d_ref_hashes, int64_t n_ref_hashes, const int64_t *d_ref_off,
                    int64_t n_ref, const uint64_t *d_qry_hashes, int64_t n_qry_hashes, const int64_t *d_qry_off,
                    int64_t n_qry, int64_t q_begin, int64_t q_end, int32_t s, uint32_t *d_out);
int hymet_mash_dist_tile(int32_t s);
int hymet_mash_dist_tune(int path, int tq);
int hymet_mash_dist_select(hymet_ctx *ctx, const uint32_t *d_block, int64_t n_rows, int64_t n_ref,
                           const uint16_t *d_min_common, int32_t s, int64_t *d_row_off, int32_t *d_ref_idx,
                           uint32_t *d_val, int64_t cap, int64_t *total);
int hymet_mash_dist_tri(hymet_ctx *ctx, const uint64_t *d_hashes, int64_t n_hashes, const int64_t *d_off, int64_t n,
                        int64_t q_begin, int64_t q_end, int32_t s, uint32_t *d_out);
int hymet_mash_link(hymet_ctx *ctx, const uint32_t *d_block, int64_t n_rows, int64_t n, int64_t q_begin,
                    const uint16_t *d_min_common, int32_t s, int32_t *d_parent, uint64_t *d_n_links);
int hymet_mash_labels(hymet_ctx *ctx, int32_t *d_parent, int64_t n, int32_t *d_label);
typedef struct hymet_sparse_counters {
    int64_t postings, emitted, candidates;
} hymet_sparse_counters;
int hymet_mash_dist_sparse(hymet_ctx *ctx, const uint64_t *d_ref_hashes, int64_t n_ref_hashes, const int64_t *d_ref_off,
                           int64_t n_ref, const uint64_t *d_qry_hashes, int64_t n_qry_hashes, const int64_t *d_qry_off,
                           int64_t n_qry, int64_t q_begin, int64_t q_end, int32_t s, int tri,
                           const uint16_t *d_min_common, int32_t cmin, int64_t max_pairs, int64_t *d_row_off,
                           int32_t *d_ref_idx, uint32_t *d_val, int64_t cap, int64_t *total,
                           hymet_sparse_counters *counters);
int hymet_mash_link_edges(hymet_ctx *ctx, const int64_t *d_row_off, int64_t n_rows, int64_t q_begin,
                          const int32_t *d_ref_idx, int32_t *d_parent, uint64_t *d_n_links);
int hymet_mash_greedy(hymet_ctx *ctx, const uint32_t *d_block, int64_t n_rows, int64_t n, int64_t q_begin,
                      const uint16_t *d_min_common, int32_t s, int32_t *d_rep, uint64_t *d_n_links, int32_t *rounds);
int hymet_mash_greedy_edges(hymet_ctx *ctx, const int64_t *d_row_off, int64_t n_rows, int64_t q_begin,
                            const int32_t *d_ref_idx, const uint32_t *d_val, int32_t s, int32_t *d_rep,
                            uint64_t *d_n_links, int32_t *rounds);
int32_t hymet_mash_topk_max(void);
int hymet_mash_topk_tune(int chunk_entries);
int hymet_mash_dist_topk(hymet_ctx *ctx, const uint32_t *d_block, int64_t n_rows, int64_t n_ref,
                         const uint16_t *d_min_common, int32_t s, int32_t K, int32_t *d_idx, uint32_t *d_val,
                         int32_t *d_cnt);
int hymet_mash_topk_edges(hymet_ctx *ctx, const int64_t *d_row_off, int64_t n_rows, const int32_t *d_ref_idx,
                          const uint32_t *d_val_in, int32_t s, int32_t K, int32_t *d_idx, uint32_t *d_val,
                          int32_t *d_cnt);

typedef struct hymet_mm_index hymet_mm_index;
int hymet_mm_sketch(hymet_ctx *ctx, const uint32_t *d_2b, const uint32_t *d_mask, const int64_t *h_starts,
                    const int64_t *h_lens, int32_t n_seq, int w, int k, int rid_mode, uint64_t *h_x,
                    uint64_t *h_y, int64_t cap, int64_t *n_out);
int hymet_mm_index_build(hymet_ctx *ctx, const uint32_t *d_2b, const uint32_t *d_mask, const int64_t *h_starts,
                         const int64_t *h_lens, int32_t n_seq, int w, int k, hymet_mm_index **out);
int hymet_mm_index_destroy(hymet_mm_index *idx);
int hymet_mm_index_info(const hymet_mm_index *idx, int32_t *w, int32_t *k, int32_t *n_seq, int64_t *n_pos);
int hymet_mm_index_max_occ(hymet_ctx *ctx, const hymet_mm_index *idx, float frac, int32_t *out);
int hymet_mm_index_save(hymet_ctx *ctx, const hymet_mm_index *idx, const char *path, int append, int64_t *end_offset);
int hymet_mm_index_load(hymet_ctx *ctx, const char *path, int64_t offset, hymet_mm_index **out, int64_t *end_offset);
int hymet_mm_index_export(hymet_ctx *ctx, const hymet_mm_index *idx, uint32_t *h_hash, uint64_t *h_pos);

typedef struct {
    int32_t mid_occ;
    float q_occ_frac;
    int32_t max_max_occ, occ_dist;
    int32_t min_cnt, min_chain_score;
    int32_t bw, bw_long, max_gap, max_chain_skip;
    int32_t rmq_inner_dist, rmq_size_cap, rmq_rescue_size;
    float rmq_rescue_ratio;
    float chain_gap_scale, chain_skip_scale;
    float mask_level, pri_ratio;
    int32_t mask_len, best_n, a, b, seed;
} hymet_mm_opt;

typedef struct {
    int32_t qs, qe, rs, re, rid, rev;
    int32_t mlen, blen, mapq, cnt, score, subsc, parent, id, n_sub, strand_retained;
    float div;
    int32_t as;
    uint32_t hash;
    int32_t pad;
} hymet_mm_reg;

typedef struct hymet_mm_result hymet_mm_result;
int hymet_mm_map(hymet_ctx *ctx, const hymet_mm_index *idx, const hymet_mm_opt *opt,
                 const uint32_t *d_2b, const uint32_t *d_mask, const int64_t *h_starts,
                 const int64_t *h_lens, const uint32_t *h_name_hash, int32_t n_q,
                 hymet_mm_result **out);
int hymet_mm_result_size(const hymet_mm_result *res, int64_t *n_regs);
int hymet_mm_result_copy(const hymet_mm_result *res, int64_t *h_off, int32_t *h_rep_len,
                         hymet_mm_reg *h_regs);
int hymet_mm_result_destroy(hymet_mm_result *res);
typedef struct hymet_paf_acc hymet_paf_acc;
int hymet_paf_acc_create(hymet_ctx *ctx, hymet_paf_acc **out);
int hymet_paf_acc_reset(hymet_paf_acc *acc);
int hymet_paf_acc_destroy(hymet_paf_acc *acc);
int hymet_paf_acc_info(const hymet_paf_acc *acc, int64_t *n_lines, void **d_regs, void **d_q, void **d_part, void **d_rl,
                       void **d_t);
int hymet_paf_acc_append(hymet_ctx *ctx, hymet_paf_acc *dst, const hymet_paf_acc *src, int64_t begin, int64_t end);
int hymet_paf_acc_copy(hymet_ctx *ctx, const hymet_paf_acc *acc, int32_t *h_q, int32_t *h_part, int32_t *h_t);
int hymet_paf_acc_field(hymet_ctx *ctx, const hymet_paf_acc *acc, int field, int32_t *h_out);
int hymet_mm_map_acc(hymet_ctx *ctx, const hymet_mm_index *idx, const hymet_mm_opt *opt, const uint32_t *d_2b,
                     const uint32_t *d_mask, const int64_t *h_starts, const int64_t *h_lens, const uint32_t *d_name_hash,
                     int32_t n_q, int32_t q_base, int32_t part_id, int32_t t_base, hymet_paf_acc *acc);
int hymet_emit_paf(hymet_ctx *ctx, const hymet_paf_acc *acc, const uint8_t *d_qname, const int64_t *d_qname_off,
                   const int64_t *d_qlen, const uint8_t *d_tname, const int64_t *d_tname_off, const int64_t *d_tlen,
                   char *d_out, int64_t cap, int64_t *n_bytes, int64_t *d_line_off);
int hymet_mm_chain_dp(hymet_ctx *ctx, const uint64_t *h_x, const uint64_t *h_y, int64_t n, int max_dist,
                      int max_dist_inner, int bw, int max_chn_skip, int cap_rmq_size, float pen_gap,
                      float pen_skip, int32_t *h_f, int64_t *h_p);
int hymet_mm_mark_compact(hymet_ctx *ctx, const uint64_t *h_x, const uint64_t *h_y, const int32_t *h_mark, int64_t n,
                          const int64_t *h_qoff, const uint32_t *h_qflag, int32_t n_q, uint64_t *h_ox, uint64_t *h_oy,
                          uint32_t *h_ohb, int64_t *n_kept);
int hymet_mm_stamp_scratch(hymet_ctx *ctx, int64_t *capacity, int64_t *nonzero);
int hymet_mm_anchor_sort(hymet_ctx *ctx, const uint64_t *h_key, const uint32_t *h_val, int64_t n,
                         const int64_t *h_qoff, int32_t n_q, int32_t rb, int32_t pb, uint64_t yhi, int64_t max_qlen,
                         uint64_t *h_ax, uint64_t *h_ay, uint32_t *h_ax32, uint32_t *h_hb, int64_t *h_stats);

int hymet_lca_ref_counts(hymet_ctx *ctx, const int32_t *d_line_t, int64_t n_lines, int32_t *d_counts);
int hymet_acc_ref_counts(hymet_ctx *ctx, const hymet_paf_acc *acc, int32_t *d_counts);
int hymet_acc_classify(hymet_ctx *ctx, const hymet_paf_acc *acc, int mode, int32_t n_q, const int64_t *d_qlen,
                       const int32_t *d_ref_counts, const int32_t *d_t_tax, const int32_t *d_tax_names,
                       const uint8_t *d_tax_in_hier, const uint8_t *d_qname_pool, const int64_t *d_qname_off,
                       const uint8_t *d_tname_pool, const int64_t *d_tname_off, int32_t *d_row_q, int32_t *d_row_part,
                       int32_t *d_row_depth, int32_t *d_row_names, double *d_row_conf, int32_t *d_row_tax,
                       int32_t *n_rows);
int hymet_emit_tsv(hymet_ctx *ctx, int mode, int32_t n_rows, const int32_t *d_row_q, const int32_t *d_row_depth,
                   const int32_t *d_row_names, const double *d_row_conf, const int32_t *d_row_tax, const uint8_t *d_qname,
                   const int64_t *d_qname_off, const uint8_t *d_label, const int64_t *d_label_off, const uint8_t *d_taxlin,
                   const int64_t *d_taxlin_off, const uint8_t *d_taxlvl, const int64_t *d_taxlvl_off, char *d_out,
                   int64_t cap, int64_t *n_bytes);
int hymet_lca(hymet_ctx *ctx, int mode, int32_t n_q, const int64_t *d_q_off, const int32_t *d_line_t,
              const int64_t *d_line_blen, const int64_t *d_line_qlen, const uint8_t *d_line_exact,
              const int32_t *d_ref_counts, const int32_t *d_t_tax, const int32_t *d_tax_names,
              const uint8_t *d_tax_in_hier, int32_t *d_scr_tid, double *d_scr_w, int32_t *d_scr_nm,
              double *d_scr_nw, int32_t *d_out_depth, int32_t *d_out_names, double *d_out_conf,
              int32_t *d_out_tax);

#ifdef __cplusplus
}
#endif
#endif
```

Baseline: 136,000.

## Skip index indirection for contiguous chain ranges in backtrack and chain stats

Two paths now detect when a group's or block's anchors form a contiguous index range and read them directly instead of through an index array. In z-order, long single-run groups no longer write z_idx and are flagged with z_runs=-1, so backtrack probes f/p/t directly. The chain-stats kernel gains a per-block descriptor pass that spots blocks whose chain ids form a contiguous range and runs a coalesced fast path without the shared-memory segment walk. This adds an extra descriptor kernel and a larger per-block struct, plus optional env-gated counters.

```diff
diff --git a/hymet_amd/_lib.py b/hymet_amd/_lib.py
--- a/hymet_amd/_lib.py
+++ b/hymet_amd/_lib.py
@@ -102,6 +102,7 @@
     "hymet_mm_chain_dp": (_i32, [_vp, _vp, _vp, _i64, _i32, _i32, _i32, _i32, _i32, _c.c_float, _c.c_float, _vp, _vp]),
     "hymet_mm_mark_compact": (_i32, [_vp, _vp, _vp, _vp, _i64, _vp, _vp, _i32, _vp, _vp, _vp, _c.POINTER(_i64)]),
     "hymet_mm_stamp_scratch": (_i32, [_vp, _c.POINTER(_i64), _c.POINTER(_i64)]),
+    "hymet_mm_range_counters": (_i32, [_vp, _vp, _i32]),
     "hymet_mm_anchor_sort": (_i32, [_vp, _vp, _vp, _i64, _vp, _i32, _i32, _i32, _u64, _i64, _vp, _vp, _vp, _vp, _vp]),
     "hymet_lca_ref_counts": (_i32, [_vp, _vp, _i64, _vp]),
     "hymet_lca": (_i32, [_vp, _i32, _i32] + [_vp] * 17),
diff --git a/hymet_amd/csrc/common.hpp b/hymet_amd/csrc/common.hpp
--- a/hymet_amd/csrc/common.hpp
+++ b/hymet_amd/csrc/common.hpp
@@ -27,6 +27,7 @@
     int32_t *stamp = nullptr;
     int64_t stamp_cap = 0;
     size_t stamp_cls = 0;
+    int64_t range_ctr[7] = {0, 0, 0, 0, 0, 0, 0};
 };
 
 namespace hymet {
diff --git a/hymet_amd/csrc/mm_chain.hip b/hymet_amd/csrc/mm_chain.hip
--- a/hymet_amd/csrc/mm_chain.hip
+++ b/hymet_amd/csrc/mm_chain.hip
@@ -1326,6 +1326,8 @@
     uint8_t *t;
     const int32_t *z_cnt;
     const int32_t *z_idx;
+    const int32_t *z_runs;
+    unsigned long long *zctr;
     int32_t n_groups;
     int min_cnt, min_sc, max_drop;
     int64_t long_min;
@@ -1338,7 +1340,6 @@
 
 constexpr int kBtWin = 8;
 
-constexpr int64_t kBtLong = 64;
 #ifndef HYMET_BT_GRAB
 #define HYMET_BT_GRAB 1
 #endif
@@ -1400,14 +1401,20 @@
         }
         const int32_t g = uni(list[wcur]);
         const int64_t g0 = uni64(P.g_start[g]);
-        const int64_t z0 = g0, z1 = g0 + uni(P.z_cnt[g]);
+        const int32_t nz = uni(P.z_cnt[g]);
+        const bool direct = uni(P.z_runs[g]) < 0;
+        const int64_t z0 = g0, z1 = direct ? uni64(P.g_start[g + 1]) : g0 + nz;
+        if (P.zctr) {
+            atomicAdd(P.zctr + (direct ? 0 : 2), lane == 0 ? 1ull : 0ull);
+            atomicAdd(P.zctr + (direct ? 1 : 3), lane == 0 ? (unsigned long long)nz : 0ull);
+        }
         int64_t wpos = g0;
         int nc = 0;
         int64_t k = z1 - 1;
         uint64_t c_probe = 0, c_walk = 0, c_step = 0, c_reload = 0, t_walk = 0, t_post = 0;
         const uint64_t t_g0 = P.prof ? clock64() : 0;
         int64_t ptop = -1;
-        int64_t zrem = z1 - z0;
+        int64_t zrem = nz;
         int32_t zc[kBtProbe], tv[kBtProbe], zfv[kBtProbe];
         int32_t zpv[kBtProbe];
         int32_t tqv[kBtProbe], fqv[kBtProbe];
@@ -1417,20 +1424,38 @@
                 c_probe++;
                 ptop = k;
                 stale = false;
+                if (direct) {
 #pragma unroll
-                for (int c = 0; c < kBtProbe; c++) {
-                    const int64_t kk = k - 64 * c - lane;
-                    zc[c] = kk >= z0 ? P.z_idx[kk] : 0;
-                }
+                    for (int c = 0; c < kBtProbe; c++) {
+                        const int64_t kk = k - 64 * c - lane;
+                        const bool ok = kk >= z0;
+                        zc[c] = ok ? (int32_t)kk : 0;
+                        tv[c] = ok ? ld_l2(P.t + kk) : 1;
+                        zfv[c] = ok ? P.f[kk] : 0;
+                        zpv[c] = ok ? P.p[kk] : -1;
+                    }
 #pragma unroll
-                for (int c = 0; c < kBtProbe; c++) {
-                    const int64_t kk = k - 64 * c - lane;
-                    tv[c] = kk >= z0 ? ld_l2(P.t + zc[c]) : 1;
-                }
+                    for (int c = 0; c < kBtProbe; c++) {
+                        tv[c] = zfv[c] < P.min_sc ? 1 : tv[c];
+                        zfv[c] = tv[c] == 0 ? zfv[c] : 0;
+                        zpv[c] = tv[c] == 0 ? zpv[c] : -1;
+                    }
+                } else {
 #pragma unroll
-                for (int c = 0; c < kBtProbe; c++) {
-                    zfv[c] = tv[c] == 0 ? P.f[zc[c]] : 0;
-                    zpv[c] = tv[c] == 0 ? P.p[zc[c]] : -1;
+                    for (int c = 0; c < kBtProbe; c++) {
+                        const int64_t kk = k - 64 * c - lane;
+                        zc[c] = kk >= z0 ? P.z_idx[kk] : 0;
+                    }
+#pragma unroll
+                    for (int c = 0; c < kBtProbe; c++) {
+                        const int64_t kk = k - 64 * c - lane;
+                        tv[c] = kk >= z0 ? ld_l2(P.t + zc[c]) : 1;
+                    }
+#pragma unroll
+                    for (int c = 0; c < kBtProbe; c++) {
+                        zfv[c] = tv[c] == 0 ? P.f[zc[c]] : 0;
+                        zpv[c] = tv[c] == 0 ? P.p[zc[c]] : -1;
+                    }
                 }
 #pragma unroll
                 for (int c = 0; c < kBtProbe; c++) {
@@ -1858,19 +1883,25 @@
 }
 
 int launch_backtrack(hymet_ctx *ctx, const int64_t *g_start, const int32_t *f, const int32_t *p, uint8_t *t,
-                     const int32_t *z_cnt, const int32_t *z_idx, int32_t n_groups, const int32_t *order, int32_t n_work,
-                     int min_cnt, int min_sc, int max_drop, int32_t *chain_ids, uint64_t *chain_u, int64_t *chain_first,
-                     int32_t *n_chains, int64_t n_anchors) {
+                     const int32_t *z_cnt, const int32_t *z_idx, const int32_t *z_runs, int32_t n_groups, const int32_t *order,
+                     int32_t n_work, int min_cnt, int min_sc, int max_drop, int32_t *chain_ids, uint64_t *chain_u,
+                     int64_t *chain_first, int32_t *n_chains, int64_t n_anchors) {
     if (n_groups <= 0) return HYMET_OK;
-    const int64_t long_min = env_int("HYMET_BT_LONG", kBtLong, 0, INT64_MAX);
+    const int64_t long_min = bt_long_min();
     const bool prof = env_flag("HYMET_BT_PROF");
-    DevBuf pbuf;
+    const bool log_stats = env_flag("HYMET_RANGE_STATS");
+    DevBuf pbuf, zbuf;
     if (prof) {
         HY_HIP(pbuf.alloc(64, ctx->stream));
         HY_HIP(hipMemsetAsync(pbuf.p, 0, 64, ctx->stream));
     }
-    BacktrackParams P{g_start,  f,         p,       t,           z_cnt,    z_idx, n_groups, min_cnt, min_sc, max_drop,
-                      long_min, (unsigned long long *)pbuf.p, chain_ids, chain_u, chain_first, n_chains};
+    if (log_stats) {
+        HY_HIP(zbuf.alloc(32, ctx->stream));
+        HY_HIP(hipMemsetAsync(zbuf.p, 0, 32, ctx->stream));
+    }
+    BacktrackParams P{g_start, f,       p,      t,        z_cnt,    z_idx, z_runs, (unsigned long long *)zbuf.p, n_groups,
+                      min_cnt, min_sc,  max_drop, long_min, (unsigned long long *)pbuf.p, chain_ids, chain_u, chain_first,
+                      n_chains};
     DevBuf cnt;
     HY_HIP(cnt.alloc(4 * (size_t)kBtCtrPad * (kBtStripes + 1), ctx->stream));
     ProfScope _ps(ctx, "mm_backtrack", 18.0 * (double)n_anchors);
@@ -1896,6 +1927,13 @@
         fprintf(stderr, "[bt_long] groups=%llu probes=%llu walks=%llu steps=%llu reloads=%llu cyc_walk=%.3g cyc_post=%.3g cyc_all=%.3g\n",
                 h[0], h[1], h[2], h[3], h[4], (double)h[5], (double)h[6], (double)h[7]);
     }
+    if (log_stats) {
+        unsigned long long h[4];
+        HY_HIP(hipMemcpyAsync(h, zbuf.p, 32, hipMemcpyDeviceToHost, ctx->stream));
+        HY_HIP(hipStreamSynchronize(ctx->stream));
+        for (int i = 0; i < 4; i++) ctx->range_ctr[3 + i] += (int64_t)h[i];
+        fprintf(stderr, "[z_direct] direct_groups %llu direct_z %llu listed_groups %llu listed_z %llu\n", h[0], h[1], h[2], h[3]);
+    }
     return HYMET_OK;
 }
 
diff --git a/hymet_amd/csrc/mm_chainset.hip b/hymet_amd/csrc/mm_chainset.hip
--- a/hymet_amd/csrc/mm_chainset.hip
+++ b/hymet_amd/csrc/mm_chainset.hip
@@ -11,9 +11,9 @@
                  int max_dist_inner, int bw, int max_chn_skip, int cap_rmq_size, float pen_gap, float pen_skip,
                  int64_t n_anchors, int64_t n_groups);
 int launch_backtrack(hymet_ctx *ctx, const int64_t *g_start, const int32_t *f, const int32_t *p, uint8_t *t,
-                     const int32_t *z_cnt, const int32_t *z_idx, int32_t n_groups, const int32_t *order, int32_t n_work,
-                     int min_cnt, int min_sc, int max_drop, int32_t *chain_ids, uint64_t *chain_u, int64_t *chain_first,
-                     int32_t *n_chains, int64_t n_anchors);
+                     const int32_t *z_cnt, const int32_t *z_idx, const int32_t *z_runs, int32_t n_groups, const int32_t *order,
+                     int32_t n_work, int min_cnt, int min_sc, int max_drop, int32_t *chain_ids, uint64_t *chain_u,
+                     int64_t *chain_first, int32_t *n_chains, int64_t n_anchors);
 
 namespace {
 
@@ -163,6 +163,7 @@
     int32_t *big_list;
     int64_t *big_off;
     int64_t *mail;
+    int64_t direct_min;
 };
 
 __global__ void zsplit_kernel(ZParams P) {
@@ -220,6 +221,7 @@
             const int64_t n = (int64_t)((uint64_t)(uint32_t)__builtin_amdgcn_readlane((int32_t)(el >> 32), r) << 32 |
                                         (uint32_t)__builtin_amdgcn_readlane((int32_t)el, r)) - g0;
             int32_t *rs = P.run_start + (int64_t)g * kZRuns;
+            const bool defer = n > P.direct_min;
             int m = 0, K = 0;
             uint64_t last = 0;
             const uint64_t below = (1ull << lane) - 1;
@@ -246,7 +248,7 @@
                     if (!lower) pk = last;
                     const bool desc = z && pos > 0 && key < pk;
                     const uint64_t dbal = __ballot(desc);
-                    if (z) P.z_idx[g0 + pos] = (int32_t)(g0 + i);
+                    if (z && !defer) P.z_idx[g0 + pos] = (int32_t)(g0 + i);
                     if (desc) {
                         const int r = K + 1 + __popcll(dbal & below);
                         if (r < kZRuns) rs[r] = pos;
@@ -260,7 +262,7 @@
             if (lane == 0) {
                 rs[0] = 0;
                 P.z_cnt[g] = m;
-                P.z_runs[g] = runs;
+                P.z_runs[g] = defer && runs == 1 ? -1 : runs;
             }
             if (runs > 1) {
                 int m2 = 0;
@@ -675,7 +677,7 @@
 };
 
 struct ZOrder {
-    DevBuf idx, cnt;
+    DevBuf idx, cnt, runs;
 };
 
 struct Backtrack {
@@ -749,11 +751,11 @@
 
 static int z_order(hymet_ctx *ctx, int min_sc, const DevBuf &f, int64_t n, const Groups &Gr, const WorkList &W, ZOrder &Z) {
     const int64_t G = Gr.G;
-    DevBuf zkey, z_runs, run_start, merge_list, mergeu_list, mid_list, big_list, big_off;
+    DevBuf zkey, run_start, merge_list, mergeu_list, mid_list, big_list, big_off;
     HY_HIP(zkey.alloc(8 * (size_t)n, ctx->stream));
     HY_HIP(Z.idx.alloc(4 * (size_t)n, ctx->stream));
     HY_HIP(Z.cnt.alloc(4 * (size_t)G, ctx->stream));
-    HY_HIP(z_runs.alloc(4 * (size_t)G, ctx->stream));
+    HY_HIP(Z.runs.alloc(4 * (size_t)G, ctx->stream));
     HY_HIP(run_start.alloc(4 * (size_t)G * kZRuns, ctx->stream));
     HY_HIP(merge_list.alloc(4 * (size_t)G, ctx->stream));
     const int zm_lds = (int)env_int("HYMET_ZM_LDS", kZmLds, 0, kZmLds);
@@ -764,11 +766,12 @@
     HY_HIP(big_list.alloc(4 * (size_t)G, ctx->stream));
     HY_HIP(big_off.alloc(8 * (size_t)G, ctx->stream));
     ProfScope _ps(ctx, "mm_z_order", 16.0 * (double)n);
+    const int64_t direct_min = env_flag("HYMET_Z_DIRECT", true) ? bt_long_min() : INT64_MAX;
     ZParams P{f.as<int32_t>(), Gr.g_start.as<int64_t>(), W.order.as<int32_t>(), (int32_t)G, min_sc,
-              max_runs, zm_lds, zm_unit, zkey.as<uint64_t>(), Z.idx.as<int32_t>(), Z.cnt.as<int32_t>(), z_runs.as<int32_t>(),
+              max_runs, zm_lds, zm_unit, zkey.as<uint64_t>(), Z.idx.as<int32_t>(), Z.cnt.as<int32_t>(), Z.runs.as<int32_t>(),
               run_start.as<int32_t>(), W.zlists.as<int32_t>(), merge_list.as<int32_t>(), mergeu_list.as<int64_t>(),
               mid_list.as<int32_t>(), big_list.as<int32_t>(),
-              big_off.as<int64_t>(), mb_dev(ctx, kMbZBig)};
+              big_off.as<int64_t>(), mb_dev(ctx, kMbZBig), direct_min};
     hipLaunchKernelGGL(zsplit_kernel, dim3(1), dim3(64), 0, ctx->stream, P);
     HY_CHECK_LAUNCH("zsplit_kernel");
     const int64_t nwb = std::min<int64_t>(cdiv(G, 4), (int64_t)ctx->n_cu * 8);
@@ -814,7 +817,7 @@
     HY_HIP(B.first.alloc(8 * (size_t)n, ctx->stream));
     HY_HIP(B.n_chains.alloc(4 * (size_t)Gr.G, ctx->stream));
     return launch_backtrack(ctx, Gr.g_start.as<int64_t>(), f.as<int32_t>(), p.as<int32_t>(), t.as<uint8_t>(), Z.cnt.as<int32_t>(),
-                            Z.idx.as<int32_t>(), (int32_t)Gr.G, W.order.as<int32_t>(), (int32_t)W.n_work, opt->min_cnt,
+                            Z.idx.as<int32_t>(), Z.runs.as<int32_t>(), (int32_t)Gr.G, W.order.as<int32_t>(), (int32_t)W.n_work, opt->min_cnt,
                             opt->min_chain_score, bw, B.ids.as<int32_t>(), B.u.as<uint64_t>(), B.first.as<int64_t>(),
                             B.n_chains.as<int32_t>(), n);
 }
@@ -1058,6 +1061,16 @@
     return HYMET_OK;
 }
 
+extern "C" int hymet_mm_range_counters(hymet_ctx *ctx, int64_t *out, int32_t reset) {
+    HY_ARG(ctx && out, "hymet_mm_range_counters: null argument");
+    HY_HIP(hipSetDevice(ctx->device));
+    HY_HIP(hipStreamSynchronize(ctx->stream));
+    for (int i = 0; i < 7; i++) out[i] = ctx->range_ctr[i];
+    if (reset)
+        for (int i = 0; i < 7; i++) ctx->range_ctr[i] = 0;
+    return HYMET_OK;
+}
+
 extern "C" int hymet_mm_mark_compact(hymet_ctx *ctx, const uint64_t *h_x, const uint64_t *h_y, const int32_t *h_mark, int64_t n,
                                      const int64_t *h_qoff, const uint32_t *h_qflag, int32_t n_q, uint64_t *h_ox,
                                      uint64_t *h_oy, uint32_t *h_ohb, int64_t *n_kept) {
diff --git a/hymet_amd/csrc/mm_common.hpp b/hymet_amd/csrc/mm_common.hpp
--- a/hymet_amd/csrc/mm_common.hpp
+++ b/hymet_amd/csrc/mm_common.hpp
@@ -89,6 +89,9 @@
     uint32_t *overflow;
 };
 
+constexpr int64_t kBtLong = 64;
+inline int64_t bt_long_min() { return env_int("HYMET_BT_LONG", kBtLong, 0, INT64_MAX); }
+
 int launch_sketch(hymet_ctx *ctx, int w, bool write, const SketchParams &P);
 
 int exclusive_scan_u32_i64(hymet_ctx *ctx, const uint32_t *in, int64_t *out, int64_t n, int64_t *total);
diff --git a/hymet_amd/csrc/mm_regs.hip b/hymet_amd/csrc/mm_regs.hip
--- a/hymet_amd/csrc/mm_regs.hip
+++ b/hymet_amd/csrc/mm_regs.hip
@@ -126,18 +126,153 @@
 constexpr int kStatItems = HYMET_STAT_ITEMS;
 constexpr int kStatSpan = 256 * kStatItems;
 
-__global__ void block_chain_kernel(const int64_t *cboff, int64_t NC, int64_t NB, int32_t *blk_c0) {
+struct alignas(16) StatBlk {
+    int32_t c, a0, cnt, j0;
+    int32_t ap, an, qlen, skip;
+    int64_t qbase, pad;
+};
+static_assert(sizeof(StatBlk) == 48, "StatBlk: three 16-byte words");
+
+__global__ void block_chain_kernel(const int64_t *cboff, int64_t NC, int64_t NB, StatBlk *blk) {
     const int64_t c = (int64_t)blockIdx.x * blockDim.x + threadIdx.x;
     if (c >= NC) return;
     const int64_t s = cboff[c], e = c + 1 < NC ? cboff[c + 1] : NB;
-    for (int64_t b = (s + kStatSpan - 1) / kStatSpan; b * kStatSpan < e; ++b) blk_c0[b] = (int32_t)c;
-}
-
-__global__ __launch_bounds__(256) void chain_stats_flat_kernel(AnchorStatParams P, const int32_t *blk_c0, int32_t *c_fv) {
+    for (int64_t b = (s + kStatSpan - 1) / kStatSpan; b * kStatSpan < e; ++b) blk[b].c = (int32_t)c;
+}
+
+constexpr int kProfStatGather = 4;
+__global__ __launch_bounds__(256) void block_desc_kernel(AnchorStatParams P, int64_t n_blk, int range_on, StatBlk *blk,
+                                                         unsigned long long *ctr, unsigned long long *gathered) {
+    const int64_t b = (int64_t)blockIdx.x * blockDim.x + threadIdx.x;
+    if (b >= n_blk) return;
+    const int64_t c = blk[b].c;
+    const int64_t b0 = b * kStatSpan, b1 = min(b0 + kStatSpan, P.NB);
+    const int64_t s = P.cboff[c], e = c + 1 < P.NC ? P.cboff[c + 1] : P.NB;
+    int32_t a0 = -1;
+    if (b1 <= e) {
+        const int32_t cnt = (int32_t)P.cu[c];
+        const int64_t f0 = P.cfirst[c] + cnt - 1;
+        const int32_t j0 = (int32_t)(b0 - s), j1 = (int32_t)(b1 - 1 - s);
+        const int32_t first = P.ids[f0 - j0], last = P.ids[f0 - j1];
+        const bool range = range_on && last - first == j1 - j0;
+        if (range) {
+            const int64_t q = (int64_t)P.cq[c];
+            StatBlk d;
+            d.c = (int32_t)c, d.a0 = a0 = first, d.cnt = cnt, d.j0 = j0;
+            d.ap = j0 > 0 ? P.ids[f0 - j0 + 1] : -1;
+            d.an = j1 + 1 < cnt ? P.ids[f0 - j1 - 1] : -1;
+            d.qlen = (int32_t)P.qlen[q];
+            d.skip = P.skip_q && P.skip_q[q];
+            d.qbase = P.qbase[q], d.pad = 0;
+            blk[b] = d;
+        }
+        if (ctr) {
+            atomicAdd(ctr, (unsigned long long)(b1 - b0));
+            if (range) atomicAdd(ctr + 1, (unsigned long long)(b1 - b0));
+        }
+    }
+    if (a0 < 0) {
+        blk[b].a0 = -1;
+        if (gathered) atomicAdd(gathered, (unsigned long long)(b1 - b0));
+    }
+}
+
+__device__ __forceinline__ void chain_stats_range(const AnchorStatParams &P, const StatBlk &D, int32_t *c_fv) {
+    constexpr int K = kStatItems;
+    if (D.skip) return;
+    const int lane = threadIdx.x & 63;
+    const int64_t b0 = (int64_t)blockIdx.x * kStatSpan;
+    const int32_t cnt = D.cnt, qlen = D.qlen, span = P.span;
+    const int64_t qbase = D.qbase;
+    bool act[K];
+    int32_t j[K], cur[K], cur_e[K], ae[K];
+    uint64_t x[K], xe[K];
+    uint32_t y[K], ye[K];
+#pragma unroll
+    for (int k = 0; k < K; k++) {
+        const int r = 256 * k + (int)threadIdx.x;
+        act[k] = b0 + r < P.NB;
+        const int rr = act[k] ? r : 0;
+        j[k] = D.j0 + rr;
+        const int32_t a = D.a0 + rr;
+        x[k] = P.ax[a], y[k] = P.ay[a];
+        ae[k] = -1;
+        if (act[k] && lane == 0 && j[k] > 0) ae[k] = r == 0 ? D.ap : a - 1;
+        if (act[k] && lane == 63 && j[k] + 1 < cnt) ae[k] = r == kStatSpan - 1 ? D.an : a + 1;
+        xe[k] = 0, ye[k] = 0;
+        if (ae[k] >= 0) xe[k] = P.ax[ae[k]], ye[k] = P.ay[ae[k]];
+    }
+    const bool rev = x[0] >> 63;
+#pragma unroll
+    for (int k = 0; k < K; k++) {
+        int32_t xq = (int32_t)y[k];
+        if (rev) xq = qlen - 1 - (int32_t)y[k] + span - 1;
+        const bool inq = xq >= 0 && xq < qlen;
+        const int32_t xc = inq ? xq : 0;
+        const int32_t v = mini_word_idx(P.mtab[(qbase + xc) >> 6], xc);
+        cur[k] = act[k] && inq ? v : -1;
+        cur_e[k] = -1;
+        if (ae[k] >= 0) {
+            int32_t xqe = (int32_t)ye[k];
+            if (rev) xqe = qlen - 1 - (int32_t)ye[k] + span - 1;
+            if (xqe >= 0 && xqe < qlen) cur_e[k] = mini_word_idx(P.mtab[(qbase + xqe) >> 6], xqe);
+        }
+    }
+    int32_t t_dm = 0, t_db = 0, t_fv = INT32_MAX;
+#pragma unroll
+    for (int k = 0; k < K; k++) {
+        uint64_t xp = __shfl_up(x[k], 1, 64);
+        uint32_t yp = __shfl_up(y[k], 1, 64);
+        int32_t cur_p = __shfl_up(cur[k], 1, 64), cur_n = __shfl_down(cur[k], 1, 64);
+        if (lane == 0) xp = xe[k], yp = ye[k], cur_p = cur_e[k];
+        if (lane == 63) cur_n = cur_e[k];
+        if (!act[k]) continue;
+        int dm, db;
+        if (j[k] == 0) {
+            dm = db = span;
+        } else {
+            const int32_t tl = (int32_t)x[k] - (int32_t)xp;
+            const int32_t ql = (int32_t)y[k] - (int32_t)yp;
+            db = tl > ql ? tl : ql;
+            dm = tl > span && ql > span ? span : tl < ql ? tl : ql;
+        }
+        const int32_t kk = rev ? cnt - 1 - j[k] : j[k];
+        int fv = cnt;
+        if (kk >= 1) {
+            const int32_t prev = rev ? cur_n : cur_p;
+            if (cur[k] < 0 || cur[k] <= prev) fv = kk;
+        }
+        if (kk == 0) P.c_st[D.c] = cur[k];
+        if (kk == cnt - 1) P.c_last[D.c] = cur[k];
+        t_dm += dm, t_db += db, t_fv = min(t_fv, fv);
+    }
+    __shared__ int32_t r_dm[4], r_db[4], r_fv[4];
+#pragma unroll
+    for (int o = 32; o > 0; o >>= 1) {
+        t_dm += __shfl_xor(t_dm, o, 64);
+        t_db += __shfl_xor(t_db, o, 64);
+        t_fv = min(t_fv, __shfl_xor(t_fv, o, 64));
+    }
+    const int w = threadIdx.x >> 6;
+    if (lane == 0) r_dm[w] = t_dm, r_db[w] = t_db, r_fv[w] = t_fv;
+    __syncthreads();
+    if (threadIdx.x == 0) {
+        atomicAdd(P.c_mlen + D.c, r_dm[0] + r_dm[1] + r_dm[2] + r_dm[3]);
+        atomicAdd(P.c_blen + D.c, r_db[0] + r_db[1] + r_db[2] + r_db[3]);
+        atomicMin(c_fv + D.c, min(min(r_fv[0], r_fv[1]), min(r_fv[2], r_fv[3])));
+    }
+}
+
+__global__ __launch_bounds__(256) void chain_stats_flat_kernel(AnchorStatParams P, const StatBlk *blk, int32_t *c_fv) {
     constexpr int K = kStatItems;
     __shared__ int32_t s_st[kStatSpan + 1];
     const int64_t b0 = (int64_t)blockIdx.x * kStatSpan;
-    const int64_t cb0 = blk_c0[blockIdx.x];
+    const StatBlk D = blk[blockIdx.x];
+    if (D.a0 >= 0) {
+        chain_stats_range(P, D, c_fv);
+        return;
+    }
+    const int64_t cb0 = D.c;
     for (int i = threadIdx.x; i <= kStatSpan; i += blockDim.x) {
         const int64_t cc = cb0 + i;
         s_st[i] = cc < P.NC ? (int32_t)min(P.cboff[cc] - b0, (int64_t)kStatSpan) : kStatSpan;
@@ -1058,20 +1193,39 @@
     int32_t *c_mlen = cst.as<int32_t>(), *c_blen = c_mlen + (NC + 1), *c_st = c_blen + (NC + 1), *c_last = c_st + (NC + 1),
             *c_fv = c_last + (NC + 1);
     {
-        ProfScope _ps(ctx, "mm_chain_stats", (double)NB * (4.0 + 12.0 + 4.0) + (double)NM * 8.0);
+        ProfScope _ps(ctx, "mm_chain_stats", (double)NB * (12.0 + 4.0) + (double)NM * 8.0);
+        if (ctx->prof) ctx->dev_bytes["mm_chain_stats"] = {kProfStatGather, 4.0};
         AnchorStatParams A{ax, cu, ay, span, ids, cfirst, cboff, qb, qlen, mp_off, mini_pos, NB, NC, n_q, cq,
                            c_mlen, c_blen, c_st, c_last, mtab, qbase, skip_q};
         if (NB > 0) {
             hipLaunchKernelGGL(chain_stats_init_kernel, dim3((unsigned)cdiv(NC + 1, 256)), dim3(256), 0, st, c_mlen, c_blen,
                                c_fv, NC + 1);
             HY_CHECK_LAUNCH("chain_stats_init_kernel");
-            HY_HIP(blk.alloc(4 * (size_t)(cdiv(NB, kStatSpan) + 1), st));
+            const int64_t n_blk = cdiv(NB, kStatSpan);
+            HY_HIP(blk.alloc(sizeof(StatBlk) * (size_t)(n_blk + 1), st));
             hipLaunchKernelGGL(block_chain_kernel, dim3((unsigned)cdiv(NC, 256)), dim3(256), 0, st, cboff, NC, NB,
-                               blk.as<int32_t>());
+                               blk.as<StatBlk>());
             HY_CHECK_LAUNCH("block_chain_kernel");
-            hipLaunchKernelGGL(chain_stats_flat_kernel, dim3((unsigned)cdiv(NB, kStatSpan)), dim3(256), 0, st, A,
-                               (const int32_t *)blk.as<int32_t>(), c_fv);
+            const bool range_on = env_flag("HYMET_STAT_RANGE", true), log_stats = env_flag("HYMET_RANGE_STATS");
+            DevBuf rctr;
+            if (log_stats) {
+                HY_HIP(rctr.alloc(16, st));
+                HY_HIP(hipMemsetAsync(rctr.p, 0, 16, st));
+            }
+            hipLaunchKernelGGL(block_desc_kernel, dim3((unsigned)cdiv(n_blk, 256)), dim3(256), 0, st, A, n_blk, (int)range_on,
+                               blk.as<StatBlk>(), log_stats ? rctr.as<unsigned long long>() : nullptr,
+                               (unsigned long long *)prof_dev_slot(ctx, kProfStatGather));
+            HY_CHECK_LAUNCH("block_desc_kernel");
+            hipLaunchKernelGGL(chain_stats_flat_kernel, dim3((unsigned)n_blk), dim3(256), 0, st, A,
+                               (const StatBlk *)blk.as<StatBlk>(), c_fv);
             HY_CHECK_LAUNCH("chain_stats_flat_kernel");
+            if (log_stats) {
+                unsigned long long h[2] = {};
+                HY_HIP(hipMemcpyAsync(h, rctr.p, 16, hipMemcpyDeviceToHost, st));
+                HY_HIP(hipStreamSynchronize(st));
+                ctx->range_ctr[0] += (int64_t)NB, ctx->range_ctr[1] += (int64_t)h[0], ctx->range_ctr[2] += (int64_t)h[1];
+                fprintf(stderr, "[stat_range] positions %lld one_chain_blocks %llu range_blocks %llu\n", (long long)NB, h[0], h[1]);
+            }
         }
         if (!sumk_done) {
             const int nqb = n_q < ctx->n_cu * 64 ? n_q : ctx->n_cu * 64;
diff --git a/include/hymet_gpu.h b/include/hymet_gpu.h
--- a/include/hymet_gpu.h
+++ b/include/hymet_gpu.h
@@ -212,6 +212,7 @@
                           const int64_t *h_qoff, const uint32_t *h_qflag, int32_t n_q, uint64_t *h_ox, uint64_t *h_oy,
                           uint32_t *h_ohb, int64_t *n_kept);
 int hymet_mm_stamp_scratch(hymet_ctx *ctx, int64_t *capacity, int64_t *nonzero);
+int hymet_mm_range_counters(hymet_ctx *ctx, int64_t *out, int32_t reset);
 int hymet_mm_anchor_sort(hymet_ctx *ctx, const uint64_t *h_key, const uint32_t *h_val, int64_t n,
                          const int64_t *h_qoff, int32_t n_q, int32_t rb, int32_t pb, uint64_t yhi, int64_t max_qlen,
                          uint64_t *h_ax, uint64_t *h_ay, uint32_t *h_ax32, uint32_t *h_hb, int64_t *h_stats);
```

Measured after the change: 138,000 (median of 6 runs). 1.4% higher.
